# imatge-upc/rsis

Hardware: AMD Instinct MI355X
Metric: training images/sec at 256x256, T=10, batch=32 per GPU (higher is better)
Workload: dtype f32

## Files before the change

### include/rsis_hip.h

```cpp
#ifndef RSIS_HIP_H
#define RSIS_HIP_H
#include <stddef.h>
#ifdef __cplusplus
extern "C" {
#endif

#define RSIS_ABI_VERSION 2

#define RSIS_DTYPE_F32 0
#define RSIS_DTYPE_BF16 1
#define RSIS_DTYPE_BF16_BLK 2
#define RSIS_DTYPE_F32_WINO 3

int rsis_version(void);
const char* rsis_error_string(int code);
int rsis_conv_uses_wino(int ks, int stride, int pad, int Cin, int Cout, int nseg, int lstm_hid);

int rsis_set_deterministic(int on);
int rsis_get_deterministic(void);

int rsis_conv_uses_bf16(int ks, int stride, int pad, int Cout);
long rsis_conv_packed_bytes_fwd(int dtype, int Cout, int ks, int stride, int pad, int nseg, const int* Cseg);
long rsis_conv_packed_bytes_dgrad(int dtype, int Cout, int ks, int stride, int pad, int c_count);
int rsis_conv_pack_fwd(const float* W, void* Wp, int Cout, int Ctot, int ks, int stride, int pad, int nseg, const int* Cseg,
                       const int* Coff, int lstm_hid, int dtype, void* stream);
int rsis_conv_pack_dgrad(const float* W, void* Wd, int Cout, int Ctot, int ks, int stride, int pad, int nseg, const int* Cseg,
                         const int* Coff, int lstm_hid, int dtype, void* stream);

int rsis_conv2d_fwd(const float* const* src, const int* Csrc, int nsrc, int B, int H, int W, const void* Wp, int Cout,
                    int ks, int stride, int pad, const float* bias, const float* addend, float* out, int Ho, int Wo,
                    int tile, int dtype, void* stream);
int rsis_conv2d_fwd_bn_eval(const float* const* src, const int* Csrc, int nsrc, int B, int H, int W, const void* Wp, int Cout,
                            int ks, int stride, int pad, const float* bias, const float* addend, const float* gamma, const float* beta,
                            const float* running_mean, const float* running_var, float eps, int relu, float* out, int Ho, int Wo,
                            int tile, int dtype, void* stream);

int rsis_conv2d_dgrad(const float* dy, int B, int Cout, int Hy, int Wy, const void* Wd, int Cin_packed, int ks, int stride,
                      int pad, float* const* dx, const int* Cdx, int ndst, int Hx, int Wx, const float* addend, int tile,
                      int dtype, void* stream);

int rsis_conv2d_wgrad(const float* dy, const float* x, float* dW, int B, int Cs, int H, int W, int Cout, int Ho, int Wo,
                      int ks, int stride, int pad, int Ctot, int c_off, int lstm_hid, int dtype, void* stream);

typedef struct rsis_wgrad_job {
  const float* dy;
  const float* x;
  float* dW;
  int B, Cs, H, W, Cout, Ho, Wo, ks, stride, pad, Ctot, c_off, lstm_hid, dtype;
} rsis_wgrad_job;
int rsis_conv2d_wgrad_batch(const rsis_wgrad_job* jobs, int njobs, void* stream);

int rsis_bias_grad(const float* dy, float* db, int B, int C, int HW, int lstm_hid, void* stream);

int rsis_convlstm_fwd(const float* const* src, const int* Csrc, int nsrc, int B, int H, int W, const void* Wp,
                      const float* bias_packed, const float* addend, const float* c_prev, float* h_out, float* c_out,
                      float* act_out, int hid, int ks, int pad, int tile, int dtype, void* stream);

typedef struct rsis_lstm_job {
  const float* src[3];
  int Csrc[3];
  int nsrc, B, H, W;
  const void* Wp;
  const float* bias_packed;
  const float* addend;
  const float* c_prev;
  float* h_out;
  float* c_out;
  float* act_out;
  int hid, ks, pad, tile, dtype;
  unsigned long long* side_key;
} rsis_lstm_job;
int rsis_convlstm_fwd_batch(const rsis_lstm_job* jobs, int njobs, void* stream);

int rsis_convlstm_bwd_gates(const float* dh, const float* dh2, const float* dc_next, const float* act, const float* c_prev,
                            const float* c, float* da, float* dc_prev, float* da_sum, int B, int hid, int HW, void* stream);

typedef struct rsis_lstm_bwd_job {
  const float* dh;
  const float* dh2;
  const float* dc_next;
  const float* act;
  const float* c_prev;
  const float* c;
  float* da;
  float* dc_prev;
  int B, hid, HW;
} rsis_lstm_bwd_job;
int rsis_convlstm_bwd_gates_batch(const rsis_lstm_bwd_job* jobs, int njobs, void* stream);
typedef struct rsis_dgrad_job {
  const float* dy;
  int B, Cout, Hy, Wy;
  const void* Wd;
  int Cin_packed, ks, stride, pad;
  float* dx[3];
  int Cdx[3];
// ... 264 lines not shown
```

### rsis_amd/csrc/api.hip

```cpp
#include "common.h"
#include "../../include/rsis_hip.h"
#include "launchers.h"
#include <stdlib.h>

static inline int krows_of(int C, int ks) { return rsis_roundup(C * ks * ks, RSIS_KPAD); }
static inline int log2i(int s) { int l = 0; while ((1 << l) < s) ++l; return l; }
static inline bool use_direct(int ks, int stride, int pad) { return ks == 3 && stride == 1 && pad == 1; }
static inline bool use_direct_s2(int ks, int stride, int pad) { return ks == 3 && stride == 2 && pad == 1; }
static inline bool use_direct_f2(int ks, int stride, int pad) {
  static const bool on = !(getenv("RSIS_CONV_F2") && getenv("RSIS_CONV_F2")[0] == '0');
  return on && use_direct_s2(ks, stride, pad);
}
static inline bool use_direct_fwd(int ks, int stride, int pad) { return use_direct(ks, stride, pad) || use_direct_f2(ks, stride, pad); }
static inline int seg_chunks(int nseg, const int* Cseg, int ck) {
  int q = 0;
  for (int s = 0; s < nseg; ++s) q += (Cseg[s] + ck - 1) / ck;
  return q;
}
static inline int direct_rows(int nseg, const int* Cseg) { return seg_chunks(nseg, Cseg, RSIS_CK) * RSIS_CK * 9; }
static inline bool bf16_geom(int ks, int stride, int pad, int Cout) {
  return Cout > 1 && ((ks == 3 && stride == 1 && pad == 1) || (ks == 1 && pad == 0));
}
static inline bool use_bf16(int dtype, int ks, int stride, int pad, int Cout) {
  return dtype == RSIS_DTYPE_BF16 && bf16_geom(ks, stride, pad, Cout);
}
static inline bool wino_geom(int ks, int stride, int pad, int Cin, int Cout, int nseg, int lstm_hid) {
  return ks == 3 && stride == 1 && pad == 1 && nseg == 1 && lstm_hid == 0 && Cin >= 32 && Cout >= 32 && Cin % 32 == 0 && Cout % 32 == 0;
}
static inline bool wino_geom_dgrad(int ks, int stride, int pad, int Cin, int Cout) {
  return ks == 3 && stride == 1 && pad == 1 && Cin >= 32 && Cout >= 32 && Cin % 32 == 0 && Cout % 32 == 0;
}
static inline bool use_wino(int dtype, int ks, int stride, int pad, int Cin, int Cout, int nseg, int lstm_hid) {
  return dtype == RSIS_DTYPE_F32_WINO && wino_geom(ks, stride, pad, Cin, Cout, nseg, lstm_hid);
}
static inline int bf16_rows(int ks, int nseg, const int* Cseg) {
  const int ckb = bf16_ckb(ks * ks);
  return seg_chunks(nseg, Cseg, ckb) * ks * ks * (ckb / 8);
}
static int g_deterministic = -1;
int rsis_deterministic() {
  if (g_deterministic < 0) g_deterministic = (getenv("RSIS_DETERMINISTIC") && getenv("RSIS_DETERMINISTIC")[0] == '1') ? 1 : 0;
  return g_deterministic;
}
static inline bool conv_splitk_ok() {
  static const bool env_ok = !(getenv("RSIS_CONV_SPLITK") && getenv("RSIS_CONV_SPLITK")[0] == '0');
  return env_ok && !rsis_deterministic();
}
static inline bool splitk_geom(int B, int H, int W, int rows, int nq, int min_chunks) {
  const long px_tiles = (long)B * rsis_cdiv(H, 8) * rsis_cdiv(W, W <= 8 ? 8 : 16);
  return nq >= min_chunks && px_tiles * rsis_cdiv(rows, 64) < 160;
}
static int zero_dsts(const ConvArgs& a, hipStream_t st) {
  for (int i = 0; i < a.ndst; ++i)
    if (rsis_zero_async(a.dst[i], sizeof(float) * (size_t)a.B * a.Cd[i] * a.oH * a.oW, st) != RSIS_OK) return RSIS_ERR_LAUNCH;
  return RSIS_OK;
}
static int splitk_enable(ConvArgs& a, hipStream_t st) { a.ksplit = 0; return zero_dsts(a, st); }
static inline int direct_variant(int tile) { const int v = tile % 10; return (tile > 0 && v >= 1 && v <= 9) ? v : 0; }

extern "C" {

int rsis_version(void) { return RSIS_ABI_VERSION; }

int rsis_set_deterministic(int on) {
  const int prev = rsis_deterministic();
  g_deterministic = on ? 1 : 0;
  return prev;
}
int rsis_get_deterministic(void) { return rsis_deterministic(); }

const char* rsis_error_string(int code) {
  switch (code) {
    case RSIS_OK: return "ok";
    case RSIS_ERR_ARG: return "invalid argument";
    case RSIS_ERR_LAUNCH: return "HIP launch failed";
    case RSIS_ERR_UNSUPPORTED: return "unsupported configuration";
    default: return "unknown error";
  }
}

int rsis_conv_uses_bf16(int ks, int stride, int pad, int Cout) { return bf16_geom(ks, stride, pad, Cout) ? 1 : 0; }
int rsis_conv_uses_wino(int ks, int stride, int pad, int Cin, int Cout, int nseg, int lstm_hid) {
  return wino_geom(ks, stride, pad, Cin, Cout, nseg, lstm_hid) ? 1 : 0;
}

struct PackPlan { int status; PackMode mode; int krows; int ldw; long bytes; };
static PackPlan pack_plan(bool dgrad, int dtype, int Cout, int Ctot, int ks, int stride, int pad, int nseg, const int* Cseg, const int* Coff,
                          int lstm_hid) {
  PackPlan p = {RSIS_OK, PACK_IGEMM_FWD, 0, 0, 0};
  int csum = 0;
  for (int s = 0; s < nseg; ++s) csum += Cseg[s];
  p.ldw = rsis_roundup(dgrad ? csum : Cout, RSIS_LDW_ALIGN);
  if (lstm_hid > 0 && dtype == RSIS_DTYPE_BF16 && ks != 3) { p.status = RSIS_ERR_UNSUPPORTED; return p; }
  if (dtype == RSIS_DTYPE_F32_WINO && (dgrad ? wino_geom_dgrad(ks, stride, pad, csum, Cout) : wino_geom(ks, stride, pad, csum, Cout, nseg, lstm_hid))) {
    if (!dgrad && (csum != Ctot || (Coff && Coff[0] != 0))) { p.status = RSIS_ERR_UNSUPPORTED; return p; }
    p.mode = dgrad ? PACK_WINO_DGRAD : PACK_WINO_FWD;
    p.krows = dgrad ? (csum / 32) * (Cout / 8) : (Cout / 32) * (csum / 8);
    p.bytes = (long)p.krows * 32 * 8 * 16 * 4;
    return p;
  }
  long cell = 4;
  if (use_bf16(dtype, ks, stride, pad, Cout)) {
    p.mode = dgrad ? PACK_BF16_DGRAD : PACK_BF16_FWD;
    p.krows = dgrad ? bf16_rows(ks, 1, &Cout) : bf16_rows(ks, nseg, Cseg);
    cell = 16;
  } else if (dgrad ? use_direct(ks, stride, pad) : use_direct_fwd(ks, stride, pad)) {
    p.mode = dgrad ? PACK_DIRECT_DGRAD : PACK_DIRECT_FWD;
    p.krows = dgrad ? direct_rows(1, &Cout) : direct_rows(nseg, Cseg);
  } else if (dgrad && use_direct_s2(ks, stride, pad) && nseg == 1) {
    p.mode = PACK_DIRECT_DGRAD_S2;
    p.krows = direct_rows(1, &Cout);
  } else {
    p.mode = dgrad ? PACK_IGEMM_DGRAD : PACK_IGEMM_FWD;
    p.krows = krows_of(dgrad ? Cout : csum, ks);
  }
  p.bytes = (long)p.krows * p.ldw * cell;
  return p;
}

long rsis_conv_packed_bytes_fwd(int dtype, int Cout, int ks, int stride, int pad, int nseg, const int* Cseg) {
  if (nseg < 1 || nseg > RSIS_MAX_SRC || !Cseg) return -1;
  int csum = 0;
  for (int s = 0; s < nseg; ++s) csum += Cseg[s];
  return pack_plan(false, dtype, Cout, csum, ks, stride, pad, nseg, Cseg, nullptr, 0).bytes;
}

long rsis_conv_packed_bytes_dgrad(int dtype, int Cout, int ks, int stride, int pad, int c_count) {
  const int one[1] = {c_count}, two[2] = {c_count, 0};
  const long a = pack_plan(true, dtype, Cout, c_count, ks, stride, pad, 1, one, nullptr, 0).bytes;
  const long b = pack_plan(true, dtype, Cout, c_count, ks, stride, pad, 2, two, nullptr, 0).bytes;
  return a > b ? a : b;
}

static int pack_args_check(int Cout, int Ctot, int ks, int nseg, const int* Cseg, const int* Coff, int lstm_hid) {
  if (nseg < 1 || nseg > RSIS_MAX_SRC || !Cseg) return RSIS_ERR_ARG;
  int base = 0;
  for (int s = 0; s < nseg; ++s) {
    const int off = Coff ? Coff[s] : base;
    if (Cseg[s] < 1 || off < 0 || off + Cseg[s] > Ctot) return RSIS_ERR_ARG;
    base += Cseg[s];
  }
  if (Cout < 1 || ks < 1 || (long)Cout * Ctot * ks * ks >= (1L << 31)) return RSIS_ERR_ARG;
  return (lstm_hid > 0 && Cout != 4 * lstm_hid) ? RSIS_ERR_ARG : RSIS_OK;
}

static int pack_one(bool dgrad, const float* W, void* out, int Cout, int Ctot, int ks, int stride, int pad, int nseg, const int* Cseg,
                    const int* Coff, int lstm_hid, int dtype, void* stream) {
  if (!W || !out || pack_args_check(Cout, Ctot, ks, nseg, Cseg, Coff, lstm_hid)) return RSIS_ERR_ARG;
  const PackPlan p = pack_plan(dgrad, dtype, Cout, Ctot, ks, stride, pad, nseg, Cseg, Coff, lstm_hid);
  if (p.status) return p.status;
  return rsis_l_pack(p.mode, W, out, Cout, Ctot, ks, nseg, Cseg, Coff, p.ldw, p.krows, lstm_hid, (hipStream_t)stream);
}
int rsis_conv_pack_fwd(const float* W, void* Wp, int Cout, int Ctot, int ks, int stride, int pad, int nseg, const int* Cseg,
                       const int* Coff, int lstm_hid, int dtype, void* stream) {
  return pack_one(false, W, Wp, Cout, Ctot, ks, stride, pad, nseg, Cseg, Coff, lstm_hid, dtype, stream);
}
int rsis_conv_pack_dgrad(const float* W, void* Wd, int Cout, int Ctot, int ks, int stride, int pad, int nseg, const int* Cseg,
                         const int* Coff, int lstm_hid, int dtype, void* stream) {
  return pack_one(true, W, Wd, Cout, Ctot, ks, stride, pad, nseg, Cseg, Coff, lstm_hid, dtype, stream);
}

int rsis_conv_pack_job_fill(rsis_pack_job* j) {
  if (!j || pack_args_check(j->Cout, j->Ctot, j->ks, j->nseg, j->Cseg, j->Coff, j->lstm_hid)) return -1;
  const PackPlan p = pack_plan(j->dgrad != 0, j->dtype, j->Cout, j->Ctot, j->ks, j->stride, j->pad, j->nseg, j->Cseg, j->Coff, j->lstm_hid);
  if (p.status) return -1;
  j->imode = p.mode; j->krows = p.krows; j->ldw = p.ldw;
  return rsis_l_pack_blocks(p.mode, p.krows, p.ldw, j->ks);
}

int rsis_conv_pack_batch(const rsis_pack_job* jobs_dev, int njobs, int total_blocks, void* stream) {
  if (!jobs_dev || njobs < 1 || total_blocks < 1) return RSIS_ERR_ARG;
  return rsis_l_pack_batch(jobs_dev, njobs, total_blocks, (hipStream_t)stream);
}


int rsis_conv_out_wgrad(const float* dy, const float* x, float* dW, float* db, int B, int Cin, int H, int W, void* stream) {
  if (!dy || !x || !dW || B < 1) return RSIS_ERR_ARG;
  if (!rsis_c1_supported(Cin) || W % 4 != 0) return RSIS_ERR_UNSUPPORTED;
  return rsis_l_c1_wgrad(dy, x, dW, db, B, Cin, H, W, 1, (hipStream_t)stream);
}

static inline bool c1_seq_ok(int T, int B, int Cin, int H, int W) {
  return T >= 1 && B >= 1 && rsis_c1_supported(Cin) && W % 4 == 0 && (long)T * B * Cin * H * W < (1L << 40);
}
int rsis_conv_out_seq_fwd(const float* x, const void* Wp, const float* bias, float* y, int T, int B, int Cin, int H, int W, void* stream) {
// ... 11 lines not shown
  if (!c1_seq_ok(T, B, Cin, H, W)) return RSIS_ERR_UNSUPPORTED;
  return rsis_l_c1_wgrad(dy, x, dW, db, T * B, Cin, H, W, T, (hipStream_t)stream);
}
int rsis_sum_leading(const float* x, float* y, int T, long n, void* stream) {
  if (!x || !y || T < 1 || n < 1) return RSIS_ERR_ARG;
  return rsis_l_sum_leading(x, y, T, n, (hipStream_t)stream);
}

int rsis_affine_nearest(const float* x, float* y, const float* mat, int mat_rows, int N, int C, int H, int W, void* stream) {
  if (!x || !y || !mat || x == y || N < 1 || C < 1 || H < 1 || W < 1 || (mat_rows != 2 && mat_rows != 3)) return RSIS_ERR_ARG;
  if ((long)H * W >= (1L << 31) || N > 65535) return RSIS_ERR_UNSUPPORTED;
  return rsis_l_affine_nearest(x, y, mat, N, C, H, W, mat_rows * 3, (hipStream_t)stream);
}

long rsis_targets_work_ints(int B) { return B < 1 ? 0 : rsis_l_targets_work_ints(B); }

int rsis_targets_from_maps(const int* ins, const int* seg, int B, int H, int W, int T, float* y_mask, long long* y_class, float* sw_mask,
                           float* sw_class, int* work, void* stream) {
  if (!ins || !seg || !y_mask || !y_class || !sw_mask || !sw_class || !work || B < 1 || H < 1 || W < 1 || T < 1) return RSIS_ERR_ARG;
  if ((long)H * W >= (1L << 31) || B > 65535) return RSIS_ERR_UNSUPPORTED;
  return rsis_l_targets_from_maps(ins, seg, B, H, W, T, y_mask, y_class, sw_mask, sw_class, work, (hipStream_t)stream);
}

long rsis_instance_maps_work_ints(int B) { return B < 1 ? 0 : rsis_l_instance_maps_work_ints(B); }

int rsis_instance_maps(const int* raw, const int* class_of_label, int n_labels, int B, int H, int W, int* ins, int* seg, int* work,
                       void* stream) {
  if (!raw || !class_of_label || !ins || !seg || !work || raw == ins || raw == seg || ins == seg || n_labels < 1 || n_labels > 66 ||
      B < 1 || H < 1 || W < 1)
    return RSIS_ERR_ARG;
  if ((long)H * W >= (1L << 31) || B > 65535) return RSIS_ERR_UNSUPPORTED;
  return rsis_l_instance_maps(raw, class_of_label, n_labels, B, H, W, ins, seg, work, (hipStream_t)stream);
}

int rsis_palette_to_ids(const unsigned char* rgb, long npix, const unsigned char* table, int ntab, unsigned char* ids, void* stream) {
  if (!rgb || !table || !ids || npix < 1 || ntab < 1 || ntab > 256) return RSIS_ERR_ARG;
  return rsis_l_palette_to_ids(rgb, npix, table, ntab, ids, (hipStream_t)stream);
}

int rsis_idmap_rle_encode(const unsigned char* idmap, int h, int w, const int* ids, int k, unsigned int* counts, int cap, int* nruns,
                          void* stream) {
  if (!idmap || !ids || !counts || !nruns || h < 1 || w < 1 || k < 1 || cap < 1 || (long)h * w >= (1L << 32)) return RSIS_ERR_ARG;
  return rsis_l_idmap_rle_encode(idmap, h, w, ids, k, counts, cap, nruns, (hipStream_t)stream);
}

static int fill_sources(ConvArgs& a, const float* const* src, const int* Csrc, int nsrc, int ks, bool allow_empty = false) {
  if (nsrc < (allow_empty ? 0 : 1) || nsrc > RSIS_MAX_SRC || (nsrc > 0 && (!src || !Csrc))) return RSIS_ERR_ARG;
  a.nsrc = nsrc;
  a.K = 0;
  for (int s = 0; s < RSIS_MAX_SRC; ++s) { a.src[s] = nsrc > 0 ? src[0] : nullptr; a.C[s] = 0; }
  for (int s = 0; s < nsrc; ++s) {
    if (!src[s] || Csrc[s] < 1) return RSIS_ERR_ARG;
    a.src[s] = src[s]; a.C[s] = Csrc[s]; a.K += Csrc[s] * ks * ks;
  }
  return RSIS_OK;
}

struct BnEval { const float* gamma; const float* beta; const float* mean; const float* var; float eps; int relu; };

static int conv2d_fwd_impl(const float* const* src, const int* Csrc, int nsrc, int B, int H, int W, const void* Wp, int Cout,
                           int ks, int stride, int pad, const float* bias, const float* addend, float* out, int Ho, int Wo,
                           int tile, int dtype, void* stream, const BnEval* bn) {
  const bool allow_splitk = tile >= 100;
  tile %= 100;
  ConvArgs a = {};
  int rc = fill_sources(a, src, Csrc, nsrc, ks);
  if (rc) return rc;
  if (!Wp || !out || B < 1 || stride < 1) return RSIS_ERR_ARG;
  if (Ho != (H + 2 * pad - ks) / stride + 1 || Wo != (W + 2 * pad - ks) / stride + 1) return RSIS_ERR_ARG;
  a.B = B; a.H = H; a.W = W; a.Ho = Ho; a.Wo = Wo; a.stride = stride; a.pad = pad; a.sshift = 0;
  a.wp = (const float*)Wp; a.ldw = rsis_roundup(Cout, RSIS_LDW_ALIGN); a.Cout = Cout; a.bias = bias; a.addend = addend;
  a.dst[0] = out; a.Cd[0] = Cout; a.ndst = 1;
  a.ostride = 1; a.oH = Ho; a.oW = Wo; a.ksplit = 1;
  a.precise = allow_splitk ? 0 : 1;
  if (bn) {
    if (!bn->gamma || !bn->beta || !bn->mean || !bn->var) return RSIS_ERR_ARG;
    if (allow_splitk || Cout % 4 != 0 || (size_t)B * Cout * Ho * Wo * 4 >= (1ull << 31)) return RSIS_ERR_UNSUPPORTED;
    if (dtype != RSIS_DTYPE_F32 && (dtype != RSIS_DTYPE_BF16 || use_bf16(dtype, ks, stride, pad, Cout))) return RSIS_ERR_UNSUPPORTED;
    if (use_direct(ks, stride, pad) && Cout == 1) return RSIS_ERR_UNSUPPORTED;
    a.ep_gamma = bn->gamma; a.ep_beta = bn->beta; a.ep_mean = bn->mean; a.ep_var = bn->var; a.ep_eps = bn->eps; a.ep_relu = bn->relu ? 1 : 0;
  }
  if (use_wino(dtype, ks, stride, pad, Csrc[0], Cout, nsrc, 0))
    return rsis_launch_conv_wino(src[0], Wp, bias, addend, out, B, Csrc[0], Cout, H, W, (hipStream_t)stream, a.precise);
  if (use_bf16(dtype, ks, stride, pad, Cout)) {
    if (stride != 1) return RSIS_ERR_UNSUPPORTED;
    if (ks == 1 && nsrc != 1) return RSIS_ERR_UNSUPPORTED;
    if (ks == 3 && allow_splitk && conv_splitk_ok() && !addend && splitk_geom(B, H, W, Cout, seg_chunks(a.nsrc, a.C, RSIS_CKB3), 16) &&
        splitk_enable(a, (hipStream_t)stream))
      return RSIS_ERR_LAUNCH;
    return rsis_launch_conv_bf16(a, ks, 0, direct_variant(tile), (hipStream_t)stream);
  }
  if (use_direct(ks, stride, pad) && Cout == 1 && nsrc == 1 && !addend && rsis_c1_supported(Csrc[0]) && W % 4 == 0)
    return rsis_l_c1_fwd(src[0], (const float*)Wp, a.ldw, bias, out, B, Csrc[0], H, W, 1, (hipStream_t)stream);
  if (use_direct(ks, stride, pad)) {
    if (allow_splitk && conv_splitk_ok() && splitk_geom(B, H, W, Cout, seg_chunks(a.nsrc, a.C, RSIS_CK), 32) && splitk_enable(a, (hipStream_t)stream))
      return RSIS_ERR_LAUNCH;
    return rsis_launch_conv3x3_direct(a, 0, direct_variant(tile), (hipStream_t)stream);
  }
  if (use_direct_f2(ks, stride, pad))
    return rsis_launch_conv3x3_direct(a, 3, direct_variant(tile), (hipStream_t)stream);
  return rsis_launch_conv_igemm(a, ks, false, 0, tile, (hipStream_t)stream);
}

int rsis_conv2d_fwd(const float* const* src, const int* Csrc, int nsrc, int B, int H, int W, const void* Wp, int Cout,
                    int ks, int stride, int pad, const float* bias, const float* addend, float* out, int Ho, int Wo,
                    int tile, int dtype, void* stream) {
  return conv2d_fwd_impl(src, Csrc, nsrc, B, H, W, Wp, Cout, ks, stride, pad, bias, addend, out, Ho, Wo, tile, dtype, stream, nullptr);
}

int rsis_conv2d_fwd_bn_eval(const float* const* src, const int* Csrc, int nsrc, int B, int H, int W, const void* Wp, int Cout,
                            int ks, int stride, int pad, const float* bias, const float* addend, const float* gamma, const float* beta,
                            const float* running_mean, const float* running_var, float eps, int relu, float* out, int Ho, int Wo,
                            int tile, int dtype, void* stream) {
  const BnEval bn = {gamma, beta, running_mean, running_var, eps, relu};
  return conv2d_fwd_impl(src, Csrc, nsrc, B, H, W, Wp, Cout, ks, stride, pad, bias, addend, out, Ho, Wo, tile % 100, dtype, stream, &bn);
}

static int dgrad_fill(ConvArgs& a, const float* dy, int B, int Cout, int Hy, int Wy, const void* Wd, int Cin_packed, int ks, int stride, int pad,
                      float* const* dx, const int* Cdx, int ndst, int Hx, int Wx, const float* addend) {
  a = ConvArgs{};
  const float* srcs[1] = {dy};
  const int cs[1] = {Cout};
  const int rc = fill_sources(a, srcs, cs, 1, ks);
  if (rc) return rc;
  int ctot = 0;
  for (int i = 0; i < ndst; ++i) { if (!dx[i] || Cdx[i] < 1) return RSIS_ERR_ARG; a.dst[i] = dx[i]; a.Cd[i] = Cdx[i]; ctot += Cdx[i]; }
  if (ctot > Cin_packed) return RSIS_ERR_ARG;
  a.ndst = ndst;
  a.B = B; a.H = Hy; a.W = Wy; a.Ho = Hx; a.Wo = Wx; a.stride = stride; a.pad = pad; a.sshift = log2i(stride);
  a.ostride = 1; a.oH = Hx; a.oW = Wx; a.ksplit = 1;
  a.wp = (const float*)Wd; a.ldw = rsis_roundup(Cin_packed, RSIS_LDW_ALIGN); a.Cout = ctot; a.bias = nullptr; a.addend = addend;
  return RSIS_OK;
}

int rsis_conv2d_dgrad(const float* dy, int B, int Cout, int Hy, int Wy, const void* Wd, int Cin_packed, int ks, int stride,
                      int pad, float* const* dx, const int* Cdx, int ndst, int Hx, int Wx, const float* addend, int tile,
                      int dtype, void* stream) {
  if (!dy || !Wd || !dx || !Cdx || ndst < 1 || ndst > RSIS_MAX_SRC) return RSIS_ERR_ARG;
  const bool inplace = addend && ndst == 1 && stride > 1 && ks == 1 && pad == 0 && addend == dx[0];
  if (addend && !inplace && (ndst != 1 || stride != 1)) return RSIS_ERR_UNSUPPORTED;
  if (stride != 1 && stride != 2 && stride != 4) return RSIS_ERR_UNSUPPORTED;
  ConvArgs a;
  const int rc = dgrad_fill(a, dy, B, Cout, Hy, Wy, Wd, Cin_packed, ks, stride, pad, dx, Cdx, ndst, Hx, Wx, addend);
  if (rc) return rc;
  const int ctot = a.Cout;
  if (dtype == RSIS_DTYPE_F32_WINO && wino_geom_dgrad(ks, stride, pad, Cin_packed, Cout)) {
    if (ndst > 2 || ctot % 32 != 0 || Cdx[0] % 32 != 0 || Hx != Hy || Wx != Wy || (ndst == 2 && addend)) return RSIS_ERR_UNSUPPORTED;
    if (ndst == 1) return rsis_launch_conv_wino(dy, Wd, nullptr, addend, dx[0], B, Cout, ctot, Hy, Wy, (hipStream_t)stream, 0);
    const float* xs[1] = {dy}; const void* us[1] = {Wd}; float* y0[1] = {dx[0]}; float* y1[1] = {dx[1]};
    const int b1[1] = {B}, c1[1] = {Cout}, co1[1] = {ctot}, c01[1] = {Cdx[0]}, h1[1] = {Hy}, w1[1] = {Wy};
    return rsis_launch_conv_wino_group(1, xs, us, y0, y1, b1, c1, co1, c01, h1, w1, (hipStream_t)stream);
  }
  if (use_bf16(dtype, ks, stride, pad, Cout)) {
    if (ks == 3) {
      if (Hx != Hy || Wx != Wy) return RSIS_ERR_ARG;
      if (conv_splitk_ok() && !addend && splitk_geom(B, Hx, Wx, ctot, seg_chunks(a.nsrc, a.C, RSIS_CKB3), 16) && splitk_enable(a, (hipStream_t)stream))
        return RSIS_ERR_LAUNCH;
      return rsis_launch_conv_bf16(a, 3, 0, direct_variant(tile), (hipStream_t)stream);
    }
    if (stride > 1) {
      if (Hy != (Hx - 1) / stride + 1 || Wy != (Wx - 1) / stride + 1) return RSIS_ERR_ARG;
      if (!inplace && zero_dsts(a, (hipStream_t)stream)) return RSIS_ERR_LAUNCH;
      a.ostride = stride;
    } else if (Hx != Hy || Wx != Wy) return RSIS_ERR_ARG;
    a.Ho = Hy; a.Wo = Wy; a.stride = 1; a.sshift = 0;
    return rsis_launch_conv_bf16(a, 1, 0, direct_variant(tile), (hipStream_t)stream);
  }
  if (use_direct(ks, stride, pad)) {
    if (Hx != Hy || Wx != Wy) return RSIS_ERR_ARG;
    if (Cout == 1 && ndst == 1 && Cin_packed == Cdx[0] && rsis_c1_supported(Cdx[0]) && !addend)
      return rsis_l_c1_dgrad(dy, (const float*)Wd, a.ldw, dx[0], B, Cdx[0], Hx, Wx, 1, (hipStream_t)stream);
    if (conv_splitk_ok() && !addend && splitk_geom(B, Hx, Wx, ctot, seg_chunks(a.nsrc, a.C, RSIS_CK), 32) && splitk_enable(a, (hipStream_t)stream))
      return RSIS_ERR_LAUNCH;
    return rsis_launch_conv3x3_direct(a, 0, direct_variant(tile), (hipStream_t)stream);
  }
  if (use_direct_s2(ks, stride, pad) && ndst == 1 && Cdx[0] == Cin_packed && Hy == (Hx + 1) / 2 && Wy == (Wx + 1) / 2) {
    a.Ho = Hy; a.Wo = Wy; a.oH = Hx; a.oW = Wx;
    return rsis_launch_conv3x3_direct(a, 2, direct_variant(tile), (hipStream_t)stream);
  }
  if (ks == 1 && pad == 0 && stride > 1) {
    if (!inplace && zero_dsts(a, (hipStream_t)stream)) return RSIS_ERR_LAUNCH;
    a.Ho = Hy; a.Wo = Wy; a.stride = 1; a.sshift = 0; a.ostride = stride;
    return rsis_launch_conv_igemm(a, ks, false, 0, tile, (hipStream_t)stream);
  }
  return rsis_launch_conv_igemm(a, ks, true, 0, tile, (hipStream_t)stream);
}

static int wgrad_route(WgradArgs& a, int ks, int lstm_hid, int dtype) {
  if (dtype == RSIS_DTYPE_BF16_BLK) {
    a.blk = 1;
    return rsis_wgrad_bf16_supported(a, ks) ? 1 : -1;
  }
  if (dtype != RSIS_DTYPE_BF16) {
    const int staged = rsis_wgrad_staged_limbs(a, ks);
    if (staged < 0) return -1;
    if (staged > 0) { a.limbs = 1; return 1; }
  }
  if (use_direct(ks, a.stride, a.pad) && a.Cout == 1 && lstm_hid == 0 && rsis_c1_supported(a.Cs) && a.H == a.Ho && a.W == a.Wo && a.W % 4 == 0)
    return 0;
  if (dtype == RSIS_DTYPE_BF16 && rsis_wgrad_bf16_supported(a, ks)) return 1;
  static const bool tiled_ok = !(getenv("RSIS_WGRAD_TILED") && getenv("RSIS_WGRAD_TILED")[0] == '0');
  if (tiled_ok && rsis_wgrad_tiled_supported(a, ks)) return 2;
  return 3;
}
static int wgrad_fill(WgradArgs& a, const float* dy, const float* x, float* dW, int B, int Cs, int H, int W, int Cout, int Ho, int Wo,
                      int ks, int stride, int pad, int Ctot, int c_off, int lstm_hid) {
  if (!dy || !x || !dW || c_off < 0 || c_off + Cs > Ctot) return RSIS_ERR_ARG;
  a = WgradArgs{};
  a.dy = dy; a.x = x; a.dw = dW; a.B = B; a.Cs = Cs; a.H = H; a.W = W; a.Ho = Ho; a.Wo = Wo; a.Cout = Cout;
  a.stride = stride; a.pad = pad; a.ldo = Ctot * ks * ks; a.n_off = c_off * ks * ks; a.interleave_hid = lstm_hid;
  return RSIS_OK;
}
static int wgrad_launch_one(WgradArgs& a, int route, int ks, hipStream_t st) {
  switch (route) {
    case 0: return rsis_l_c1_wgrad(a.dy, a.x, a.dw + a.n_off, nullptr, a.B, a.Cs, a.H, a.W, 1, st);
    case 1: return rsis_launch_conv_wgrad_bf16(a, ks, st);
    case 2: return rsis_launch_conv_wgrad_tiled(a, ks, st);
    default: return rsis_launch_conv_wgrad(a, ks, st);
  }
}

int rsis_conv2d_wgrad(const float* dy, const float* x, float* dW, int B, int Cs, int H, int W, int Cout, int Ho, int Wo,
                      int ks, int stride, int pad, int Ctot, int c_off, int lstm_hid, int dtype, void* stream) {
  WgradArgs a;
  const int rc = wgrad_fill(a, dy, x, dW, B, Cs, H, W, Cout, Ho, Wo, ks, stride, pad, Ctot, c_off, lstm_hid);
  if (rc) return rc;
  const int route = wgrad_route(a, ks, lstm_hid, dtype);
  if (route < 0) return RSIS_ERR_UNSUPPORTED;
  return wgrad_launch_one(a, route, ks, (hipStream_t)stream);
}

int rsis_conv2d_wgrad_batch(const rsis_wgrad_job* jobs, int njobs, void* stream) {
  if (!jobs || njobs < 1) return RSIS_ERR_ARG;
  WgradArgs* tiled[4] = {(WgradArgs*)malloc(sizeof(WgradArgs) * njobs), (WgradArgs*)malloc(sizeof(WgradArgs) * njobs),
                         (WgradArgs*)malloc(sizeof(WgradArgs) * njobs), (WgradArgs*)malloc(sizeof(WgradArgs) * njobs)};
  int nt[4] = {0, 0, 0, 0};
  int rc = (tiled[0] && tiled[1] && tiled[2] && tiled[3]) ? RSIS_OK : RSIS_ERR_LAUNCH;
  for (int j = 0; j < njobs && rc == RSIS_OK; ++j) {
    const rsis_wgrad_job& q = jobs[j];
    WgradArgs a;
    rc = wgrad_fill(a, q.dy, q.x, q.dW, q.B, q.Cs, q.H, q.W, q.Cout, q.Ho, q.Wo, q.ks, q.stride, q.pad, q.Ctot, q.c_off, q.lstm_hid);
    if (rc) break;
    const int route = wgrad_route(a, q.ks, q.lstm_hid, q.dtype);
    if (route < 0) { rc = RSIS_ERR_UNSUPPORTED; break; }
    if ((route == 1 || route == 2) && (q.ks == 1 || q.ks == 3) && !rsis_deterministic()) {
      const int li = (route == 1 ? 2 : 0) + (q.ks == 3);
      tiled[li][nt[li]++] = a;
    } else rc = wgrad_launch_one(a, route, q.ks, (hipStream_t)stream);
  }
  if (rc == RSIS_OK) rc = rsis_launch_conv_wgrad_tiled_group(tiled[0], nt[0], 1, (hipStream_t)stream);
  if (rc == RSIS_OK) rc = rsis_launch_conv_wgrad_tiled_group(tiled[1], nt[1], 3, (hipStream_t)stream);
  if (rc == RSIS_OK) rc = rsis_launch_conv_wgrad_bf16_group(tiled[2], nt[2], 1, (hipStream_t)stream);
  if (rc == RSIS_OK) rc = rsis_launch_conv_wgrad_bf16_group(tiled[3], nt[3], 3, (hipStream_t)stream);
  for (int i = 0; i < 4; ++i) free(tiled[i]);
  return rc;
}

int rsis_bias_grad(const float* dy, float* db, int B, int C, int HW, int lstm_hid, void* stream) {
  if (!dy || !db) return RSIS_ERR_ARG;
  return rsis_l_channel_sum(dy, db, B, C, HW, lstm_hid, (hipStream_t)stream);
}

static int lstm_fill(ConvArgs& a, int& route, const float* const* src, const int* Csrc, int nsrc, int B, int H, int W, const void* Wp,
                     const float* bias_packed, const float* addend, const float* c_prev, float* h_out, float* c_out, float* act_out, int hid,
                     int ks, int pad, int dtype, unsigned long long* side_key = nullptr) {
  a = ConvArgs{};
  int rc = fill_sources(a, src, Csrc, nsrc, ks, addend != nullptr);
  if (rc) return rc;
  if (!Wp || !h_out || !c_out || hid < 1 || B < 1) return RSIS_ERR_ARG;
  if (2 * pad != ks - 1) return RSIS_ERR_UNSUPPORTED;
  if (dtype == RSIS_DTYPE_BF16 && ks != 3) return RSIS_ERR_UNSUPPORTED;
  a.B = B; a.H = H; a.W = W; a.Ho = H; a.Wo = W; a.stride = 1; a.pad = pad; a.sshift = 0;
  a.wp = (const float*)Wp; a.ldw = rsis_roundup(4 * hid, RSIS_LDW_ALIGN); a.Cout = 4 * hid; a.bias = bias_packed; a.addend = addend;
  a.ndst = 1; a.dst[0] = nullptr; a.Cd[0] = 4 * hid;
  a.hid = hid; a.c_prev = c_prev; a.h_out = h_out; a.c_out = c_out; a.act_out = act_out;
  a.ostride = 1; a.oH = H; a.oW = W; a.ksplit = 1;
  route = use_bf16(dtype, ks, 1, pad, 4 * hid) ? 0 : (use_direct(ks, 1, pad) ? 1 : 2);
  a.side_key = side_key;
  a.precise = act_out ? 0 : 1;
  if (side_key && (route == 2 || (long)H * W >= 0x7FFFFFFFL)) return RSIS_ERR_UNSUPPORTED;
  return RSIS_OK;
}
static int lstm_launch_one(ConvArgs& a, int route, int ks, int tile, hipStream_t st) {
  if (route == 0) return rsis_launch_conv_bf16(a, 3, 1, direct_variant(tile), st);
  if (route == 1) return rsis_launch_conv3x3_direct(a, 1, direct_variant(tile), st);
  return rsis_launch_conv_igemm(a, ks, false, 1, tile, st);
}

int rsis_convlstm_fwd(const float* const* src, const int* Csrc, int nsrc, int B, int H, int W, const void* Wp,
                      const float* bias_packed, const float* addend, const float* c_prev, float* h_out, float* c_out,
                      float* act_out, int hid, int ks, int pad, int tile, int dtype, void* stream) {
  ConvArgs a;
  int route = 0;
  const int rc = lstm_fill(a, route, src, Csrc, nsrc, B, H, W, Wp, bias_packed, addend, c_prev, h_out, c_out, act_out, hid, ks, pad, dtype);
  if (rc) return rc;
  return lstm_launch_one(a, route, ks, tile, (hipStream_t)stream);
}

int rsis_convlstm_fwd_batch(const rsis_lstm_job* jobs, int njobs, void* stream) {
  if (!jobs || njobs < 1) return RSIS_ERR_ARG;
  ConvArgs* grp = (ConvArgs*)malloc(sizeof(ConvArgs) * njobs);
  int* force = (int*)malloc(sizeof(int) * njobs);
  if (!grp || !force) { free(grp); free(force); return RSIS_ERR_LAUNCH; }
  int ng = 0, rc = RSIS_OK;
  for (int j = 0; j < njobs && rc == RSIS_OK; ++j) {
    const rsis_lstm_job& q = jobs[j];
    if (q.nsrc < 0 || q.nsrc > RSIS_MAX_SRC) { rc = RSIS_ERR_ARG; break; }
    ConvArgs a;
    int route = 0;
    rc = lstm_fill(a, route, q.src, q.Csrc, q.nsrc, q.B, q.H, q.W, q.Wp, q.bias_packed, q.addend, q.c_prev, q.h_out, q.c_out, q.act_out,
                   q.hid, q.ks, q.pad, q.dtype, q.side_key);
    if (rc) break;
    const bool groupable = route == 1 && (size_t)q.B * 4 * q.hid * q.H * q.W * 4 < (1ull << 31) && !rsis_deterministic();
    if (groupable) { force[ng] = direct_variant(q.tile % 100); grp[ng++] = a; }
    else rc = lstm_launch_one(a, route, q.ks, q.tile, (hipStream_t)stream);
  }
  if (rc == RSIS_OK && ng == 1) rc = rsis_launch_conv3x3_direct(grp[0], 1, force[0], (hipStream_t)stream);
  else if (rc == RSIS_OK && ng > 1) rc = rsis_launch_convlstm_direct_group(grp, ng, force, (hipStream_t)stream);
  free(grp); free(force);
  return rc;
}

int rsis_convlstm_bwd_gates(const float* dh, const float* dh2, const float* dc_next, const float* act, const float* c_prev,
                            const float* c, float* da, float* dc_prev, float* da_sum, int B, int hid, int HW, void* stream) {
  if (!act || !c || !da) return RSIS_ERR_ARG;
  return rsis_l_lstm_bwd(dh, dh2, dc_next, act, c_prev, c, da, dc_prev, da_sum, B, hid, HW, (hipStream_t)stream);
}

int rsis_upsample_bilinear_ac_fwd(const float* x, float* y, long BC, int Hi, int Wi, int Ho, int Wo, void* stream) {
  if (!x || !y) return RSIS_ERR_ARG;
  return rsis_l_upsample_fwd(x, y, BC, Hi, Wi, Ho, Wo, nullptr, (hipStream_t)stream);
}
int rsis_upsample_bilinear_ac_scaled_fwd(const float* x, const float* scale, float* y, long BC, int Hi, int Wi, int Ho, int Wo, void* stream) {
  if (!x || !y || BC < 1 || Hi < 1 || Wi < 1 || Ho < 1 || Wo < 1) return RSIS_ERR_ARG;
  if (scale && Hi == Ho && Wi == Wo) return rsis_l_scale_planes(x, scale, y, BC, Hi * Wi, (hipStream_t)stream);
  return rsis_l_upsample_fwd(x, y, BC, Hi, Wi, Ho, Wo, scale, (hipStream_t)stream);
}
int rsis_upsample_maxpool_scaled_bwd(const float* dy, const float* dpool, const int* argmax, const float* scale, float* dx, long BC, int Hi, int Wi,
                                     int Ho, int Wo, void* stream) {
  if (!dy || !dx || !dpool || !argmax || BC < 1 || Hi < 1 || Wi < 1 || Ho < 1 || Wo < 1) return RSIS_ERR_ARG;
  return rsis_l_upsample_bwd(dy, dx, BC, Hi, Wi, Ho, Wo, dpool, argmax, scale, (hipStream_t)stream);
}
int rsis_global_maxpool_scaled_bwd_add(const float* dy, const int* argmax, const float* scale, float* dx, long BC, int HW, void* stream) {
  if (!dy || !dx || !argmax || BC < 1 || HW < 1) return RSIS_ERR_ARG;
  return rsis_l_gmax_bwd_add(dy, argmax, dx, BC, HW, scale, (hipStream_t)stream);
}
int rsis_scale_planes(const float* x, const float* scale, float* y, long BC, int HW, void* stream) {
  if (!x || !scale || !y || BC < 1 || HW < 1) return RSIS_ERR_ARG;
  return rsis_l_scale_planes(x, scale, y, BC, HW, (hipStream_t)stream);
}
int rsis_dropout_scales(unsigned int* state, float* s2, float* mc, float* ms, long n, float p2, float pc, float ps, void* stream) {
  if (!state || !s2 || !mc || !ms || n < 1 || n > (1L << 33)) return RSIS_ERR_ARG;
  if (!(p2 >= 0.f && p2 < 1.f) || !(pc >= 0.f && pc < 1.f) || !(ps >= 0.f && ps < 1.f)) return RSIS_ERR_ARG;
  return rsis_l_dropout_scales(state, s2, mc, ms, n, p2, pc, ps, (hipStream_t)stream);
}
int rsis_dropout_heads_mask(float* side, const float* s2, const float* mc, const float* ms, float* side_c, float* side_s, long n, void* stream) {
  if (!side || !s2 || !mc || !ms || !side_c || !side_s || n < 1) return RSIS_ERR_ARG;
  return rsis_l_dropout_heads_mask(side, s2, mc, ms, side_c, side_s, n, (hipStream_t)stream);
}
int rsis_dropout_heads_mask_bwd(const float* dside_c, const float* dside_s, const float* mc, const float* ms, float* dside, long n, void* stream) {
  if (!mc || !ms || !dside || n < 1) return RSIS_ERR_ARG;
  return rsis_l_dropout_heads_mask_bwd(dside_c, dside_s, mc, ms, dside, n, (hipStream_t)stream);
// ... 453 lines not shown
    const int rc = blk_resize_jobs(&plain, 1, &out[j], bwd);
    if (rc) return rc;
    out[j].scale = q.scale;
  }
  return RSIS_OK;
}
int rsis_blk_upsample_fwd_scaled_batch(const rsis_blk_resize_scaled_job* jobs, int njobs, void* stream) {
  BlkResizeScaledJob a[64];
  const int rc = blk_resize_scaled_jobs(jobs, njobs, a, false);
  return rc ? rc : rsis_l_blk_upsample_fwd_scaled(a, njobs, (hipStream_t)stream);
}
int rsis_blk_upsample_bwd_scaled_batch(const rsis_blk_resize_scaled_job* jobs, int njobs, void* stream) {
  BlkResizeScaledJob a[64];
  const int rc = blk_resize_scaled_jobs(jobs, njobs, a, true);
  return rc ? rc : rsis_l_blk_upsample_bwd_scaled(a, njobs, (hipStream_t)stream);
}
int rsis_blk_lstm_bwd_batch(const rsis_blk_lstm_bwd_job* jobs, int njobs, void* stream) {
  if (!jobs || njobs < 1 || njobs > 64) return RSIS_ERR_ARG;
  BlkLstmBwdJob a[64];
  for (int j = 0; j < njobs; ++j) {
    const rsis_blk_lstm_bwd_job& q = jobs[j];
    if (!q.dh || !q.act || !q.c || !q.da || q.B < 1 || q.hid < 8 || (q.hid & 7) || q.HW < 1) return RSIS_ERR_ARG;
    a[j].dh = q.dh; a[j].dh2 = q.dh2; a[j].dc_next = q.dc_next; a[j].act = q.act; a[j].c_prev = q.c_prev; a[j].c = q.c; a[j].da = q.da;
    a[j].dc_prev = q.dc_prev; a[j].B = q.B; a[j].hid = q.hid; a[j].HW = q.HW;
  }
  return rsis_l_blk_lstm_bwd(a, njobs, (hipStream_t)stream);
}
static inline bool blk_c1_ok(int T, int B, int H, int W) { return T >= 1 && B >= 1 && H >= 1 && W >= 4 && W % 4 == 0 && (long)H * W < (1L << 27); }
int rsis_blk_conv_out_seq_fwd(const void* x, const float* Wref, const float* bias, float* y, int T, int B, int H, int W, void* stream) {
  if (!x || !Wref || !y) return RSIS_ERR_ARG;
  if (!blk_c1_ok(T, B, H, W)) return RSIS_ERR_UNSUPPORTED;
  return rsis_l_blk_c1_fwd(x, Wref, bias, y, T, B, H, W, (hipStream_t)stream);
}
int rsis_blk_conv_out_seq_dgrad(const float* dy, const float* Wref, void* dx, int T, int B, int H, int W, void* stream) {
  if (!dy || !Wref || !dx) return RSIS_ERR_ARG;
  if (!blk_c1_ok(T, B, H, W)) return RSIS_ERR_UNSUPPORTED;
  return rsis_l_blk_c1_dgrad(dy, Wref, dx, T, B, H, W, (hipStream_t)stream);
}
int rsis_blk_conv_out_seq_wgrad(const float* dy, const void* x, float* dW, float* db, int T, int B, int H, int W, void* stream) {
  if (!dy || !x || !dW) return RSIS_ERR_ARG;
  if (!blk_c1_ok(T, B, H, W)) return RSIS_ERR_UNSUPPORTED;
  return rsis_l_blk_c1_wgrad(dy, x, dW, db, T, B, H, W, (hipStream_t)stream);
}
int rsis_blk_sum_leading(const void* x, void* y, int T, long ncells, void* stream) {
  if (!x || !y || T < 1 || ncells < 1) return RSIS_ERR_ARG;
  return rsis_l_blk_sum_leading(x, y, T, ncells, (hipStream_t)stream);
}
int rsis_blk_bias_grad(const void* dy, float* db, int B, int C, int HW, int lstm_hid, void* stream) {
  if (!dy || !db || B < 1 || C < 8 || (C & 7) || HW < 1 || (lstm_hid > 0 && C != 4 * lstm_hid)) return RSIS_ERR_ARG;
  return rsis_l_blk_channel_sum(dy, db, B, C, HW, lstm_hid, (hipStream_t)stream);
}

int rsis_convlstm_bwd_gates_batch(const rsis_lstm_bwd_job* jobs, int njobs, void* stream) {
  if (!jobs || njobs < 1 || njobs > 64) return RSIS_ERR_ARG;
  const void* ptrs[64 * 8];
  int dims[64 * 3];
  for (int j = 0; j < njobs; ++j) {
    const rsis_lstm_bwd_job& q = jobs[j];
    if (!q.act || !q.c || !q.da || q.B < 1 || q.hid < 1 || q.HW < 1) return RSIS_ERR_ARG;
    const void* p8[8] = {q.dh, q.dh2, q.dc_next, q.act, q.c_prev, q.c, q.da, q.dc_prev};
    for (int k = 0; k < 8; ++k) ptrs[j * 8 + k] = p8[k];
    dims[j * 3] = q.B; dims[j * 3 + 1] = q.hid; dims[j * 3 + 2] = q.HW;
  }
  return rsis_l_lstm_bwd_group(ptrs, dims, njobs, (hipStream_t)stream);
}
int rsis_conv2d_dgrad_batch(const rsis_dgrad_job* jobs, int njobs, void* stream) {
  if (!jobs || njobs < 1 || njobs > 64) return RSIS_ERR_ARG;
  ConvArgs grp[64];
  int force[64], ng = 0, rc = RSIS_OK;
  const float* wx[4]; const void* wu[4]; float* wy0[4]; float* wy1[4];
  int wb[4], wc[4], wco[4], wc0[4], wh[4], ww[4], nw = 0;
  for (int j = 0; j < njobs && rc == RSIS_OK; ++j) {
    const rsis_dgrad_job& q = jobs[j];
    if (!q.dy || !q.Wd || q.ndst < 1 || q.ndst > RSIS_MAX_SRC) return RSIS_ERR_ARG;
    int ctot = 0;
    for (int i = 0; i < q.ndst; ++i) { if (!q.dx[i] || q.Cdx[i] < 1) return RSIS_ERR_ARG; ctot += q.Cdx[i]; }
    if (q.dtype == RSIS_DTYPE_F32_WINO && wino_geom_dgrad(q.ks, q.stride, q.pad, q.Cin_packed, q.Cout) && !q.addend && q.ndst <= 2 &&
        ctot % 32 == 0 && q.Cdx[0] % 32 == 0 && q.Hx == q.Hy && q.Wx == q.Wy) {
      wx[nw] = q.dy; wu[nw] = q.Wd; wy0[nw] = q.dx[0]; wy1[nw] = q.ndst == 2 ? q.dx[1] : nullptr;
      wb[nw] = q.B; wc[nw] = q.Cout; wco[nw] = ctot; wc0[nw] = q.Cdx[0]; wh[nw] = q.Hy; ww[nw] = q.Wy;
      if (++nw == 4) { rc = rsis_launch_conv_wino_group(nw, wx, wu, wy0, wy1, wb, wc, wco, wc0, wh, ww, (hipStream_t)stream); nw = 0; }
      continue;
    }
    const bool groupable = q.dtype == RSIS_DTYPE_F32 && use_direct(q.ks, q.stride, q.pad) && !q.addend && q.Hx == q.Hy && q.Wx == q.Wy &&
                           !(q.Cout == 1) && ctot <= q.Cin_packed && (size_t)q.B * (ctot > q.Cout ? ctot : q.Cout) * q.Hy * q.Wy * 4 < (1ull << 31) &&
                           !rsis_deterministic();
    if (!groupable) {
      rc = rsis_conv2d_dgrad(q.dy, q.B, q.Cout, q.Hy, q.Wy, q.Wd, q.Cin_packed, q.ks, q.stride, q.pad, q.dx, q.Cdx, q.ndst, q.Hx, q.Wx, q.addend, q.tile,
                             q.dtype, stream);
      continue;
    }
    rc = dgrad_fill(grp[ng], q.dy, q.B, q.Cout, q.Hy, q.Wy, q.Wd, q.Cin_packed, q.ks, q.stride, q.pad, q.dx, q.Cdx, q.ndst, q.Hx, q.Wx, q.addend);
    if (rc) break;
    force[ng++] = direct_variant(q.tile);
  }
  if (rc == RSIS_OK && nw > 0) rc = rsis_launch_conv_wino_group(nw, wx, wu, wy0, wy1, wb, wc, wco, wc0, wh, ww, (hipStream_t)stream);
  if (rc == RSIS_OK && ng == 1) rc = rsis_launch_conv3x3_direct(grp[0], 0, force[0], (hipStream_t)stream);
  else if (rc == RSIS_OK && ng > 1) rc = rsis_launch_conv3x3_direct_group_plain(grp, ng, force, (hipStream_t)stream);
  return rc;
}

int rsis_upconv_out_supported(int C, int Hs, int Ws, int Ho, int Wo) { return rsis_upconv_supported(C, Hs, Ws, Ho, Wo) ? 1 : 0; }
int rsis_upconv_out_bwd_blocks(int T, int B, int Hs, int Ws) { return rsis_upconv_bwd_blocks(T, B, Hs, Ws); }
int rsis_upconv_out_fwd(const void* h, int h_blk, const float* w, const float* bias, float* out, int T, int B, int C, int Hs, int Ws, int Ho, int Wo,
                        void* stream) {
  if (!h || !w || !out || T < 1 || B < 1) return RSIS_ERR_ARG;
  if (!rsis_upconv_supported(C, Hs, Ws, Ho, Wo)) return RSIS_ERR_UNSUPPORTED;
  return rsis_l_upconv_fwd(h, h_blk, w, bias, out, T, B, Hs, Ws, Ho, Wo, (hipStream_t)stream);
}
int rsis_upconv_out_bwd(const float* dout, const void* h, int h_blk, const float* w, void* dh, float* dW, float* db, const float* dside, const int* arg,
                        float* partial, int T, int B, int C, int Hs, int Ws, int Ho, int Wo, void* stream) {
  if (!dout || !h || !w || !dh || !partial || T < 1 || B < 1 || (dside && !arg)) return RSIS_ERR_ARG;
  if (!rsis_upconv_supported(C, Hs, Ws, Ho, Wo)) return RSIS_ERR_UNSUPPORTED;
  return rsis_l_upconv_bwd(dout, h, h_blk, w, dh, dW, db, dside, arg, partial, T, B, Hs, Ws, Ho, Wo, (hipStream_t)stream);
}
}
```

### rsis_amd/csrc/common.h

```cpp
#pragma once
#include <hip/hip_runtime.h>
#include <stdint.h>

#define RSIS_OK 0
#define RSIS_ERR_ARG 1
#define RSIS_ERR_LAUNCH 2
#define RSIS_ERR_UNSUPPORTED 3

#define RSIS_KPAD 32
#define RSIS_CK 8
#define RSIS_CKB3 16
#define RSIS_CKB1 64
#define RSIS_LDW_ALIGN 128
#define RSIS_MAX_SRC 3

enum PackMode {
  PACK_IGEMM_FWD = 0,
  PACK_IGEMM_DGRAD = 1,
  PACK_DIRECT_FWD = 2,
  PACK_DIRECT_DGRAD = 3,
  PACK_DIRECT_DGRAD_S2 = 4,
  PACK_BF16_FWD = 5,
  PACK_BF16_DGRAD = 6,
  PACK_WINO_FWD = 7,
  PACK_WINO_DGRAD = 8
};
__host__ __device__ __forceinline__ int bf16_ckb(int KK) { return KK == 1 ? RSIS_CKB1 : RSIS_CKB3; }

typedef float f32x16 __attribute__((ext_vector_type(16)));
typedef float f32x4 __attribute__((ext_vector_type(4)));

static inline int rsis_check_launch() {
  hipError_t e = hipGetLastError();
  return e == hipSuccess ? RSIS_OK : RSIS_ERR_LAUNCH;
}

int rsis_zero_async(void* p, size_t bytes, hipStream_t st);

int rsis_deterministic();

static inline int ew_grid(long total) {
  long g = (total + 255) / 256;
  if (g > 256 * 16) g = 256 * 16;
  if (g < 1) g = 1;
  return (int)g;
}
static inline int rsis_cdiv(long a, long b) { return (int)((a + b - 1) / b); }
static inline int rsis_roundup(int a, int b) { return ((a + b - 1) / b) * b; }

__device__ __forceinline__ void rsis_bn_affine(float rstd, float gamma, float beta, float mean, float& sc, float& sh) {
  sc = rstd * gamma;
  sh = __builtin_fmaf(-mean, sc, beta);
}
__device__ __forceinline__ float rsis_bn_eval_rstd(float var, float eps) { return 1.0f / sqrtf(var + eps); }
__device__ __forceinline__ float rsis_bn_apply(float v, float sc, float sh, float r, int relu) {
  const float t = __builtin_fmaf(v, sc, sh) + r;
  return relu ? fmaxf(t, 0.f) : t;
}
__device__ __forceinline__ float rsis_sigmoid(float x) { return 1.0f / (1.0f + expf(-x)); }
__device__ __forceinline__ float rsis_sigmoid_fast(float x) { return __builtin_amdgcn_rcpf(1.0f + __builtin_amdgcn_exp2f(-1.4426950408889634f * x)); }
__device__ __forceinline__ float rsis_tanh_fast(float x) { return 2.0f * __builtin_amdgcn_rcpf(1.0f + __builtin_amdgcn_exp2f(-2.8853900817779268f * x)) - 1.0f; }

__device__ __forceinline__ void ac_coord(int o, float scale, int in, int& i0, int& i1, float& l1) {
  const float of = (float)o;
  const float src = scale * of;
  i0 = (int)src;
  if (i0 > in - 1) i0 = in - 1;
  i1 = i0 + (i0 < in - 1 ? 1 : 0);
  l1 = fmaf(scale, of, -(float)i0);
}
static inline float ac_scale(int in, int out) { return out > 1 ? (float)(in - 1) / (float)(out - 1) : 0.f; }

struct ConvArgs {
  const float* src[RSIS_MAX_SRC];
  int C[RSIS_MAX_SRC];
  int nsrc;
  int K;
  int B, H, W;
  int Ho, Wo;
  int stride, pad, sshift;
  const float* wp;
  int ldw;
  int Cout;
  const float* bias;
  const float* addend;
  const float* ep_gamma; const float* ep_beta; const float* ep_mean; const float* ep_var;
  float ep_eps;
  int ep_relu, ep_round;
  float* dst[RSIS_MAX_SRC];
  int Cd[RSIS_MAX_SRC];
  int ndst;
  int n_co_tiles, n_px_tiles;
  int ostride, oH, oW;
  int ksplit;
  int hid;
  const float* c_prev;
  float* h_out;
  float* c_out;
  float* act_out;
  unsigned long long* side_key;
  int precise;
};

__device__ __forceinline__ unsigned long long rsis_side_key(float v, int idx) {
  unsigned u = __float_as_uint(v);
  u = (u & 0x80000000u) ? ~u : (u | 0x80000000u);
  return ((unsigned long long)u << 32) | (unsigned)(0x7FFFFFFF - idx);
}
__device__ __forceinline__ float rsis_side_value(unsigned long long k) {
  unsigned u = (unsigned)(k >> 32);
  u = (u & 0x80000000u) ? (u & 0x7FFFFFFFu) : ~u;
  return __uint_as_float(u);
}
__device__ __forceinline__ int rsis_side_index(unsigned long long k) { return 0x7FFFFFFF - (int)(unsigned)(k & 0xFFFFFFFFull); }
__device__ __forceinline__ unsigned long long rsis_key_max32(unsigned long long k) {
#pragma unroll
  for (int o = 16; o > 0; o >>= 1) {
    const unsigned long long t = __shfl_xor(k, o, 64);
    k = t > k ? t : k;
  }
  return k;
}

#define RSIS_SIDE_CHECK_TILES 192
__device__ __forceinline__ void rsis_side_key_max4(unsigned long long* row, int j0, int hid, const unsigned long long* k, bool lane_ok, bool check) {
  unsigned long long cur[4] = {0ull, 0ull, 0ull, 0ull};
  if (check && lane_ok) {
#pragma unroll
    for (int r4 = 0; r4 < 4; ++r4) cur[r4] = __hip_atomic_load(row + (j0 + 2 * r4 < hid ? j0 + 2 * r4 : 0), __ATOMIC_RELAXED, __HIP_MEMORY_SCOPE_AGENT);
  }
#pragma unroll
  for (int r4 = 0; r4 < 4; ++r4)
    if (lane_ok && k[r4] != 0ull && j0 + 2 * r4 < hid && k[r4] > cur[r4]) atomicMax(row + j0 + 2 * r4, k[r4]);
}

__device__ __forceinline__ void rsis_side_key_block(unsigned long long* park, int wave, int WGM, int WGN, int hi, const unsigned long long* kk,
                                                    bool lane_ok, unsigned long long* row, int jbase, int hid, bool check) {
  if (lane_ok) {
#pragma unroll
    for (int r4 = 0; r4 < 4; ++r4) park[wave * 8 + 2 * r4 + hi] = kk[r4];
  }
  __syncthreads();
  const int t = threadIdx.x;
  if (t < WGM * 8) {
    const int wm = t >> 3, c = t & 7;
    unsigned long long k = 0ull;
    for (int wn = 0; wn < WGN; ++wn) {
      const unsigned long long v = park[(wm * WGN + wn) * 8 + c];
      k = v > k ? v : k;
    }
    const int j = jbase + t;
    if (k != 0ull && j < hid) {
      const unsigned long long cur = check ? __hip_atomic_load(row + j, __ATOMIC_RELAXED, __HIP_MEMORY_SCOPE_AGENT) : 0ull;
      if (k > cur) atomicMax(row + j, k);
    }
  }
}

struct WgradArgs {
  const float* dy;
  const float* x;
  float* dw;
  int B, Cs, H, W, Ho, Wo, Cout;
  int stride, pad;
  int ldo, n_off;
  int interleave_hid;
  int chunk;
  int n_co_tiles, n_n_tiles;
  int blk;
  int limbs;
};

struct BlkConvJob {
  const void* src[RSIS_MAX_SRC];
  int C[RSIS_MAX_SRC];
  int nsrc;
  int B, H, W;
  const void* wp;
  int ldw;
  int Cout;
  const float* bias;
  const void* addend;
  void* dst[2];
  int Cd[2];
// ... 31 lines not shown
```

### rsis_amd/csrc/conv3x3_direct.hip

```cpp
#include "common.h"
#include "launchers.h"
#include <stdlib.h>
#ifndef XCD_CHUNKED
#define XCD_CHUNKED 1
#endif

enum { EPI_PLAIN = 0, EPI_LSTM = 1, EPI_S2 = 2, EPI_F2 = 3 };
typedef __attribute__((address_space(3))) void* lds_vp_t;
#define CK RSIS_CK
#ifndef RSIS_ACC_FLUSH
#define RSIS_ACC_FLUSH 4
#endif
#define RSIS_FLUSH_MIN_CHUNKS 48

typedef const float __attribute__((address_space(1)))* gcf_t;
typedef float __attribute__((address_space(1)))* gf_t;
typedef const f32x4 __attribute__((address_space(1)))* gcf4_t;

template <int BM, int TW, int TH, int NI, int EPI, int NWV>
constexpr int direct_lds_floats() {
  constexpr int S = EPI == EPI_F2 ? 2 : 1;
  constexpr int PW = TW * S + 3 - S, PH = TH * S + 3 - S;
  constexpr int XS = CK * NI * PH * PW, WS = CK * 9 * BM, NT = NWV * 64;
  return 2 * ((XS + NT - 1) / NT * NT + WS);
}

template <int BM, int TW, int TH, int NI, int EPI, int KSP = 1, int NWV = 4, bool FLUSH = false, bool BNE = false>
__device__ __forceinline__ void conv3x3_direct_body(const ConvArgs& p, const int bid, const int kz, const int ksplit, float* const lds) {
#if __HIP_DEVICE_COMPILE__
  constexpr int BN = TW * TH * NI;
  constexpr int NT = NWV * 64;
  constexpr int WGM = BM / 32, WGN = NWV / WGM / KSP;
  constexpr int TN = BN / WGN / 32;
  constexpr int S = EPI == EPI_F2 ? 2 : 1;
  constexpr int PW = TW * S + 3 - S, PH = TH * S + 3 - S;
  constexpr int IMS = PH * PW;
  constexpr int CHS = NI * IMS;
  constexpr int XS = CK * CHS, WS = CK * 9 * BM;
  constexpr int XSP = (XS + NT - 1) / NT * NT;
  constexpr int NX = (XS + NT - 1) / NT;
  constexpr int W_F4 = WS / 4;
  constexpr int NW = (W_F4 + NT - 1) / NT;
  static_assert(TN >= 1 && BN % (WGN * 32) == 0 && WGM * WGN * KSP == NWV && (CK / 2) % KSP == 0 && (KSP == 1 || EPI != EPI_S2), "tile");

  static_assert(2 * (XSP + WS) == direct_lds_floats<BM, TW, TH, NI, EPI, NWV>(), "LDS size helper out of sync");
  float* const Xs0 = lds;
  float* const Ws0 = lds + 2 * XSP;

  const gcf_t src0 = (gcf_t)p.src[0], src1 = (gcf_t)p.src[1], src2 = (gcf_t)p.src[2];
  const int C0 = p.C[0], C1 = p.C[1], C2 = p.C[2];
  const int q0 = (C0 + CK - 1) / CK, q1 = (C1 + CK - 1) / CK, q2 = (C2 + CK - 1) / CK;
  const int nq_all = q0 + q1 + q2;
  const int q_begin = (int)((long)nq_all * kz / ksplit), q_end = (int)((long)nq_all * (kz + 1) / ksplit);
  const int nq = q_end - q_begin;
  const int Hs = p.H, Ws = p.W, HWs = Hs * Ws;
  const int H = EPI == EPI_F2 ? p.Ho : p.H, W = EPI == EPI_F2 ? p.Wo : p.W, HW = H * W, B = p.B;
  const int ldw = p.ldw;

  const int xcd = bid & 7, q = bid >> 3;
  const int co_t = q % p.n_co_tiles;
  const int sp_t = XCD_CHUNKED ? xcd * ((p.n_px_tiles + 7) >> 3) + q / p.n_co_tiles : (q / p.n_co_tiles) * 8 + xcd;
  if (sp_t >= p.n_px_tiles) return;
  const int tiles_x = (W + TW - 1) / TW, tiles_y = (H + TH - 1) / TH;
  const int tx = sp_t % tiles_x;
  const int ty = (sp_t / tiles_x) % tiles_y;
  const int b0 = (sp_t / (tiles_x * tiles_y)) * NI;
  const int x0 = tx * TW, y0 = ty * TH;

  const int tid = threadIdx.x;
  const int lane = tid & 63, l31 = lane & 31, hi = lane >> 5;
  const int wave = __builtin_amdgcn_readfirstlane(tid >> 6);
  const int wk = wave / (WGM * WGN);
  const int wm = (wave / WGN) % WGM, wn = wave % WGN;

  static_assert(NI == 1, "LDS-DMA staging addresses one image per block");
  unsigned xvo[NX];
#pragma unroll
  for (int i = 0; i < NX; ++i) {
    const int e = tid + i * NT;
    const int cl = e / CHS, rem2 = e - cl * CHS;
    const int py = rem2 / PW, pxx = rem2 - py * PW;
    const int gy = y0 * S + py - 1, gx = x0 * S + pxx - 1;
    const bool ok = (e < XS) && ((unsigned)gy < (unsigned)Hs) && ((unsigned)gx < (unsigned)Ws);
    xvo[i] = ok ? (unsigned)(cl * HWs + gy * Ws + gx) * 4u : 0x7FFFFFF0u;
  }
  unsigned wvo[NW];
#pragma unroll
  for (int i = 0; i < NW; ++i) {
    const int idx = tid + i * NT;
    const int row = idx / (BM / 4), c4 = idx % (BM / 4);
    wvo[i] = (unsigned)(row * ldw + c4 * 4) * 4u;
  }

  int xoff[TN];
#pragma unroll
  for (int j = 0; j < TN; ++j) {
    const int pp = (wn * TN + j) * 32 + l31;
    const int x = pp % TW, y = (pp / TW) % TH, img = pp / (TW * TH);
    xoff[j] = hi * CHS + img * IMS + y * S * PW + x * S;
  }
  constexpr int C2W = CK / 2 / KSP;
  const int woff = hi * BM + wm * 32 + l31 + wk * (C2W * 9 * 2) * BM;
  const int xk = wk * (2 * C2W) * CHS;

  constexpr int NACC = EPI == EPI_S2 ? 4 : 1;
  f32x16 accs[NACC][TN];
#pragma unroll
  for (int c = 0; c < NACC; ++c)
#pragma unroll
    for (int j = 0; j < TN; ++j)
#pragma unroll
      for (int r = 0; r < 16; ++r) accs[c][j][r] = 0.f;
  f32x16 (&acc)[TN] = accs[0];

  const gcf_t wbase = (gcf_t)p.wp + co_t * BM;

  int cs = 0, cq = q_begin;
  if (cs == 0 && cq >= q0 && q0 < nq_all) { cq -= q0; cs = 1; }
  if (cs == 1 && cq >= q1 && q0 + q1 < nq_all) { cq -= q1; cs = 2; }

#define DIRECT_ISSUE(QG, BUF)                                                                             \
  {                                                                                                       \
    gcf_t src = src0; int Cs = C0;                                                                        \
    if (cs == 1) { src = src1; Cs = C1; }                                                                 \
    if (cs == 2) { src = src2; Cs = C2; }                                                                 \
    const int c0 = cq * CK;                                                                               \
    const int cn = min(CK, Cs - c0);                                                                      \
    const float* xb = (const float*)src + ((size_t)b0 * Cs + c0) * HWs;                                   \
    const __amdgpu_buffer_rsrc_t rx_ = __builtin_amdgcn_make_buffer_rsrc((void*)xb, 0, cn * HWs * 4, 0x00020000); \
    float* Xs = Xs0 + (BUF) * XSP + wave * 64;                                                            \
    _Pragma("unroll") for (int i = 0; i < NX; ++i)                                                        \
      __builtin_amdgcn_raw_ptr_buffer_load_lds(rx_, (lds_vp_t)(Xs + i * NT), 4, xvo[i], 0, 0, 0);        \
    const float* wrow = (const float*)wbase + (size_t)(QG) * (CK * 9) * ldw;                              \
    const __amdgpu_buffer_rsrc_t rw_ = __builtin_amdgcn_make_buffer_rsrc((void*)wrow, 0, CK * 9 * ldw * 4, 0x00020000); \
    float* Ws = Ws0 + (BUF) * WS + wave * 256;                                                            \
    _Pragma("unroll") for (int i = 0; i < NW; ++i)                                                        \
      if (W_F4 % NT == 0 || i * NT + wave * 64 < W_F4)                                                    \
        __builtin_amdgcn_raw_ptr_buffer_load_lds(rw_, (lds_vp_t)(Ws + i * NT * 4), 16, wvo[i], 0, 0, 0);  \
    if (++cq == (cs == 0 ? q0 : (cs == 1 ? q1 : q2))) { cq = 0; ++cs; if (cs == 1 && q1 == 0) ++cs; }     \
  }
#define DIRECT_LAND() __builtin_amdgcn_s_waitcnt(0x0F70);
  if (nq > 0) DIRECT_ISSUE(q_begin, 0)
  DIRECT_LAND()
  __syncthreads();
  static_assert(!FLUSH || EPI == EPI_PLAIN || EPI == EPI_LSTM, "segmented accumulation: plain and LSTM epilogues");
  f32x16 tot[FLUSH ? TN : 1];
  if constexpr (FLUSH) {
#pragma unroll
    for (int j = 0; j < TN; ++j)
#pragma unroll
      for (int r = 0; r < 16; ++r) tot[j][r] = 0.f;
  }
  for (int t = 0; t < nq; ++t) {
    const int cur = t & 1;
    const bool more = t + 1 < nq;
    if constexpr (FLUSH) {
      if (t > 0 && (t & (RSIS_ACC_FLUSH - 1)) == 0) {
#pragma unroll
        for (int j = 0; j < TN; ++j)
#pragma unroll
          for (int r = 0; r < 16; ++r) { tot[j][r] += acc[j][r]; acc[j][r] = 0.f; }
      }
    }
    if (more) DIRECT_ISSUE(q_begin + t + 1, cur ^ 1)
    {
      const float* Xs = Xs0 + cur * XSP;
      const float* Ws = Ws0 + cur * WS + woff;
#pragma unroll
      for (int c2 = 0; c2 < C2W; ++c2)
#pragma unroll
        for (int r = 0; r < 3; ++r)
#pragma unroll
          for (int s = 0; s < 3; ++s) {
            const float a = Ws[((c2 * 9 + r * 3 + s) * 2) * BM];
            float b[TN];
#pragma unroll
            for (int j = 0; j < TN; ++j)
              b[j] = Xs[xk + xoff[j] + (2 * c2) * CHS + (EPI == EPI_S2 ? ((r == 0) + 1) * PW + (s == 0) + 1 : r * PW + s)];
            const int cls = EPI == EPI_S2 ? (r != 1) * 2 + (s != 1) : 0;
#pragma unroll
            for (int j = 0; j < TN; ++j) accs[cls][j] = __builtin_amdgcn_mfma_f32_32x32x2f32(a, b[j], accs[cls][j], 0, 0, 0);
          }
    }
    DIRECT_LAND()
    __syncthreads();
  }
#undef DIRECT_ISSUE
#undef DIRECT_LAND
  if constexpr (FLUSH) {
#pragma unroll
    for (int j = 0; j < TN; ++j)
#pragma unroll
      for (int r = 0; r < 16; ++r) acc[j][r] += tot[j][r];
  }

  if constexpr (BNE) {
    float* tab = lds + direct_lds_floats<BM, TW, TH, NI, EPI, NWV>() - 2 * BM;
    if (tid < BM) {
      const int row = co_t * BM + tid;
      float sc = 0.f, sh = 0.f;
      if (row < p.Cout) rsis_bn_affine(rsis_bn_eval_rstd(p.ep_var[row], p.ep_eps), p.ep_gamma[row], p.ep_beta[row], p.ep_mean[row], sc, sh);
      tab[tid] = sc; tab[BM + tid] = sh;
    }
    if constexpr (KSP == 1) __syncthreads();
  }
  if constexpr (KSP > 1) {
    float* red = lds + ((wm * WGN + wn) * TN) * 16 * 64;
    if (wk > 0) {
#pragma unroll
      for (int j = 0; j < TN; ++j)
#pragma unroll
        for (int r = 0; r < 16; ++r) red[(j * 16 + r) * 64 + lane] = acc[j][r];
    }
    __syncthreads();
    if (wk > 0) return;
#pragma unroll
    for (int j = 0; j < TN; ++j)
#pragma unroll
      for (int r = 0; r < 16; ++r) acc[j][r] += red[(j * 16 + r) * 64 + lane];
  }
  const int co_base = co_t * BM + wm * 32;
  const gcf_t bias = (gcf_t)p.bias, addend = (gcf_t)p.addend;
  unsigned long long best[4] = {0ull, 0ull, 0ull, 0ull};
  float bv[16];
  {
    const int nrows = EPI == EPI_LSTM ? 4 * p.hid : p.Cout;
    const __amdgpu_buffer_rsrc_t rb = __builtin_amdgcn_make_buffer_rsrc((void*)(bias ? (const void*)p.bias : (const void*)p.wp), 0, bias ? nrows * 4 : 0, 0x00020000);
#pragma unroll
    for (int r = 0; r < 16; ++r)
      bv[r] = __builtin_bit_cast(float, __builtin_amdgcn_raw_buffer_load_b32(rb, (unsigned)(co_base + 4 * hi + (r & 3) + 8 * (r >> 2)) * 4u, 0, 0));
  }
#pragma unroll
  for (int j = 0; j < TN; ++j) {
    const int pp = (wn * TN + j) * 32 + l31;
    const int x = pp % TW, y = (pp / TW) % TH, img = pp / (TW * TH);
    const int ob = b0 + img, oy = y0 + y, ox = x0 + x;
    const bool inb = ob < B && oy < H && ox < W;
    const bool fast_plain = (EPI == EPI_PLAIN || EPI == EPI_F2) && p.ndst == 1 && ksplit == 1 && (size_t)B * p.Cout * HW * 4 < (1ull << 31);
    const bool fast_lstm = EPI == EPI_LSTM && (size_t)p.B * 4 * p.hid * HW * 4 < (1ull << 31);
    if (!inb && !fast_plain && !fast_lstm) continue;
    const int osp = oy * W + ox;
    if (EPI == EPI_S2) {
      const gf_t d0 = (gf_t)p.dst[0];
      const int Cd0 = p.Cd[0], oH = p.oH, oW = p.oW;
#pragma unroll
      for (int c = 0; c < NACC; ++c) {
        const int py = 2 * oy + (c >> 1), px = 2 * ox + (c & 1);
        if (py >= oH || px >= oW) continue;
#pragma unroll
        for (int r = 0; r < 16; ++r) {
          const int co = co_base + (r & 3) + 8 * (r >> 2) + 4 * hi;
          if (co < Cd0) d0[((size_t)ob * Cd0 + co) * ((size_t)oH * oW) + py * oW + px] = accs[c][j][r];
        }
      }
    } else if (EPI == EPI_PLAIN || EPI == EPI_F2) {
      const gf_t d0 = (gf_t)p.dst[0], d1 = (gf_t)p.dst[1], d2 = (gf_t)p.dst[2];
      const int Cd0 = p.Cd[0], Cd1 = p.Cd[1], Cd2 = p.Cd[2], Cout = p.Cout;
      const int e1 = Cd0, e2 = Cd0 + Cd1;
      if (fast_plain) {
        const __amdgpu_buffer_rsrc_t ro = __builtin_amdgcn_make_buffer_rsrc((void*)p.dst[0], 0, (unsigned)((size_t)B * Cout * HW * 4), 0x00020000);
        const __amdgpu_buffer_rsrc_t ra = __builtin_amdgcn_make_buffer_rsrc((void*)(addend ? p.addend : p.dst[0]), 0, (unsigned)((size_t)B * Cout * HW * 4), 0x00020000);
        const unsigned vo = (unsigned)((ob * Cout + co_base + 4 * hi) * HW + osp) * 4u;
        const unsigned rowb = (unsigned)HW * 4u;
        const int rows_left = inb ? Cout - (co_base + 4 * hi) : 0;
        float av[16];
        if (addend) {
#pragma unroll
          for (int r = 0; r < 16; ++r) {
            const int k = (r & 3) + 8 * (r >> 2);
            av[r] = __builtin_bit_cast(float, __builtin_amdgcn_raw_buffer_load_b32(ra, k < rows_left ? vo + k * rowb : 0x7FFFFFF0u, 0, 0));
          }
        }
        if constexpr (BNE) {
          const float* tab = lds + direct_lds_floats<BM, TW, TH, NI, EPI, NWV>() - 2 * BM + wm * 32 + 4 * hi;
#pragma unroll
          for (int g = 0; g < 4; ++g) {
// ... 44 lines not shown
        const __amdgpu_buffer_rsrc_t r_c = __builtin_amdgcn_make_buffer_rsrc((void*)p.c_out, 0, sspan, 0x00020000);
        const __amdgpu_buffer_rsrc_t r_h = __builtin_amdgcn_make_buffer_rsrc((void*)p.h_out, 0, sspan, 0x00020000);
        const unsigned rowb = (unsigned)HW * 4u;
        const int jh0 = (co_base >> 2) + hi;
        const unsigned vg = (unsigned)((ob * 4 * hid + 4 * jh0) * HW + osp) * 4u;
        const unsigned vs = (unsigned)((ob * hid + jh0) * HW + osp) * 4u;
        float ga[4][4], cpv[4];
#pragma unroll
        for (int r4 = 0; r4 < 4; ++r4) {
          const bool ok = inb && jh0 + 2 * r4 < hid;
#pragma unroll
          for (int g = 0; g < 4; ++g)
            ga[r4][g] = __builtin_bit_cast(float, __builtin_amdgcn_raw_buffer_load_b32(r_add, ok ? vg + (8 * r4 + g) * rowb : 0x7FFFFFF0u, 0, 0));
          cpv[r4] = __builtin_bit_cast(float, __builtin_amdgcn_raw_buffer_load_b32(r_cp, ok ? vs + 2 * r4 * rowb : 0x7FFFFFF0u, 0, 0));
        }
#pragma unroll
        for (int r4 = 0; r4 < 4; ++r4) {
          const bool ok = inb && jh0 + 2 * r4 < hid;
          const float ai = acc[j][4 * r4 + 0] + ga[r4][0] + bv[4 * r4 + 0], af = acc[j][4 * r4 + 1] + ga[r4][1] + bv[4 * r4 + 1];
          const float ao = acc[j][4 * r4 + 2] + ga[r4][2] + bv[4 * r4 + 2], ag = acc[j][4 * r4 + 3] + ga[r4][3] + bv[4 * r4 + 3];
          const float gi = rsis_sigmoid(ai), gf = rsis_sigmoid(af), go = rsis_sigmoid(ao), gg = tanhf(ag);
          const float c = gf * cpv[r4] + gi * gg;
          const float h = go * tanhf(c);
          if (p.side_key && ok) { const unsigned long long k = rsis_side_key(h, osp); best[r4] = k > best[r4] ? k : best[r4]; }
          const unsigned os = ok ? vs + 2 * r4 * rowb : 0x7FFFFFF0u, og = ok ? vg + 8 * r4 * rowb : 0x7FFFFFF0u;
          __builtin_amdgcn_raw_buffer_store_b32(__builtin_bit_cast(unsigned, c), r_c, os, 0, 0);
          __builtin_amdgcn_raw_buffer_store_b32(__builtin_bit_cast(unsigned, h), r_h, os, 0, 0);
          __builtin_amdgcn_raw_buffer_store_b32(__builtin_bit_cast(unsigned, gi), r_act, og, 0, 0);
          __builtin_amdgcn_raw_buffer_store_b32(__builtin_bit_cast(unsigned, gf), r_act, og + rowb, 0, 0);
          __builtin_amdgcn_raw_buffer_store_b32(__builtin_bit_cast(unsigned, go), r_act, og + 2 * rowb, 0, 0);
          __builtin_amdgcn_raw_buffer_store_b32(__builtin_bit_cast(unsigned, gg), r_act, og + 3 * rowb, 0, 0);
        }
        continue;
      }
      if (!inb) continue;
#pragma unroll
      for (int r4 = 0; r4 < 4; ++r4) {
        const int jh = (co_base >> 2) + 2 * r4 + hi;
        if (jh >= hid) continue;
        const int cop = jh * 4;
        float ai = acc[j][4 * r4 + 0], af = acc[j][4 * r4 + 1], ao = acc[j][4 * r4 + 2], ag = acc[j][4 * r4 + 3];
        if (bias) { ai += bias[cop]; af += bias[cop + 1]; ao += bias[cop + 2]; ag += bias[cop + 3]; }
        const size_t gidx = ((size_t)ob * 4 * hid + cop) * HW + osp;
        if (addend) {
          ai += addend[gidx]; af += addend[gidx + HW];
          ao += addend[gidx + 2 * (size_t)HW]; ag += addend[gidx + 3 * (size_t)HW];
        }
        const float gi = rsis_sigmoid(ai), gf = rsis_sigmoid(af), go = rsis_sigmoid(ao), gg = tanhf(ag);
        const size_t sidx = ((size_t)ob * hid + jh) * HW + osp;
        const float cp = c_prev ? c_prev[sidx] : 0.f;
        const float c = gf * cp + gi * gg;
        const float h = go * tanhf(c);
        if (p.side_key) { const unsigned long long k = rsis_side_key(h, osp); best[r4] = k > best[r4] ? k : best[r4]; }
        c_out[sidx] = c;
        h_out[sidx] = h;
        if (act_out) {
          act_out[gidx] = gi; act_out[gidx + HW] = gf;
          act_out[gidx + 2 * (size_t)HW] = go; act_out[gidx + 3 * (size_t)HW] = gg;
        }
      }
    }
  }
  if constexpr (EPI == EPI_LSTM) {
    if (p.side_key) {
      unsigned long long kk[4];
#pragma unroll
      for (int r4 = 0; r4 < 4; ++r4) kk[r4] = rsis_key_max32(best[r4]);
      if constexpr (KSP == 1)
        rsis_side_key_block((unsigned long long*)lds, wave, WGM, WGN, hi, kk, l31 == 0, p.side_key + (size_t)b0 * p.hid, (co_t * BM) >> 2, p.hid,
                            tiles_x * tiles_y >= RSIS_SIDE_CHECK_TILES);
      else
        rsis_side_key_max4(p.side_key + (size_t)b0 * p.hid, (co_base >> 2) + hi, p.hid, kk, l31 == 0, tiles_x * tiles_y >= RSIS_SIDE_CHECK_TILES);
    }
  }
#endif
}

template <int BM, int TW, int TH, int NI, int EPI, int KSP = 1, int NWV = 4, bool FLUSH = false, bool BNE = false>
__global__ __launch_bounds__(NWV * 64) void conv3x3_direct_kernel(const ConvArgs p) {
  __shared__ __attribute__((aligned(16))) float lds[direct_lds_floats<BM, TW, TH, NI, EPI, NWV>()];
  conv3x3_direct_body<BM, TW, TH, NI, EPI, KSP, NWV, FLUSH, BNE>(p, blockIdx.x, blockIdx.y, gridDim.y, lds);
}

#define RSIS_DG_MAXJ 8
constexpr int cmax(int a, int b) { return a > b ? a : b; }
struct DirectGroup {
  int n;
  int begin[RSIS_DG_MAXJ + 1];
  int variant[RSIS_DG_MAXJ];
  ConvArgs job[RSIS_DG_MAXJ];
};
static_assert(sizeof(DirectGroup) <= 4000, "kernel arguments are limited to 4 KB");

template <int EPI, bool FLUSH = false>
__global__ __launch_bounds__(256) void conv3x3_direct_group_kernel(const DirectGroup g) {
  constexpr int LMAX = cmax(cmax(direct_lds_floats<32, 16, 8, 1, EPI, 4>(), direct_lds_floats<32, 32, 8, 1, EPI, 4>()),
                            direct_lds_floats<32, 8, 8, 1, EPI, 4>());
  __shared__ __attribute__((aligned(16))) float lds[LMAX];
  const int b = blockIdx.x;
  int j = 0;
#pragma unroll
  for (int k = 1; k < RSIS_DG_MAXJ; ++k) j += (k < g.n && g.begin[k] <= b) ? 1 : 0;
  const ConvArgs& p = g.job[j];
  const int local = b - g.begin[j];
  switch (g.variant[j]) {
    case 4: conv3x3_direct_body<32, 16, 8, 1, EPI, 1, 4, FLUSH>(p, local, 0, 1, lds); break;
    case 5: conv3x3_direct_body<32, 32, 8, 1, EPI, 1, 4, FLUSH>(p, local, 0, 1, lds); break;
    default: conv3x3_direct_body<32, 8, 8, 1, EPI, 2, 4, FLUSH>(p, local, 0, 1, lds); break;
  }
}

template <int BM, int TW, int TH, int NI, int EPI, int KSP = 1, int NWV = 4>
static int launch_direct_cfg(ConvArgs& a, hipStream_t st) {
  a.n_co_tiles = rsis_cdiv(a.Cout, BM);
  const int gw = EPI == EPI_F2 ? a.Wo : a.W, gh = EPI == EPI_F2 ? a.Ho : a.H;
  a.n_px_tiles = rsis_cdiv(gw, TW) * rsis_cdiv(gh, TH) * rsis_cdiv(a.B, NI);
  const int grid = a.n_co_tiles * 8 * rsis_cdiv(a.n_px_tiles, 8);
  int ksplit = 1;
  if (EPI == EPI_PLAIN && a.ksplit == 0) {
    int nq = 0;
    for (int s = 0; s < a.nsrc; ++s) nq += (a.C[s] + RSIS_CK - 1) / RSIS_CK;
    const int blocks = a.n_co_tiles * a.n_px_tiles;
    if (blocks < 160 && nq >= 32) {
      ksplit = rsis_cdiv(512, blocks);
      if (ksplit > nq / 8) ksplit = nq / 8;
      if (ksplit > 16) ksplit = 16;
      if (ksplit < 1) ksplit = 1;
    }
  }
  if (a.ep_gamma) {
    if constexpr (EPI == EPI_PLAIN || EPI == EPI_F2) {
      if (ksplit != 1 || a.ndst != 1 || a.Cout % 4 != 0 || (size_t)a.B * a.Cout * a.H * a.W * 4 >= (1ull << 31)) return RSIS_ERR_UNSUPPORTED;
      hipLaunchKernelGGL((conv3x3_direct_kernel<BM, TW, TH, NI, EPI, KSP, NWV, NWV == 4 && EPI == EPI_PLAIN, true>), dim3(grid, 1), dim3(NWV * 64), 0, st, a);
      return rsis_check_launch();
    } else {
      return RSIS_ERR_UNSUPPORTED;
    }
  }
  if constexpr ((EPI == EPI_PLAIN || EPI == EPI_LSTM) && NWV == 4) {
    int nq = 0;
    for (int s = 0; s < a.nsrc; ++s) nq += (a.C[s] + RSIS_CK - 1) / RSIS_CK;
    if (nq / ksplit >= RSIS_FLUSH_MIN_CHUNKS || (a.precise && nq / ksplit > RSIS_ACC_FLUSH)) {
      hipLaunchKernelGGL((conv3x3_direct_kernel<BM, TW, TH, NI, EPI, KSP, NWV, true>), dim3(grid, ksplit), dim3(NWV * 64), 0, st, a);
      return rsis_check_launch();
    }
  }
  hipLaunchKernelGGL((conv3x3_direct_kernel<BM, TW, TH, NI, EPI, KSP, NWV>), dim3(grid, ksplit), dim3(NWV * 64), 0, st, a);
  return rsis_check_launch();
}

template <int EPI>
static int pick_direct_variant(const ConvArgs& a, int force) {
  int v = force;
  if (v <= 0) {
    const bool small_co = a.Cout <= 32;
    if (a.W <= 8 && a.H <= 8) {
      const long b64 = (long)rsis_cdiv(a.Cout, 64) * a.B;
      const bool gsplit = EPI == EPI_PLAIN && a.ksplit == 0 && b64 < 160;
      v = (EPI != EPI_S2 && b64 < 1024 && !gsplit) ? 6 : 1;
    }
    else if (a.W <= 16) v = small_co ? 4 : 2;
    else v = small_co ? 5 : 3;
    if (v == 3) {
      const long blocks = (long)rsis_cdiv(a.Cout, 64) * rsis_cdiv(a.W, 32) * rsis_cdiv(a.H, 8) * a.B;
      if (blocks < 200) v = 2;
    }
    if (v == 2 || v == 3) {
      const int tw = v == 2 ? 16 : 32;
      const long blocks = (long)rsis_cdiv(a.Cout, 64) * rsis_cdiv(a.W, tw) * rsis_cdiv(a.H, 8) * a.B;
      if (blocks < 512) v = v == 2 ? 4 : 5;
    }
    if (v == 5 && a.W <= 32 && a.Cout > 32) v = 4;
    if (EPI != EPI_S2 && (v == 3 || v == 5) && a.W >= 64 && a.H >= 16 && a.Cout <= 64) v = 8;
  }
  if (EPI == EPI_S2 && v == 3) v = 5;
  if (EPI == EPI_S2 && v == 6) v = 1;
  return v;
}

template <int EPI>
static int launch_direct_epi(ConvArgs& a, hipStream_t st, int force) {
  const int v = pick_direct_variant<EPI>(a, force);
  switch (v) {
    case 1: return launch_direct_cfg<64, 8, 8, 1, EPI>(a, st);
    case 2: return launch_direct_cfg<64, 16, 8, 1, EPI>(a, st);
    case 3: if constexpr (EPI != EPI_S2) return launch_direct_cfg<64, 32, 8, 1, EPI>(a, st); else return RSIS_ERR_ARG;
    case 4: return launch_direct_cfg<32, 16, 8, 1, EPI>(a, st);
    case 5: return launch_direct_cfg<32, 32, 8, 1, EPI>(a, st);
    case 6: if constexpr (EPI != EPI_S2) return launch_direct_cfg<32, 8, 8, 1, EPI, 2>(a, st); else return RSIS_ERR_ARG;
    case 7: if constexpr (EPI != EPI_S2) return launch_direct_cfg<64, 32, 16, 1, EPI, 1, 8>(a, st); else return RSIS_ERR_ARG;
    case 8: if constexpr (EPI != EPI_S2) return launch_direct_cfg<32, 32, 16, 1, EPI, 1, 8>(a, st); else return RSIS_ERR_ARG;
    case 9: if constexpr (EPI != EPI_S2) return launch_direct_cfg<64, 16, 16, 1, EPI, 1, 8>(a, st); else return RSIS_ERR_ARG;
    default: return RSIS_ERR_ARG;
  }
}

static int launch_direct_f2(ConvArgs& a, hipStream_t st, int force) {
  int v = force;
  if (v != 1 && v != 4) v = (a.Wo <= 8 || (long)rsis_cdiv(a.Cout, 32) * rsis_cdiv(a.Wo, 16) * rsis_cdiv(a.Ho, 8) * a.B < 256) ? 1 : 4;
  if (v == 1) return launch_direct_cfg<64, 8, 8, 1, EPI_F2>(a, st);
  return launch_direct_cfg<32, 16, 8, 1, EPI_F2>(a, st);
}

int rsis_launch_conv3x3_direct(ConvArgs& a, int epi, int force_variant, hipStream_t st) {
  if (a.nsrc < 0 || a.nsrc > RSIS_MAX_SRC) return RSIS_ERR_ARG;
  if (epi == EPI_F2) return launch_direct_f2(a, st, force_variant);
  if (epi == EPI_LSTM) return launch_direct_epi<EPI_LSTM>(a, st, force_variant);
  if (epi == EPI_S2) return launch_direct_epi<EPI_S2>(a, st, force_variant);
  return launch_direct_epi<EPI_PLAIN>(a, st, force_variant);
}

template <int EPI>
static int launch_direct_group(ConvArgs* jobs, int n, const int* force_variant, hipStream_t st);
int rsis_launch_convlstm_direct_group(ConvArgs* jobs, int n, const int* force_variant, hipStream_t st) {
  return launch_direct_group<EPI_LSTM>(jobs, n, force_variant, st);
}
int rsis_launch_conv3x3_direct_group_plain(ConvArgs* jobs, int n, const int* force_variant, hipStream_t st) {
  return launch_direct_group<EPI_PLAIN>(jobs, n, force_variant, st);
}
template <int EPI>
static int launch_direct_group(ConvArgs* jobs, int n, const int* force_variant, hipStream_t st) {
  if (n < 1) return RSIS_OK;
  for (int j0 = 0; j0 < n; j0 += RSIS_DG_MAXJ) {
    const int m = n - j0 < RSIS_DG_MAXJ ? n - j0 : RSIS_DG_MAXJ;
    int order[RSIS_DG_MAXJ], var[RSIS_DG_MAXJ];
    long work[RSIS_DG_MAXJ];
    for (int j = 0; j < m; ++j) {
      ConvArgs& a = jobs[j0 + j];
      if (a.nsrc < 0 || a.nsrc > RSIS_MAX_SRC) return RSIS_ERR_ARG;
      int v = pick_direct_variant<EPI>(a, force_variant ? force_variant[j0 + j] : 0);
      if (v == 1) v = 6; else if (v == 2 || v == 9) v = 4; else if (v == 3 || v == 7 || v == 8) v = 5;
      var[j] = v;
      int nq = 0;
      for (int s = 0; s < a.nsrc; ++s) nq += (a.C[s] + RSIS_CK - 1) / RSIS_CK;
      work[j] = (long)nq * (v == 6 ? 64 : (v == 5 ? 256 : 128));
      order[j] = j;
    }
    for (int x = 1; x < m; ++x)
      for (int y = x; y > 0 && work[order[y]] > work[order[y - 1]]; --y) { const int t = order[y]; order[y] = order[y - 1]; order[y - 1] = t; }
    DirectGroup g;
    g.n = m;
    int blocks = 0;
    for (int k = 0; k < m; ++k) {
      const int j = order[k];
      ConvArgs a = jobs[j0 + j];
      const int v = var[j];
      const int bm = 32, tw = v == 6 ? 8 : (v == 5 ? 32 : 16);
      a.n_co_tiles = rsis_cdiv(a.Cout, bm);
      a.n_px_tiles = rsis_cdiv(a.W, tw) * rsis_cdiv(a.H, 8) * a.B;
      a.ksplit = 1;
      g.begin[k] = blocks;
      g.variant[k] = v;
      g.job[k] = a;
      blocks += a.n_co_tiles * 8 * rsis_cdiv(a.n_px_tiles, 8);
    }
    for (int k = m; k <= RSIS_DG_MAXJ; ++k) g.begin[k] = blocks;
    bool precise = false;
    for (int k = 0; k < m; ++k) precise = precise || g.job[k].precise != 0;
    if (EPI == EPI_LSTM && precise) hipLaunchKernelGGL((conv3x3_direct_group_kernel<EPI_LSTM, true>), dim3(blocks), dim3(256), 0, st, g);
    else hipLaunchKernelGGL((conv3x3_direct_group_kernel<EPI>), dim3(blocks), dim3(256), 0, st, g);
    if (rsis_check_launch() != RSIS_OK) return RSIS_ERR_LAUNCH;
  }
  return RSIS_OK;
}
```

### rsis_amd/csrc/pack.hip

```cpp
#include "blk_cell.h"
#include "../../include/rsis_hip.h"
#include "launchers.h"

struct SegMap { int n; int C[3]; int off[3]; };

__device__ __forceinline__ int seg_channel(const SegMap& m, int cg) {
  int base = 0;
#pragma unroll
  for (int s = 0; s < 3; ++s) {
    if (s < m.n) {
      if (cg < base + m.C[s]) return m.off[s] + (cg - base);
      base += m.C[s];
    }
  }
  return -1;
}
__device__ __forceinline__ int ref_row(int cop, int hid) { return hid > 0 ? (cop & 3) * hid + (cop >> 2) : cop; }

template <int KKC = 0>
__device__ __forceinline__ int pack_elem_idx(int mode, int row, int col, int Cout, int Ctot, int KKr, const SegMap& m, int hid) {
  const int KK = KKC ? KKC : KKr;
  if (mode == PACK_IGEMM_FWD) {
    if (col >= Cout) return -1;
    const int cg = row / KK, rs = row - cg * KK;
    const int ci = seg_channel(m, cg);
    return ci >= 0 ? (ref_row(col, hid) * Ctot + ci) * KK + rs : -1;
  }
  if (mode == PACK_IGEMM_DGRAD) {
    const int cop = row / KK, rs = row - cop * KK;
    const int ci = seg_channel(m, col);
    return (cop < Cout && ci >= 0) ? (ref_row(cop, hid) * Ctot + ci) * KK + rs : -1;
  }
  const int qg = row / (RSIS_CK * 9), kin = row - qg * (RSIS_CK * 9);
  const int pair = kin >> 1, h = kin & 1;
  const int cc = pair / 9, rs = pair - cc * 9;
  if (mode == PACK_DIRECT_FWD) {
    if (col >= Cout) return -1;
    int qs = 0, r = -1;
#pragma unroll
    for (int s = 0; s < 3; ++s) {
      if (s < m.n) {
        const int nq = (m.C[s] + RSIS_CK - 1) / RSIS_CK;
        if (qg >= qs && qg < qs + nq) {
          const int c = (qg - qs) * RSIS_CK + 2 * cc + h;
          if (c < m.C[s]) r = (ref_row(col, hid) * Ctot + m.off[s] + c) * 9 + rs;
        }
        qs += nq;
      }
    }
    return r;
  }
  const int c = qg * RSIS_CK + 2 * cc + h;
  const int ci = seg_channel(m, col);
  return (c < Cout && ci >= 0) ? (ref_row(c, hid) * Ctot + ci) * 9 + (mode == PACK_DIRECT_DGRAD ? 8 - rs : rs) : -1;
}
template <int KKC = 0>
__device__ __forceinline__ float pack_elem(int mode, const float* __restrict__ W, int row, int col, int Cout, int Ctot, int KKr,
                                           const SegMap& m, int hid) {
  const int i = pack_elem_idx<KKC>(mode, row, col, Cout, Ctot, KKr, m, hid);
  const float v = W[i < 0 ? 0 : i];
  return i < 0 ? 0.f : v;
}

__global__ void pack_kernel(int mode, const float* __restrict__ W, float* __restrict__ out, int Cout, int Ctot, int KK, SegMap m, int ldw,
                            int krows, int hid) {
  const long total = (long)krows * ldw;
  for (long e = blockIdx.x * (long)blockDim.x + threadIdx.x; e < total; e += (long)gridDim.x * blockDim.x) {
    const int row = (int)(e / ldw), col = (int)(e - (long)row * ldw);
    out[e] = pack_elem(mode, W, row, col, Cout, Ctot, KK, m, hid);
  }
}

__device__ __forceinline__ unsigned short to_bf16(float v) { return (unsigned short)(blk_pack2(v, 0.f) & 0xFFFFu); }

__device__ __forceinline__ int pack_bf16_idx(int mode, int kb, int col, int e, int Cout, int Ctot, int KK, const SegMap& m, int hid) {
  const int CKB = bf16_ckb(KK), NCB = CKB / 8;
  const int q = kb / (KK * NCB), rem = kb - q * (KK * NCB);
  const int rs = rem / NCB, cb = rem - rs * NCB;
  const int cl = cb * 8 + e;
  if (mode == PACK_BF16_FWD) {
    if (col >= Cout) return -1;
    int qs = 0, r = -1;
#pragma unroll
    for (int s = 0; s < 3; ++s) {
      if (s < m.n) {
        const int nq = (m.C[s] + CKB - 1) / CKB;
        if (q >= qs && q < qs + nq) {
          const int c = (q - qs) * CKB + cl;
          if (c < m.C[s]) r = (ref_row(col, hid) * Ctot + m.off[s] + c) * KK + rs;
        }
        qs += nq;
      }
    }
    return r;
  }
  const int c = q * CKB + cl;
  const int ci = seg_channel(m, col);
  return (c < Cout && ci >= 0) ? (ref_row(c, hid) * Ctot + ci) * KK + (KK == 9 ? 8 - rs : rs) : -1;
}
__device__ __forceinline__ float pack_bf16_src(int mode, const float* __restrict__ W, int kb, int col, int e, int Cout, int Ctot, int KK,
                                               const SegMap& m, int hid) {
  const int i = pack_bf16_idx(mode, kb, col, e, Cout, Ctot, KK, m, hid);
  const float v = W[i < 0 ? 0 : i];
  return i < 0 ? 0.f : v;
}

__global__ void pack_bf16_kernel(int mode, const float* __restrict__ W, unsigned short* __restrict__ out, int Cout, int Ctot, int KK,
                                 SegMap m, int ldw, int nkb, int hid) {
  const long total = (long)nkb * ldw * 8;
  for (long i = blockIdx.x * (long)blockDim.x + threadIdx.x; i < total; i += (long)gridDim.x * blockDim.x) {
    const int e = (int)(i & 7);
    const long cell = i >> 3;
    const int kb = (int)(cell / ldw), col = (int)(cell - (long)kb * ldw);
    out[i] = to_bf16(pack_bf16_src(mode, W, kb, col, e, Cout, Ctot, KK, m, hid));
  }
}

__device__ __forceinline__ void pack_tile_bf16(const rsis_pack_job& j, int tb, unsigned short* lds16) {
  SegMap m;
  m.n = j.nseg;
#pragma unroll
  for (int s = 0; s < 3; ++s) { m.C[s] = j.Cseg[s]; m.off[s] = j.Coff[s]; }
  const int KK = j.ks * j.ks, CKB = bf16_ckb(KK), NCB = CKB / 8;
  const int nct = j.ldw / 64;
  const int c0 = (tb % nct) * 64;
  unsigned short* out = (unsigned short*)j.out;
  if (j.imode == PACK_BF16_FWD) {
    const int R = KK * NCB;
    const int q = tb / nct;
    const int run = KK * CKB;
    for (int i0 = threadIdx.x; i0 < 64 * run; i0 += 256 * 4) {
      int src[4], dst[4];
#pragma unroll
      for (int u = 0; u < 4; ++u) {
        const int i = i0 + 256 * u;
        const int cl = i / run, idx = i - cl * run;
        const int ch = idx / KK, rs = idx - ch * KK;
        const int kb = q * R + rs * NCB + (ch >> 3);
        dst[u] = i < 64 * run ? ((rs * NCB + (ch >> 3)) * 64 + cl) * 8 + (ch & 7) : -1;
        src[u] = i < 64 * run ? pack_bf16_idx(PACK_BF16_FWD, kb, c0 + cl, ch & 7, j.Cout, j.Ctot, KK, m, j.lstm_hid) : -1;
      }
      float v[4];
#pragma unroll
      for (int u = 0; u < 4; ++u) v[u] = j.W[src[u] < 0 ? 0 : src[u]];
#pragma unroll
      for (int u = 0; u < 4; ++u)
        if (dst[u] >= 0) lds16[dst[u]] = to_bf16(src[u] < 0 ? 0.f : v[u]);
    }
    __syncthreads();
    const u32x4* src = (const u32x4*)lds16;
    for (int i = threadIdx.x; i < R * 64; i += 256) {
      const int rr = i >> 6, cl = i & 63;
      *(u32x4*)(out + ((long)(q * R + rr) * j.ldw + c0 + cl) * 8) = src[i];
    }
  } else {
    const int r0 = (tb / nct) * 16;
    for (int i = threadIdx.x; i < 16 * 64; i += 256) {
      const int rr = i >> 6, cl = i & 63;
      if (r0 + rr >= j.krows) continue;
      int src[8];
      float f[8];
#pragma unroll
      for (int e = 0; e < 8; ++e) src[e] = pack_bf16_idx(PACK_BF16_DGRAD, r0 + rr, c0 + cl, e, j.Cout, j.Ctot, KK, m, j.lstm_hid);
#pragma unroll
      for (int e = 0; e < 8; ++e) f[e] = j.W[src[e] < 0 ? 0 : src[e]];
      unsigned v[4];
#pragma unroll
      for (int e2 = 0; e2 < 4; ++e2) {
        const unsigned lo = to_bf16(src[2 * e2] < 0 ? 0.f : f[2 * e2]), hi = to_bf16(src[2 * e2 + 1] < 0 ? 0.f : f[2 * e2 + 1]);
        v[e2] = lo | (hi << 16);
      }
      const u32x4 cell = {v[0], v[1], v[2], v[3]};
      *(u32x4*)(out + ((long)(r0 + rr) * j.ldw + c0 + cl) * 8) = cell;
    }
  }
}

__device__ __forceinline__ void pack_tile_wino(int mode, const float* __restrict__ W, float* __restrict__ out, int Cout, int Ctot, int tb,
                                               const SegMap& m, int hid) {
  int csum = 0;
#pragma unroll
  for (int s_ = 0; s_ < 3; ++s_) csum += s_ < m.n ? m.C[s_] : 0;
  const int n_red = mode == PACK_WINO_FWD ? csum : Cout, nq = n_red >> 3;
  const int ot = tb / nq, q = tb - ot * nq;
  const int cl = threadIdx.x >> 5, col = threadIdx.x & 31;
  const int o = ot * 32 + col, rch = q * 8 + cl;
  const int cop = mode == PACK_WINO_FWD ? o : rch, cg = mode == PACK_WINO_FWD ? rch : o;
  const int ci = seg_channel(m, cg);
  const bool ok = ci >= 0 && cop < Cout;
  const float* g_ = W + ((size_t)ref_row(ok ? cop : 0, hid) * Ctot + (ok ? ci : 0)) * 9;
  float g[9];
#pragma unroll
  for (int k = 0; k < 9; ++k) g[k] = g_[mode == PACK_WINO_FWD ? k : 8 - k];
#pragma unroll
  for (int k = 0; k < 9; ++k) g[k] = ok ? g[k] : 0.f;
  float t[4][3];
#pragma unroll
  for (int s_ = 0; s_ < 3; ++s_) {
    t[0][s_] = g[s_];
    t[1][s_] = 0.5f * (g[s_] + g[3 + s_] + g[6 + s_]);
    t[2][s_] = 0.5f * (g[s_] - g[3 + s_] + g[6 + s_]);
    t[3][s_] = g[6 + s_];
  }
  float* o_ = out + ((size_t)tb * 16) * 256 + cl * 32 + col;
#pragma unroll
  for (int i = 0; i < 4; ++i) {
    o_[(4 * i + 0) * 256] = t[i][0];
    o_[(4 * i + 1) * 256] = 0.5f * (t[i][0] + t[i][1] + t[i][2]);
    o_[(4 * i + 2) * 256] = 0.5f * (t[i][0] - t[i][1] + t[i][2]);
    o_[(4 * i + 3) * 256] = t[i][2];
  }
}
__global__ __launch_bounds__(256) void pack_wino_kernel(int mode, const float* __restrict__ W, float* __restrict__ out, int Cout, int Ctot, SegMap m,
                                                        int hid) {
  pack_tile_wino(mode, W, out, Cout, Ctot, blockIdx.x, m, hid);
}

#define PACK_T 64
#define PACK_TC 64
template <int KKC>
__device__ __forceinline__ void pack_tile(const rsis_pack_job& j, int tb, float (*tile)[PACK_TC + 1]) {
  SegMap m;
  m.n = j.nseg;
#pragma unroll
  for (int s = 0; s < 3; ++s) { m.C[s] = j.Cseg[s]; m.off[s] = j.Coff[s]; }
  const int nct = j.ldw / PACK_TC;
  const int l = threadIdx.x & 63, q = threadIdx.x >> 6, KK = j.ks * j.ks;
  const int c0 = (tb % nct) * PACK_TC;
  int r0, nrow;
  if (j.imode >= PACK_DIRECT_DGRAD) {
    constexpr int R = RSIS_CK * 9;
    r0 = (tb / nct) * R;
    nrow = R;
    constexpr int PER = (PACK_TC * 9 + 255) / 256;
    for (int c = 0; c < RSIS_CK; c += 2) {
      int src[2 * PER], kin_[2 * PER], cl_[2 * PER];
#pragma unroll
      for (int u = 0; u < 2 * PER; ++u) {
        const int cu = c + u / PER, i = threadIdx.x + 256 * (u % PER);
        const int cl = i / 9, tap = i - cl * 9;
        const int rs = j.imode == PACK_DIRECT_DGRAD ? 8 - tap : tap;
        const int kin = ((cu >> 1) * 9 + rs) * 2 + (cu & 1);
        const bool ok = i < PACK_TC * 9;
        kin_[u] = ok ? kin : -1; cl_[u] = cl;
        src[u] = ok ? pack_elem_idx<KKC>(j.imode, r0 + kin, c0 + cl, j.Cout, j.Ctot, KK, m, j.lstm_hid) : -1;
      }
      float v[2 * PER];
#pragma unroll
      for (int u = 0; u < 2 * PER; ++u) v[u] = j.W[src[u] < 0 ? 0 : src[u]];
#pragma unroll
      for (int u = 0; u < 2 * PER; ++u)
        if (kin_[u] >= 0) tile[kin_[u]][cl_[u]] = src[u] < 0 ? 0.f : v[u];
    }
  } else {
    r0 = (tb / nct) * PACK_T;
    nrow = min(PACK_T, j.krows - r0);
    if (j.imode == PACK_IGEMM_DGRAD) {
      static_assert(PACK_TC == 64, "one column per lane");
      for (int rr0 = q; rr0 < nrow; rr0 += 16) {
        int src[4];
#pragma unroll
        for (int u = 0; u < 4; ++u) src[u] = rr0 + 4 * u < nrow ? pack_elem_idx<KKC>(PACK_IGEMM_DGRAD, r0 + rr0 + 4 * u, c0 + l, j.Cout, j.Ctot, KK, m, j.lstm_hid) : -1;
        float v[4];
#pragma unroll
        for (int u = 0; u < 4; ++u) v[u] = j.W[src[u] < 0 ? 0 : src[u]];
#pragma unroll
        for (int u = 0; u < 4; ++u)
          if (rr0 + 4 * u < nrow) tile[rr0 + 4 * u][l] = src[u] < 0 ? 0.f : v[u];
      }
    } else {
      const int lr = l < nrow ? l : 0;
      for (int k0 = 0; k0 < PACK_TC / 4; k0 += 4) {
        int src[4];
#pragma unroll
        for (int u = 0; u < 4; ++u) src[u] = l < nrow ? pack_elem_idx<KKC>(j.imode, r0 + lr, c0 + (k0 + u) * 4 + q, j.Cout, j.Ctot, KK, m, j.lstm_hid) : -1;
        float v[4];
#pragma unroll
        for (int u = 0; u < 4; ++u) v[u] = j.W[src[u] < 0 ? 0 : src[u]];
#pragma unroll
        for (int u = 0; u < 4; ++u)
          if (l < nrow) tile[l][(k0 + u) * 4 + q] = src[u] < 0 ? 0.f : v[u];
      }
    }
  }
  __syncthreads();
  for (int rr = q; rr < nrow; rr += 4) {
#pragma unroll
    for (int cc = l; cc < PACK_TC; cc += 64) ((float*)j.out)[(long)(r0 + rr) * j.ldw + c0 + cc] = tile[rr][cc];
  }
}

#define PACK_TPB 1
__global__ __launch_bounds__(256) void pack_batch_kernel(const rsis_pack_job* __restrict__ jobs, int njobs, int total_tiles) {
  __shared__ __attribute__((aligned(16))) float tile[RSIS_CK * 9][PACK_TC + 1];
  int lo = 0, hi = njobs - 1;
  int b = blockIdx.x * PACK_TPB;
  while (lo < hi) {
    const int mid = (lo + hi + 1) >> 1;
    if (jobs[mid].block_begin <= b) lo = mid; else hi = mid - 1;
  }
  rsis_pack_job j = jobs[lo];
  int next_begin = lo + 1 < njobs ? jobs[lo + 1].block_begin : total_tiles;
  for (int t = 0; t < PACK_TPB && b < total_tiles; ++t, ++b) {
    if (b >= next_begin) {
      ++lo;
      j = jobs[lo];
      next_begin = lo + 1 < njobs ? jobs[lo + 1].block_begin : total_tiles;
    }
    const int tb = b - j.block_begin;
    if (j.imode >= PACK_WINO_FWD) {
      SegMap wm;
      wm.n = j.nseg;
#pragma unroll
      for (int s_ = 0; s_ < 3; ++s_) { wm.C[s_] = j.Cseg[s_]; wm.off[s_] = j.Coff[s_]; }
      pack_tile_wino(j.imode, j.W, (float*)j.out, j.Cout, j.Ctot, tb, wm, j.lstm_hid);
    }
    else if (j.imode >= PACK_BF16_FWD) pack_tile_bf16(j, tb, (unsigned short*)&tile[0][0]);
    else if (j.ks == 1) pack_tile<1>(j, tb, tile);
    else if (j.ks == 3) pack_tile<9>(j, tb, tile);
    else pack_tile<0>(j, tb, tile);
    __syncthreads();
  }
}

int rsis_l_pack_batch(const rsis_pack_job* jobs, int njobs, int total_blocks, hipStream_t st) {
  hipLaunchKernelGGL(pack_batch_kernel, dim3((total_blocks + PACK_TPB - 1) / PACK_TPB), dim3(256), 0, st, jobs, njobs, total_blocks);
  return rsis_check_launch();
}
int rsis_l_pack_blocks(PackMode mode, int krows, int ldw, int ks) {
  if (mode >= PACK_WINO_FWD) return krows;
  if (mode == PACK_BF16_FWD) return krows / (ks * ks * (bf16_ckb(ks * ks) / 8)) * (ldw / 64);
  if (mode == PACK_BF16_DGRAD) return (krows + 15) / 16 * (ldw / 64);
  return (mode >= PACK_DIRECT_DGRAD ? krows / (RSIS_CK * 9) : (krows + PACK_T - 1) / PACK_T) * (ldw / PACK_TC);
}

static inline int pack_grid(long total) {
  long g = (total + 255) / 256;
  if (g > 4096) g = 4096;
  return (int)(g < 1 ? 1 : g);
}

int rsis_l_pack(PackMode mode, const float* W, void* out, int Cout, int Ctot, int ks, int nseg, const int* Cseg, const int* Coff,
                int ldw, int krows, int hid, hipStream_t st) {
  SegMap m = {};
  m.n = nseg;
  int base = 0;
  for (int s = 0; s < nseg; ++s) { m.C[s] = Cseg[s]; m.off[s] = Coff ? Coff[s] : base; base += Cseg[s]; }
  const long total = (long)krows * ldw;
  const dim3 g(pack_grid(total)), b(256);
  if (mode >= PACK_WINO_FWD) {
    hipLaunchKernelGGL(pack_wino_kernel, dim3(krows), b, 0, st, mode, W, (float*)out, Cout, Ctot, m, hid);
    return rsis_check_launch();
  }
  if (mode >= PACK_BF16_FWD) {
    hipLaunchKernelGGL(pack_bf16_kernel, dim3(pack_grid(total * 8)), b, 0, st, mode, W, (unsigned short*)out, Cout, Ctot, ks * ks, m, ldw,
                       krows, hid);
    return rsis_check_launch();
  }
  hipLaunchKernelGGL(pack_kernel, g, b, 0, st, mode, W, (float*)out, Cout, Ctot, ks * ks, m, ldw, krows, hid);
  return rsis_check_launch();
}
```

### rsis_amd/decoder_fused.py

```python
import os

import torch

from . import _lib, ops
from ._lib import check, int_array, lib, ptr, ptr_array, require_cuda_f32, stream

_GATE_QUEUE = [None]
WAVEFRONT = [os.environ.get("RSIS_DECODER_WAVEFRONT", "1") != "0"]
FUSED_POOL = [os.environ.get("RSIS_FUSED_POOL", "1") != "0"]
_BLK_WGRAD = [os.environ.get("RSIS_DECODER_BLK_WGRAD", "1") != "0"]


def _flush_gates():
    q, _GATE_QUEUE[0] = _GATE_QUEUE[0], None
    if not q:
        return
    jobs = (_lib.LstmJob * len(q))()
    for j, (f, _keep) in zip(jobs, q):
        srcs, segs, j.B, j.H, j.W, j.Wp, j.bias_packed, j.addend, j.c_prev, j.h_out, j.c_out, j.act_out, j.hid, j.ks, j.pad, j.tile, j.dtype, j.side_key = f
        j.nsrc = len(srcs)
        for k, (s, c) in enumerate(zip(srcs, segs)):
            j.src[k], j.Csrc[k] = s, c
    check(lib().rsis_convlstm_fwd_batch(jobs, len(q), stream()), "rsis_convlstm_fwd_batch")


class LevelTape(object):

    def __init__(self, cell, level, c_up, c_skip, cap):
        self.cell, self.level, self.c_up, self.c_skip, self.cap = cell, level, c_up, c_skip, cap
        self.hid = cell.hidden_size
        self.ks, self.pad = cell.kernel_size, cell.padding
        self.H = self.C = self.ACT = self.UP = self.DA = self.da_sum = None
        self.DHP, self.dhp_t = None, -1
        self.G = None
        self.n_fwd = 0
        self.n_bwd = 0
        self.last_h = self.last_c = None
        self.need_grad = False
        self.KEY = self.SIDE = self.ARG = None

    def pooled(self, t):
        return None if self.KEY is None else (self.SIDE[t], self.ARG[t])

    def release(self):
        self.H = self.C = self.ACT = self.UP = self.DA = self.da_sum = None
        self.DHP, self.dhp_t = None, -1
        self.G = self.last_h = self.last_c = None
        self.KEY = self.SIDE = self.ARG = None

    def alloc_forward(self, B, Hh, Ww, device, need_grad):
        hid, cap = self.hid, self.cap
        self.need_grad = need_grad
        if need_grad:
            self.H = torch.empty((cap, B, hid, Hh, Ww), dtype=torch.float32, device=device)
            self.C = torch.empty_like(self.H)
            self.ACT = torch.empty((cap, B, 4 * hid, Hh, Ww), dtype=torch.float32, device=device)
            if self.c_up > 0:
                self.UP = torch.empty((cap, B, self.c_up, Hh, Ww), dtype=torch.float32, device=device)


def _packs(cell, c_up, c_skip):
    key = ("fused", c_up, c_skip, getattr(cell, "dtype", ops.DTYPE_F32))
    if key not in cell._packs:
        hid, ks, pad = cell.hidden_size, cell.kernel_size, cell.padding
        skip_off = c_up
        h_off = c_up + c_skip
        dt = getattr(cell, "dtype", ops.DTYPE_F32)
        hoist = ops.PackedConv(ks, [c_skip], lstm_hid=hid, stride=1, pad=pad, offs=[skip_off], dtype=dt)
        segs, offs = ([c_up], [0]) if c_up > 0 else ([], [])
        dyn = ops.PackedConv(ks, segs + [hid], lstm_hid=hid, stride=1, pad=pad, offs=offs + [h_off], dtype=dt)
        cell._packs[key] = (hoist, dyn)
    return cell._packs[key]


def dyn_dgrad_pack(cell, c_up, c_skip, H, W):
    _hoist, dyn = _packs(cell, c_up, c_skip)
    hid = cell.hidden_size
    if (dyn.dtype != ops.DTYPE_F32 or not ops.WINOGRAD_GATES[0] or cell.kernel_size != 3 or cell.padding != 1 or min(H, W) < 12
            or (c_up + hid) % 32 or c_up % 32 or c_up == 0 or (4 * hid) % 32):
        return dyn
    key = ("fused-dgrad-wino", c_up, c_skip)
    if key not in cell._packs:
        cell._packs[key] = ops.PackedConv(3, list(dyn.segs), lstm_hid=hid, stride=1, pad=1, offs=list(dyn.offs), dtype=ops.DTYPE_F32_WINO)
    return cell._packs[key]


class _HoistFn(torch.autograd.Function):

    @staticmethod
    def forward(ctx, tl, skip, weight, bias):
        skip = skip if skip.is_contiguous() else skip.contiguous()
        require_cuda_f32(skip, weight, bias)
        L = lib()
        hoist, _dyn = _packs(tl.cell, tl.c_up, tl.c_skip)
        B, Cs, H, W = skip.shape
        wp = hoist.fwd(weight, bias)
        G = torch.empty((B, 4 * tl.hid, H, W), dtype=torch.float32, device=skip.device)
        check(L.rsis_conv2d_fwd(ptr_array([skip]), int_array([Cs]), 1, B, H, W, ptr(wp), 4 * tl.hid, tl.ks, 1, tl.pad,
                                ptr(hoist.bias_p), None, ptr(G), H, W, ops.FORCE_TILE[0], hoist.dtype, stream()), "rsis_conv2d_fwd(hoist)")
        ctx.tl = tl
        ctx.wparam, ctx.bparam = weight, bias
        ctx.save_for_backward(skip, weight)
        return G

    @staticmethod
    def backward(ctx, dG):
        tl = ctx.tl
        skip, weight = ctx.saved_tensors
        L = lib()
        dG = dG if dG.is_contiguous() else dG.contiguous()
        hoist, _dyn = _packs(tl.cell, tl.c_up, tl.c_skip)
        B, Cs, H, W = skip.shape
        dskip = dW = db = None
        if ctx.needs_input_grad[1]:
            wd = hoist.dgrad(weight)
            dskip = torch.empty_like(skip)
            check(L.rsis_conv2d_dgrad(ptr(dG), B, 4 * tl.hid, H, W, ptr(wd), hoist.cin, tl.ks, 1, tl.pad, ptr_array([dskip]),
                                      int_array([Cs]), 1, H, W, None, ops.FORCE_TILE[0], hoist.dtype, stream()), "rsis_conv2d_dgrad(hoist)")
        if ctx.needs_input_grad[2]:
            tgt = ops._direct_target(ctx.wparam)
            dW = tgt if tgt is not None else torch.zeros_like(weight)
            ops.wgrad_launch(L, dG, skip, dW, B, Cs, H, W, 4 * tl.hid, H, W, tl.ks, 1, tl.pad, weight.shape[1], tl.c_up, tl.hid,
                             hoist.dtype, "rsis_conv2d_wgrad(hoist)", tgt is not None)
            if tgt is not None:
                dW = None
        if ctx.needs_input_grad[3]:
            tgt = ops._direct_target(ctx.bparam)
            db = tgt if tgt is not None else torch.zeros(4 * tl.hid, dtype=torch.float32, device=dG.device)
            check(L.rsis_bias_grad(ptr(dG), ptr(db), B, 4 * tl.hid, H * W, tl.hid, stream()), "rsis_bias_grad(hoist)")
            if tgt is not None:
                db = None
        return None, dskip, dW, db


class _StepFn(torch.autograd.Function):

    @staticmethod
    def forward(ctx, tl, t, up, h_prev, c_prev, G, weight):
        require_cuda_f32(up, h_prev, c_prev, G, weight)
        L = lib()
        _hoist, dyn = _packs(tl.cell, tl.c_up, tl.c_skip)
        B, _, H, W = G.shape
        hid = tl.hid
        need_grad = any(ctx.needs_input_grad) and tl.need_grad
        stacked = need_grad and t < tl.cap
        srcs = []
        if up is not None:
            srcs.append(up if up.is_contiguous() else up.contiguous())
        if h_prev is not None:
            h_prev = h_prev if h_prev.is_contiguous() else h_prev.contiguous()
            c_prev = c_prev if c_prev.is_contiguous() else c_prev.contiguous()
            srcs.append(h_prev)
        if stacked:
            h, c, act = tl.H[t], tl.C[t], tl.ACT[t]
        else:
            h = torch.empty((B, hid, H, W), dtype=torch.float32, device=G.device)
            c = torch.empty_like(h)
            act = torch.empty((B, 4 * hid, H, W), dtype=torch.float32, device=G.device) if need_grad else None
        wp = dyn.fwd(weight)
        pa = ptr_array(srcs) if srcs else None
        ia = int_array([s.shape[1] for s in srcs]) if srcs else None
        if _GATE_QUEUE[0] is not None:
# ... 317 lines not shown
```

### rsis_amd/decoder_seq.py

```python
import os

import torch

from . import _lib, decoder_fused, dropout, ops
from ._lib import check, int_array, lib, ptr, ptr_array, stream

ENABLED = [os.environ.get("RSIS_DECODER_SEQ", "1") != "0"]
RECORD, LAST = [False], {}


def _is_blk(t):
    return t.dtype == torch.bfloat16 and t.dim() == 5 and t.shape[-1] == 8


def _chan(t):
    return t.shape[1] * 8 if _is_blk(t) else t.shape[1]


def supported(decoder, skip_feats, T):
    n = len(decoder.clstm_list)
    if not (ENABLED[0] and decoder_fused.WAVEFRONT[0] and decoder_fused.FUSED_POOL[0] and decoder.fused and decoder.skip_mode == "concat" and
            len(skip_feats) == n and T >= 1 and "forward" not in decoder.__dict__):
        return False
    if not all(0 <= p < 1 for p in dropout.rates(decoder)):
        return False
    if not all(f.is_cuda and ((f.dtype == torch.float32 and f.dim() == 4) or _is_blk(f)) for f in skip_feats):
        return False
    if any(_is_blk(f) for f in skip_feats) and not blk_supported(decoder, skip_feats):
        return False
    if not all(c.kernel_size == 3 and c.padding == 1 for c in decoder.clstm_list):
        return False
    if decoder.conv_out.kernel_size != 3 or decoder.conv_out.padding != 1 or decoder.conv_out.bias is None:
        return False
    hs = [c.hidden_size for c in decoder.clstm_list]
    if sum(hs) != decoder.fc_class.weight.shape[1] or not ops.heads_supported([skip_feats[0]] * n, decoder.fc_class, decoder.fc_stop, min_rows=1):
        return False
    for i, c in enumerate(decoder.clstm_list):
        c_up = 0 if i == 0 else hs[i - 1]
        if c.input_size != c_up + _chan(skip_feats[i]):
            return False
    return True


class ShapeProbe(object):

    def __init__(self, B, C, H, W, blk):
        self.is_cuda = True
        self.dtype = torch.bfloat16 if blk else torch.float32
        self.shape = (B, C // 8, H, W, 8) if blk else (B, C, H, W)

    def dim(self):
        return len(self.shape)


def supported_for_input(decoder, skip_channels, B, H, W, T):
    sizes, h, w = [], H, W
    for _ in range(5):
        h, w = (h + 1) // 2, (w + 1) // 2
        sizes.append((h, w))
    sizes = sizes[::-1]
    if any(c % 8 for c in skip_channels[:4]):
        return False
    probes = [ShapeProbe(B, c, hh, ww, i < 4) for i, (c, (hh, ww)) in enumerate(zip(skip_channels, sizes))]
    return supported(decoder, probes, T) and blk_supported(decoder, probes)


BLK_ENABLED = [os.environ.get("RSIS_DECODER_BLK", "1") != "0"]


def blk_supported(decoder, skip_feats):
    if not BLK_ENABLED[0]:
        return False
    hs = [c.hidden_size for c in decoder.clstm_list]
    if not all(getattr(c, "dtype", ops.DTYPE_F32) == ops.DTYPE_BF16 for c in decoder.clstm_list):
        return False
    if any(h % 8 for h in hs) or any(_chan(f) % 8 for f in skip_feats) or hs[-1] != 8:
        return False
    return (2 * skip_feats[-1].shape[3]) % 4 == 0


class _Level(object):
    __slots__ = ("cell", "hid", "c_up", "c_skip", "H", "W", "hoist", "dyn", "G", "Hs", "Cs", "ACT", "UP", "KEY", "SIDE", "ARG", "skip")


UPCONV = [os.environ.get("RSIS_UPCONV", "1") != "0"]


def _heads_bwd_all_steps(L, levels, hs, n, T, B, Wc, Ws, probs_tb, dp_tb, ds_tb, dsides, hb):
    def call(rows, sl, wide=False):
        return ops.heads_bwd_launch(L, [lv.SIDE[sl] for lv in levels], hs, rows, Wc, Ws, probs_tb[sl], dp_tb[sl] if dp_tb is not None else None,
                                    ds_tb[sl] if ds_tb is not None else None, [ds[sl] for ds in dsides], hb, wide)
    K, ncls = sum(hs), Wc.shape[0]
    if ops.heads_family(T * B, K, ncls, backward=True) == "small":
        check(call(T * B, slice(None)), "rsis_heads_bwd(all steps)")
    elif ops.heads_family(B, K, ncls, backward=True) == "small":
        for t in range(T):
            check(call(B, t), "rsis_heads_bwd")
    else:
        check(call(T * B, slice(None), True), "rsis_heads_wide_bwd(all steps)")


class _Side(object):
    __slots__ = ("SIDE",)

    def __init__(self, side):
        self.SIDE = side


class _Drop(object):
    __slots__ = ("S2", "MC", "MS", "s2", "SIDEC", "SIDES")


def _heads_fwd_masked(L, SIDE, drop, hs, T, B, Wc, bc, Ws, bs, probs_tb, stop_tb):
    check(L.rsis_dropout_heads_mask(ptr(SIDE), ptr(drop.S2), ptr(drop.MC), ptr(drop.MS), ptr(drop.SIDEC), ptr(drop.SIDES), SIDE.numel(), stream()),
          "rsis_dropout_heads_mask")
    ops.heads_fwd_launch(L, _per_level(drop.SIDEC, hs, T, B), hs, T * B, Wc, bc, Ws, bs, probs_tb, torch.empty_like(stop_tb))
    ops.heads_fwd_launch(L, _per_level(drop.SIDES, hs, T, B), hs, T * B, Wc, bc, Ws, bs, torch.empty_like(probs_tb), stop_tb)


def _heads_bwd_masked(L, drop, hs, T, B, Wc, Ws, probs_tb, dp_tb, ds_tb, DSIDE, hb):
    n = len(hs)
    dsc = dss = None
    if dp_tb is not None:
        dsc = torch.empty_like(DSIDE)
        _heads_bwd_all_steps(L, [_Side(v) for v in _per_level(drop.SIDEC, hs, T, B)], hs, n, T, B, Wc, Ws, probs_tb, dp_tb, None,
                             _per_level(dsc, hs, T, B), [hb[0], hb[1], None, None])
    if ds_tb is not None:
        dss = torch.empty_like(DSIDE)
        _heads_bwd_all_steps(L, [_Side(v) for v in _per_level(drop.SIDES, hs, T, B)], hs, n, T, B, Wc, Ws, probs_tb, None, ds_tb,
                             _per_level(dss, hs, T, B), [None, None, hb[2], hb[3]])
    check(L.rsis_dropout_heads_mask_bwd(ptr(dsc), ptr(dss), ptr(drop.MC), ptr(drop.MS), ptr(DSIDE), DSIDE.numel(), stream()),
          "rsis_dropout_heads_mask_bwd")


def _per_level(buf, hs, T, B):
    return [v.view(T, B, h) for v, h in zip(buf.split([T * B * h for h in hs]), hs)]


def _diagonal(d, n, T):
    return [(i, d - i) for i in range(n) if 0 <= d - i < T]


def _gate_srcs(lv, t):
    return ([lv.UP[t]] if lv.c_up > 0 else []) + ([lv.Hs[t - 1]] if t > 0 else [])


class _Layout(object):

    def __init__(self, L, T, B, dev):
        self.L, self.T, self.B, self.dev = L, T, B, dev


class _Nchw(_Layout):
    blk = 0
    by_level = True

    def empty(self, lead, C, H, W):
        return torch.empty(lead + (C, H, W), dtype=torch.float32, device=self.dev)

    def to_nchw(self, x):
        return x
    from_nchw = to_nchw

    def hoist(self, levels, feats, gates_w, gates_b, need_grad):
        _lib.require_cuda_f32(*feats)
        for lv, f, w, b in zip(levels, feats, gates_w, gates_b):
            lv.skip = f
            wp = lv.hoist.fwd(w, b)
            check(self.L.rsis_conv2d_fwd(ptr_array([f]), int_array([lv.c_skip]), 1, self.B, lv.H, lv.W, ptr(wp), 4 * lv.hid, 3, 1, 1,
                                         ptr(lv.hoist.bias_p), None, ptr(lv.G), lv.H, lv.W, ops.FORCE_TILE[0] + (100 if need_grad else 0),
                                         lv.hoist.dtype, stream()), "rsis_conv2d_fwd(hoist)")

    def gates(self, levels, cells, wps):
        jobs = (_lib.LstmJob * len(cells))()
        for j, (i, t) in zip(jobs, cells):
            lv = levels[i]
            srcs = _gate_srcs(lv, t)
            j.nsrc = len(srcs)
            for k, s in enumerate(srcs):
                j.src[k], j.Csrc[k] = s.data_ptr(), s.shape[1]
            (j.B, j.H, j.W, j.Wp, j.bias_packed, j.addend, j.c_prev, j.h_out, j.c_out, j.act_out, j.hid, j.ks, j.pad, j.tile, j.dtype,
             j.side_key) = (self.B, lv.H, lv.W, wps[i].data_ptr(), None, lv.G.data_ptr(), lv.Cs[t - 1].data_ptr() if t > 0 else None,
                            lv.Hs[t].data_ptr(), lv.Cs[t].data_ptr(), lv.ACT[t].data_ptr() if lv.ACT is not None else None, lv.hid, 3, 1,
                            ops.FORCE_TILE[0], lv.dyn.dtype, lv.KEY[t].data_ptr())
        check(self.L.rsis_convlstm_fwd_batch(jobs, len(cells), stream()), "rsis_convlstm_fwd_batch")

    def up(self, levels, cells, s2=None):
        for i, t in cells:
            if i + 1 < len(levels):
                lv, nx = levels[i], levels[i + 1]
                if s2 is not None:
                    check(self.L.rsis_upsample_bilinear_ac_scaled_fwd(ptr(lv.Hs[t]), ptr(s2[i][t]), ptr(nx.UP[t]), self.B * lv.hid, lv.H, lv.W, nx.H,
                                                                      nx.W, stream()), "rsis_upsample_scaled_fwd")
                elif (nx.H, nx.W) == (lv.H, lv.W):
                    nx.UP[t].copy_(lv.Hs[t])
                else:
                    check(self.L.rsis_upsample_bilinear_ac_fwd(ptr(lv.Hs[t]), ptr(nx.UP[t]), self.B * lv.hid, lv.H, lv.W, nx.H, nx.W, stream()),
                          "rsis_upsample_fwd")

    def tail(self, last, UP5, conv_out, co_w, co_b, out_masks, heads, sc=None):
        L, T, B = self.L, self.T, self.B
        H5, W5 = 2 * last.H, 2 * last.W
        if sc is not None:
            check(L.rsis_upsample_bilinear_ac_scaled_fwd(ptr(last.Hs), ptr(sc), ptr(UP5), T * B * last.hid, last.H, last.W, H5, W5, stream()),
                  "rsis_upsample_scaled_fwd(all steps)")
        else:
            check(L.rsis_upsample_bilinear_ac_fwd(ptr(last.Hs), ptr(UP5), T * B * last.hid, last.H, last.W, H5, W5, stream()), "rsis_upsample_fwd(all steps)")
        heads()
        co_pack = conv_out._pack
        co_wp = co_pack.fwd(co_w)
        self.seq_ok = last.hid in (4, 8, 16) and W5 % 4 == 0
        if self.seq_ok:
            check(L.rsis_conv_out_seq_fwd(ptr(UP5), ptr(co_wp), ptr(co_b.detach()), ptr(out_masks), T, B, last.hid, H5, W5, stream()),
                  "rsis_conv_out_seq_fwd")
        else:
            tmp = torch.empty((B, 1, H5, W5), dtype=torch.float32, device=self.dev)
            for t in range(T):
                check(L.rsis_conv2d_fwd(ptr_array([UP5[t]]), int_array([last.hid]), 1, B, H5, W5, ptr(co_wp), 1, 3, 1, 1, ptr(co_b.detach()), None,
                                        ptr(tmp), H5, W5, ops.FORCE_TILE[0], co_pack.dtype, stream()), "rsis_conv2d_fwd(conv_out)")
                out_masks[:, t].copy_(tmp.view(B, -1))

    def tail_bwd(self, d_masks, last, UP5, dUP5, conv_out, co_w, dW, db):
        L, T, B = self.L, self.T, self.B
        H5, W5 = 2 * last.H, 2 * last.W
        co_pack = conv_out._pack
        co_wd = co_pack.dgrad(co_w)
        dW = dW() if dW else None
        db = db() if db else None
        if self.seq_ok:
            check(L.rsis_conv_out_seq_dgrad(ptr(d_masks), ptr(co_wd), ptr(dUP5), T, B, last.hid, H5, W5, stream()), "rsis_conv_out_seq_dgrad")
            if dW is not None:
                check(L.rsis_conv_out_seq_wgrad(ptr(d_masks), ptr(UP5), ptr(dW), ptr(db), T, B, last.hid, H5, W5, stream()), "rsis_conv_out_seq_wgrad")
            elif db is not None:
                db += d_masks.sum()
            return
        for t in range(T):
            dy = d_masks[:, t].contiguous().view(B, 1, H5, W5)
            check(L.rsis_conv2d_dgrad(ptr(dy), B, 1, H5, W5, ptr(co_wd), co_pack.cin, 3, 1, 1, ptr_array([dUP5[t]]), int_array([last.hid]), 1,
                                      H5, W5, None, ops.FORCE_TILE[0], co_pack.dtype, stream()), "rsis_conv2d_dgrad(conv_out)")
            if dW is not None:
                check(L.rsis_conv2d_wgrad(ptr(dy), ptr(UP5[t]), ptr(dW), B, last.hid, H5, W5, 1, H5, W5, 3, 1, 1, last.hid, 0, 0, co_pack.dtype,
                                          stream()), "rsis_conv2d_wgrad(conv_out)")
            if db is not None:
                check(L.rsis_bias_grad(ptr(dy), ptr(db), B, 1, H5 * W5, 0, stream()), "rsis_bias_grad(conv_out)")

    def up5_bwd(self, dUP5, dside, last, DH_last, sc=None):
        if sc is not None:
            check(self.L.rsis_upsample_maxpool_scaled_bwd(ptr(dUP5), ptr(dside), ptr(last.ARG), ptr(sc), ptr(DH_last), self.T * self.B * last.hid,
                                                          last.H, last.W, 2 * last.H, 2 * last.W, stream()), "rsis_upsample_maxpool_scaled_bwd(all steps)")
            return
        check(self.L.rsis_upsample_maxpool_bwd(ptr(dUP5), ptr(dside), ptr(last.ARG), ptr(DH_last), self.T * self.B * last.hid, last.H, last.W,
                                               2 * last.H, 2 * last.W, stream()), "rsis_upsample_maxpool_bwd(all steps)")

    def up_bwd(self, levels, cells, DUP, DH, dsides, s2=None):
        B = self.B
        for i, t in cells:
            if i + 1 < len(levels):
                lv, nx = levels[i], levels[i + 1]
                if s2 is not None and (nx.H, nx.W) == (lv.H, lv.W):
                    check(self.L.rsis_scale_planes(ptr(DUP[i + 1]), ptr(s2[i][t]), ptr(DH[i]), B * lv.hid, lv.H * lv.W, stream()), "rsis_scale_planes")
                    check(self.L.rsis_global_maxpool_scaled_bwd_add(ptr(dsides[i][t]), ptr(lv.ARG[t]), ptr(s2[i][t]), ptr(DH[i]), B * lv.hid,
                                                                    lv.H * lv.W, stream()), "rsis_global_maxpool_scaled_bwd_add")
                elif s2 is not None:
                    check(self.L.rsis_upsample_maxpool_scaled_bwd(ptr(DUP[i + 1]), ptr(dsides[i][t]), ptr(lv.ARG[t]), ptr(s2[i][t]), ptr(DH[i]),
                                                                  B * lv.hid, lv.H, lv.W, nx.H, nx.W, stream()), "rsis_upsample_maxpool_scaled_bwd")
                elif (nx.H, nx.W) == (lv.H, lv.W):
                    DH[i].copy_(DUP[i + 1])
# ... 89 lines not shown
        if dW or db:
            dW = dW() if dW else torch.zeros_like(co_w)
            db = db() if db else None
            check(L.rsis_blk_conv_out_seq_wgrad(ptr(d_masks), ptr(UP5), ptr(dW), ptr(db), T, B, H5, W5, stream()), "rsis_blk_conv_out_seq_wgrad")

    def up5_bwd(self, dUP5, dside, last, DH_last, sc=None):
        ops.blk_upsample_bwd_batch([ops.blk_resize_job(dUP5.flatten(0, 1), DH_last.flatten(0, 1), dside, last.ARG, backward=True, scale=sc)])

    def up_bwd(self, levels, cells, DUP, DH, dsides, s2=None):
        ups = [ops.blk_resize_job(DUP[i + 1], DH[i], dsides[i][t], levels[i].ARG[t], backward=True, scale=s2[i][t] if s2 is not None else None)
               for i, t in cells if i + 1 < len(levels)]
        if ups:
            ops.blk_upsample_bwd_batch(ups)

    def lstm_bwd(self, jobs):
        ops.blk_lstm_bwd_batch([ops.blk_lstm_bwd_job(*job) for job in jobs])

    def dgrad(self, jobs):
        if jobs:
            ops.blk_conv3x3_batch([ops.blk_conv_job([dy], wd, sum(x.shape[1] for x in dxs) * 8, cpack=cin, dsts=dxs) for dy, wd, cin, _dt, dxs in jobs])

    def sum_t(self, DA, dG):
        check(self.L.rsis_blk_sum_leading(ptr(DA), ptr(dG), self.T, dG.numel() // 8, stream()), "rsis_blk_sum_leading")

    skip_dgrad = dgrad

    def bias_grad(self, dG, db, lv):
        check(self.L.rsis_blk_bias_grad(ptr(dG), ptr(db), self.B, 4 * lv.hid, lv.H * lv.W, lv.hid, stream()), "rsis_blk_bias_grad")

    def wgrad_formats(self, lv):
        return ops.DTYPE_BF16_BLK, ops.DTYPE_BF16_BLK, lambda x: x.flatten(0, 1)


class _DecoderSeqFn(torch.autograd.Function):

    @staticmethod
    def forward(ctx, layout, decoder, T, keep, want_hidden, *tensors):
        L = lib()
        n = len(decoder.clstm_list)
        feats = [t.contiguous() for t in tensors[:n]]
        params = tensors[n:]
        gates_w, gates_b = params[0:2 * n:2], params[1:2 * n:2]
        co_w, co_b, Wc, bc, Ws, bs = params[2 * n:2 * n + 6]
        _lib.require_cuda_f32(*params)
        need_grad = bool(keep) and any(ctx.needs_input_grad)
        dev = feats[0].device
        B = feats[0].shape[0]
        lay = layout(L, T, B, dev)
        hs = [c.hidden_size for c in decoder.clstm_list]
        tot = sum(hs)
        f32 = dict(dtype=torch.float32, device=dev)
        KEY = torch.zeros(T * B * tot, dtype=torch.int64, device=dev)
        SIDE = torch.empty(T * B * tot, **f32)
        ARG = torch.empty(T * B * tot, dtype=torch.int32, device=dev)
        levels = []
        for i, cell in enumerate(decoder.clstm_list):
            lv = _Level()
            lv.cell, lv.hid, lv.c_up, lv.c_skip = cell, hs[i], (0 if i == 0 else hs[i - 1]), _chan(feats[i])
            lv.H, lv.W = feats[i].shape[2], feats[i].shape[3]
            lv.hoist, lv.dyn = decoder_fused._packs(cell, lv.c_up, lv.c_skip)
            lv.G = lay.empty((B,), 4 * lv.hid, lv.H, lv.W)
            lv.Hs = lay.empty((T, B), lv.hid, lv.H, lv.W)
            lv.Cs = torch.empty((T, B, lv.hid, lv.H, lv.W), **f32)
            lv.ACT = lay.empty((T, B), 4 * lv.hid, lv.H, lv.W) if need_grad else None
            lv.UP = lay.empty((T, B), lv.c_up, lv.H, lv.W) if lv.c_up > 0 else None
            levels.append(lv)
        for lv, key, side, arg in zip(levels, _per_level(KEY, hs, T, B), _per_level(SIDE, hs, T, B), _per_level(ARG, hs, T, B)):
            lv.KEY, lv.SIDE, lv.ARG = key, side, arg
        drop = None
        p2, pc, ps = dropout.rates(decoder)
        if p2 > 0 or pc > 0 or ps > 0:
            drop = _Drop()
            drop.S2, drop.MC, drop.MS = dropout.draw(dropout.decoder_state(decoder, dev), T * B * tot, p2, pc, ps)
            drop.s2 = _per_level(drop.S2, hs, T, B) if p2 > 0 else None
            drop.SIDEC, drop.SIDES = torch.empty(T * B * tot, **f32), torch.empty(T * B * tot, **f32)
        s2 = drop.s2 if drop is not None else None
        lay.hoist(levels, feats, gates_w, gates_b, need_grad)
        last = levels[-1]
        H5, W5 = 2 * last.H, 2 * last.W
        upc = UPCONV[0] and s2 is None and L.rsis_upconv_out_supported(last.hid, last.H, last.W, H5, W5) == 1
        UP5 = None if upc else lay.empty((T, B), last.hid, H5, W5)
        probs_tb = torch.empty((T, B, Wc.shape[0]), **f32)
        stop_tb = torch.empty((T, B, 1), **f32)
        wps = [lv.dyn.fwd(w) for lv, w in zip(levels, gates_w)]
        for d in range(T + n - 1):
            cells = _diagonal(d, n, T)
            lay.gates(levels, cells, wps)
            if s2 is not None:
                lay.up(levels, cells, s2)
            else:
                lay.up(levels, cells)

        def heads():
            ops.heads_fwd_launch(L, [v.SIDE for v in levels], hs, T * B, Wc, bc, Ws, bs, probs_tb, stop_tb,
                                 ([v.KEY for v in levels], [v.ARG for v in levels]))
            if drop is not None:
                _heads_fwd_masked(L, SIDE, drop, hs, T, B, Wc, bc, Ws, bs, probs_tb, stop_tb)
        out_masks = torch.empty((B, T, H5 * W5), **f32)
        if upc:
            heads()
            check(L.rsis_upconv_out_fwd(ptr(last.Hs), lay.blk, ptr(co_w.detach()), ptr(co_b.detach()), ptr(out_masks), T, B, last.hid, last.H, last.W,
                                        H5, W5, stream()), "rsis_upconv_out_fwd")
        else:
            if s2 is not None:
                lay.tail(last, UP5, decoder.conv_out, co_w, co_b, out_masks, heads, s2[n - 1])
            else:
                lay.tail(last, UP5, decoder.conv_out, co_w, co_b, out_masks, heads)
        out_probs = probs_tb.transpose(0, 1).contiguous()
        out_stops = stop_tb.transpose(0, 1).contiguous()
        hidden = []
        if want_hidden:
            for lv in levels:
                hidden += [lay.to_nchw(lv.Hs[T - 1]), lv.Cs[T - 1]]
        if RECORD[0]:
            LAST["arg"] = [lv.ARG.clone() for lv in levels]
            if drop is not None:
                LAST["drop"] = {"s2": [v.clone() for v in s2] if s2 is not None else None, "mc": [v.clone() for v in _per_level(drop.MC, hs, T, B)],
                                "ms": [v.clone() for v in _per_level(drop.MS, hs, T, B)]}
        ctx.set_materialize_grads(False)
        if need_grad:
            ctx.lay, ctx.decoder, ctx.T, ctx.levels, ctx.upc = lay, decoder, T, levels, upc
            ctx.UP5, ctx.probs_tb, ctx.feats, ctx.params = UP5, probs_tb, feats, params
            ctx.drop = drop
        else:
            for lv in levels:
                lv.G = lv.ACT = lv.UP = lv.skip = None
        return (out_masks, out_probs, out_stops) + tuple(hidden)

    @staticmethod
    def backward(ctx, d_masks, d_probs, d_stops, *d_hidden):
        L = lib()
        lay, decoder, T, levels = ctx.lay, ctx.decoder, ctx.T, ctx.levels
        n = len(levels)
        feats, params = ctx.feats, ctx.params
        gates_w = params[0:2 * n:2]
        co_w, co_b, Wc, bc, Ws, bs = params[2 * n:2 * n + 6]
        need = ctx.needs_input_grad
        need_feat = [need[5 + i] for i in range(n)]
        need_par = [need[5 + n + k] for k in range(len(params))]
        dev = feats[0].device
        B = feats[0].shape[0]
        hs = [lv.hid for lv in levels]
        f32 = dict(dtype=torch.float32, device=dev)
        last = levels[-1]
        H5, W5 = 2 * last.H, 2 * last.W
        UP5 = ctx.UP5
        drop = ctx.drop
        s2 = drop.s2 if drop is not None else None
        grads_par = [None] * len(params)

        def target(k):
            p = params[k]
            t = ops._direct_target(p)
            if t is not None:
                return t, True
            g = torch.zeros_like(p)
            grads_par[k] = g
            return g, False

        upc = ctx.upc
        dUP5 = None if upc else torch.empty_like(UP5)
        kw, kb = 2 * n, 2 * n + 1
        have_masks = d_masks is not None
        if upc:
            d_masks = torch.zeros((B, T, H5 * W5), **f32) if d_masks is None else d_masks.contiguous()
        elif d_masks is None:
            dUP5.zero_()
        else:
            lay.tail_bwd(d_masks.contiguous(), last, UP5, dUP5, decoder.conv_out, co_w, (lambda: target(kw)[0]) if need_par[kw] else None,
                         (lambda: target(kb)[0]) if need_par[kb] else None)
        DSIDE = torch.empty(T * B * sum(hs), **f32)
        dsides = _per_level(DSIDE, hs, T, B)
        if d_probs is None and d_stops is None:
            DSIDE.zero_()
        else:
            dp_tb = d_probs.transpose(0, 1).contiguous() if d_probs is not None else None
            ds_tb = d_stops.transpose(0, 1).contiguous() if d_stops is not None else None
            hb = [target(2 * n + 2 + k)[0] if need_par[2 * n + 2 + k] else None for k in range(4)]
            if drop is None:
                _heads_bwd_all_steps(L, levels, hs, n, T, B, Wc, Ws, ctx.probs_tb, dp_tb, ds_tb, dsides, hb)
            else:
                _heads_bwd_masked(L, drop, hs, T, B, Wc, Ws, ctx.probs_tb, dp_tb, ds_tb, DSIDE, hb)
        DA = [torch.empty_like(lv.ACT) for lv in levels]
        DH = [lay.empty((B,), lv.hid, lv.H, lv.W) for lv in levels]
        DHP = [lay.empty((B,), lv.hid, lv.H, lv.W) for lv in levels]
        DC = [[torch.empty((B, lv.hid, lv.H, lv.W), **f32) for _ in range(2)] for lv in levels]
        DUP = [lay.empty((B,), lv.c_up, lv.H, lv.W) if lv.c_up > 0 else None for lv in levels]
        dpk = [decoder_fused.dyn_dgrad_pack(lv.cell, lv.c_up, lv.c_skip, lv.H, lv.W) for lv in levels]
        wds = [pk.dgrad(w) for pk, w in zip(dpk, gates_w)]
        d_hidden = d_hidden or (None,) * (2 * n)
        dhf = [lay.from_nchw(g.contiguous()) if g is not None else None for g in d_hidden[0::2]]
        dcf = [g.contiguous() if g is not None else None for g in d_hidden[1::2]]
        DH_last = lay.empty((T, B), last.hid, last.H, last.W)
        if upc:
            dW = target(kw)[0] if need_par[kw] and have_masks else None
            db = target(kb)[0] if need_par[kb] and have_masks else None
            partial = torch.empty(L.rsis_upconv_out_bwd_blocks(T, B, last.H, last.W) * 80, **f32)
            check(L.rsis_upconv_out_bwd(ptr(d_masks), ptr(last.Hs), lay.blk, ptr(co_w.detach()), ptr(DH_last), ptr(dW), ptr(db), ptr(dsides[n - 1]),
                                        ptr(last.ARG), ptr(partial), T, B, last.hid, last.H, last.W, H5, W5, stream()), "rsis_upconv_out_bwd")
        else:
            if s2 is not None:
                lay.up5_bwd(dUP5, dsides[n - 1], last, DH_last, s2[n - 1])
            else:
                lay.up5_bwd(dUP5, dsides[n - 1], last, DH_last)
        for d in range(T + n - 2, -1, -1):
            cells = _diagonal(d, n, T)
            if s2 is not None:
                lay.up_bwd(levels, cells, DUP, DH, dsides, s2)
            else:
                lay.up_bwd(levels, cells, DUP, DH, dsides)
            lstm, dg = [], []
            for i, t in cells:
                lv = levels[i]
                dh2, dcn = (dhf[i], dcf[i]) if t == T - 1 else (DHP[i], DC[i][(t + 1) & 1])
                lstm.append((DH[i] if i + 1 < n else DH_last[t], dh2, dcn, lv.ACT[t], lv.Cs[t - 1] if t > 0 else None, lv.Cs[t], DA[i][t],
                             DC[i][t & 1] if t > 0 else None))
                dxs = ([DUP[i]] if lv.c_up > 0 else []) + ([DHP[i]] if t > 0 else [])
                if dxs:
                    dg.append((DA[i][t], wds[i], lv.dyn.cin, dpk[i].dtype, dxs))
            lay.lstm_bwd(lstm)
            lay.dgrad(dg)
        dG, dskip, dfeats = [None] * n, [None] * n, [None] * n
        for grp in ([[i] for i in range(n)] if lay.by_level else [range(n)]):
            for i in grp:
                if T == 1:
                    dG[i] = DA[i][0]
                else:
                    dG[i] = torch.empty_like(levels[i].G)
                    lay.sum_t(DA[i], dG[i])
                if need_feat[i]:
                    dskip[i] = torch.empty_like(levels[i].skip)
            lay.skip_dgrad([(dG[i], levels[i].hoist.dgrad(gates_w[i]), levels[i].hoist.cin, levels[i].hoist.dtype, [dskip[i]]) for i in grp
                            if need_feat[i]])
            for i in grp:
                lv = levels[i]
                kw, kb = 2 * i, 2 * i + 1
                hid, H, W = lv.hid, lv.H, lv.W
                if need_feat[i]:
                    dfeats[i] = dskip[i] if _is_blk(feats[i]) else lay.to_nchw(dskip[i])
                if need_par[kb]:
                    lay.bias_grad(dG[i], target(kb)[0], lv)
                if need_par[kw]:
                    dW, direct = target(kw)
                    Ctot = gates_w[i].shape[1]
                    dt_skip, dt, rows = lay.wgrad_formats(lv)
                    ops.wgrad_launch(L, dG[i], lv.skip, dW, B, lv.c_skip, H, W, 4 * hid, H, W, 3, 1, 1, Ctot, lv.c_up, hid, dt_skip,
                                     "rsis_conv2d_wgrad(hoist)", direct)
                    da = rows(DA[i])
                    if lv.c_up > 0:
                        ops.wgrad_launch(L, da, rows(lv.UP), dW, T * B, lv.c_up, H, W, 4 * hid, H, W, 3, 1, 1, Ctot, 0, hid, dt,
                                         "rsis_conv2d_wgrad(batched up)", direct)
                    if T > 1:
                        ops.wgrad_launch(L, da[B:], rows(lv.Hs[:T - 1]), dW, (T - 1) * B, hid, H, W, 4 * hid, H, W, 3, 1, 1, Ctot, lv.c_up + lv.c_skip,
                                         hid, dt, "rsis_conv2d_wgrad(batched h)", direct)
        for lv in levels:
            lv.G = lv.Hs = lv.Cs = lv.ACT = lv.UP = lv.skip = None
        ctx.lay = ctx.levels = ctx.UP5 = ctx.feats = ctx.params = ctx.decoder = ctx.drop = None
        return (None, None, None, None, None) + tuple(dfeats) + tuple(grads_par)


def decoder_sequence_stacked(decoder, skip_feats, T, want_hidden=True):
    n = len(decoder.clstm_list)
    params = []
    for c in decoder.clstm_list:
        params += [c.Gates.weight, c.Gates.bias]
    params += [decoder.conv_out.weight, decoder.conv_out.bias, decoder.fc_class.weight, decoder.fc_class.bias, decoder.fc_stop.weight,
               decoder.fc_stop.bias]
    keep = torch.is_grad_enabled() and (any(f.requires_grad for f in skip_feats) or any(p.requires_grad for p in params))
    layout = _Blk if blk_supported(decoder, skip_feats) else _Nchw
    res = _DecoderSeqFn.apply(layout, decoder, int(T), keep, bool(want_hidden), *skip_feats, *params)
    out_masks, out_probs, out_stops = res[:3]
# ... 4 lines not shown
```

### rsis_amd/ops.py

```python
import ctypes
import os
import weakref

import torch

from . import _lib
from ._lib import check, int_array, lib, ptr, ptr_array, require_cuda_f32, stream

_WEIGHT_EPOCH = [0]


FORCE_TILE = [0]


DIRECT_GRAD = [False]


def _direct_target(param):
    g = param.grad if DIRECT_GRAD[0] and param is not None else None
    return g if (g is not None and g.is_contiguous() and g.dtype == torch.float32 and g.is_cuda) else None


DTYPE_F32, DTYPE_BF16 = 0, 1
DTYPE_F32_WINO = 3


def _wino_rule():
    v = os.environ.get("RSIS_WINOGRAD", "64,128,256").strip().lower()
    if v in ("0", "", "off", "none"):
        return None
    if v == "all":
        return "all"
    return {int(t) for t in v.split(",") if t.strip()}


WINOGRAD = [_wino_rule()]
TRAINING_FORWARD = [False]
WINOGRAD_INFER = [os.environ.get("RSIS_WINOGRAD_INFER", "0") == "1"]
WINOGRAD_GATES = [os.environ.get("RSIS_WINOGRAD_GATES", "1") != "0" and os.environ.get("RSIS_WINOGRAD", "x").strip().lower() not in ("0", "off", "none")]


def conv_dtype(dtype, ks, stride, pad, cin, cout):
    d = int(dtype)
    rule = WINOGRAD[0]
    if d != DTYPE_F32 or rule is None or not lib().rsis_conv_uses_wino(int(ks), int(stride), int(pad), int(cin), int(cout), 1, 0):
        return d
    return DTYPE_F32_WINO if (rule == "all" or (cin == cout and cin in rule)) else d

DTYPES = {"fp32": DTYPE_F32, "f32": DTYPE_F32, "float32": DTYPE_F32, "bf16": DTYPE_BF16, "bfloat16": DTYPE_BF16}


def set_dtype(module, dtype):
    d = DTYPES[dtype] if isinstance(dtype, str) else int(dtype)
    for m in module.modules():
        if hasattr(m, "_set_rsis_dtype"):
            m._set_rsis_dtype(d)
    return module


def set_deterministic(on=True):
    return bool(lib().rsis_set_deterministic(1 if on else 0))


def is_deterministic():
    return bool(lib().rsis_get_deterministic())


SUBSAMPLE_1X1 = [os.environ.get("RSIS_SUBSAMPLE_1X1", "1") != "0"]
_PACKS = weakref.WeakSet()
_BATCH = {"sig": None, "jobs": None, "n": 0, "blocks": 0}


def repack_all():
    L = lib()
    todo = []
    for p in list(_PACKS):
        w = p._refs[0]() if p._refs is not None else None
        if w is None or not w.is_cuda:
            continue
        b = p._refs[1]() if p._refs[1] is not None else None
        if p.wp is not None and p._key_f is not None:
            todo.append((p, w, b, p.wp, 0))
        if p.wd is not None and p._key_d is not None:
            todo.append((p, w, b, p.wd, 1))
    if not todo:
        return
    sig = tuple((id(p), w.data_ptr(), out.data_ptr(), d) for p, w, _b, out, d in todo)
    if _BATCH["sig"] != sig:
        jobs = (_lib.PackJob * len(todo))()
        blocks = 0
        for i, (p, w, _b, out, d) in enumerate(todo):
            jobs[i] = p._job(w, out, d)
            nb = L.rsis_conv_pack_job_fill(ctypes.byref(jobs[i]))
            if nb < 0:
                raise _lib.RsisHipError("rsis_conv_pack_job_fill rejected a pack job")
            jobs[i].block_begin = blocks
            blocks += nb
        raw = torch.frombuffer(bytearray(bytes(jobs)), dtype=torch.uint8).to(todo[0][1].device)
        _BATCH.update(sig=sig, jobs=raw, n=len(todo), blocks=blocks)
    check(L.rsis_conv_pack_batch(ptr(_BATCH["jobs"]), _BATCH["n"], _BATCH["blocks"], stream()), "rsis_conv_pack_batch")
    for p, w, b, _out, d in todo:
        if d == 0:
            p._key_f = p._key(w) + ((b._version, b.data_ptr()) if b is not None else ())
            if b is not None and p.lstm_hid > 0:
                p._pack_bias(b)
        else:
            p._key_d = p._key(w)


def bump_weight_epoch():
    _WEIGHT_EPOCH[0] += 1


class PackedConv(object):

    def __init__(self, ks, segs, lstm_hid=0, stride=1, pad=None, offs=None, dtype=DTYPE_F32):
        self.dtype = int(dtype)
        if int(lstm_hid) > 0 and int(ks) != 3:
            self.dtype = DTYPE_F32
        self.ks = int(ks)
        self.stride = int(stride)
        self.pad = int(ks // 2 if pad is None else pad)
        self.segs = [int(s) for s in segs]
        self.offs = [int(o) for o in offs] if offs is not None else None
        self.cin = sum(self.segs)
        self.lstm_hid = int(lstm_hid)
        self._key_f = None
        self._key_d = None
        self.training_call = False
        self._twin = None
        self.wp = None
        self.wd = None
        self.bias_p = None
        self._refs = None

    def _key(self, w):
        return (_WEIGHT_EPOCH[0], w._version, w.data_ptr(), self.dtype)

    def direct_twin(self):
        if self._twin is None:
            self._twin = PackedConv(self.ks, self.segs, lstm_hid=self.lstm_hid, stride=self.stride, pad=self.pad, offs=self.offs, dtype=DTYPE_F32)
        return self._twin

    def _pack_bias(self, bias):
        n = 4 * self.lstm_hid
        if self.bias_p is None or self.bias_p.numel() != n or self.bias_p.device != bias.device:
            self.bias_p = torch.empty(n, dtype=torch.float32, device=bias.device)
        self.bias_p.view(self.lstm_hid, 4).copy_(bias.detach().view(4, self.lstm_hid).t())

    def _job(self, w, out, dgrad):
        j = _lib.PackJob()
        j.W, j.out, j.dgrad, j.dtype = w.data_ptr(), out.data_ptr(), int(dgrad), self.dtype
        j.Cout, j.Ctot, j.ks, j.stride, j.pad = w.shape[0], w.shape[1], self.ks, self.stride, self.pad
        j.nseg, j.lstm_hid = len(self.segs), self.lstm_hid
        off = 0
        for i, c in enumerate(self.segs):
            j.Cseg[i] = c
            j.Coff[i] = self.offs[i] if self.offs is not None else off
            off += c
        return j

    def _seg_args(self):
        return len(self.segs), int_array(self.segs), (int_array(self.offs) if self.offs is not None else None)

    def fwd(self, w, bias=None):
        key = self._key(w) + ((bias._version, bias.data_ptr()) if bias is not None else ())
        if self._key_f != key:
            L = lib()
            Cout, Ctot = w.shape[0], w.shape[1]
            nseg, segs, offs = self._seg_args()
            n = L.rsis_conv_packed_bytes_fwd(self.dtype, Cout, self.ks, self.stride, self.pad, nseg, segs) // 4
            if self.wp is None or self.wp.numel() != n:
                self.wp = torch.zeros(n, dtype=torch.float32, device=w.device)
            check(L.rsis_conv_pack_fwd(ptr(w.detach()), ptr(self.wp), Cout, Ctot, self.ks, self.stride, self.pad, nseg, segs, offs,
                                       self.lstm_hid, self.dtype, stream()), "rsis_conv_pack_fwd")
            if bias is not None and self.lstm_hid > 0:
                self._pack_bias(bias)
            self._key_f = key
            self._refs = (weakref.ref(w), weakref.ref(bias) if bias is not None else None)
            _PACKS.add(self)
        return self.wp

    def dgrad(self, w):
        key = self._key(w)
        if self._key_d != key:
            L = lib()
            Cout, Ctot = w.shape[0], w.shape[1]
            nseg, segs, offs = self._seg_args()
            n = L.rsis_conv_packed_bytes_dgrad(self.dtype, Cout, self.ks, self.stride, self.pad, self.cin) // 4
            if self.wd is None or self.wd.numel() != n:
                self.wd = torch.zeros(n, dtype=torch.float32, device=w.device)
            check(L.rsis_conv_pack_dgrad(ptr(w.detach()), ptr(self.wd), Cout, Ctot, self.ks, self.stride, self.pad, nseg, segs, offs,
                                         self.lstm_hid, self.dtype, stream()), "rsis_conv_pack_dgrad")
            self._key_d = key
            if self._refs is None:
                self._refs = (weakref.ref(w), None)
            _PACKS.add(self)
        return self.wd


def _contig(t):
    return t if t.is_contiguous() else t.contiguous()


def _conv_out_size(n, ks, stride, pad):
    return (n + 2 * pad - ks) // stride + 1


def _dgrad_all(L, dy, wd, cin_packed, ks, stride, pad, srcs, Hx, Wx, addend=None, inplace=False, dtype=DTYPE_F32):
    B, Cout, Hy, Wy = dy.shape
    shapes = [tuple(s.shape) if torch.is_tensor(s) else tuple(s) for s in srcs]
    dxs = [addend] if inplace else [torch.empty(sh, dtype=torch.float32, device=dy.device) for sh in shapes]
    check(L.rsis_conv2d_dgrad(ptr(dy), B, Cout, Hy, Wy, ptr(wd), cin_packed, ks, stride, pad, ptr_array(dxs),
                              int_array([sh[1] for sh in shapes]), len(shapes), Hx, Wx, ptr(addend), FORCE_TILE[0], dtype, stream()),
          "rsis_conv2d_dgrad")
    return dxs


class GradSlot(object):

    def __init__(self):
        self.grad = None
        self.done = False

    def reset(self):
        self.grad, self.done = None, False

    def take(self):
        g, self.grad = self.grad, None
        self.done = True
        return g

    def park(self, g):
        if self.done or self.grad is not None or g is None:
            return False
        self.grad = g
        return True


class _GradTapFn(torch.autograd.Function):
    @staticmethod
    def forward(ctx, x, slot):
        ctx.slot = slot
# ... 852 lines not shown
```

Before: 963.1.

## Add bf16 three-limb split-precision path for decoder ConvLSTM gate convolutions

Adds a new F32_LIMB dtype that splits f32 weights and activations into three bf16 limbs and runs the 3x3 gate convolutions of the decoder ConvLSTM on bf16 matrix instructions, so the result stays close to f32. It covers forward and grouped dgrad, with new packing, new kernels and routing through the grouped direct launcher, and it is on by default for several decoder levels during training. The aim is to replace f32 FMA work with faster bf16 MFMA throughput. The cost is three times the packed weight memory, extra conversion work and possibly more LDS per block.

New measurement: 990.8 (median of 6 runs). 2.9% higher.

```diff
diff --git a/include/rsis_hip.h b/include/rsis_hip.h
--- a/include/rsis_hip.h
+++ b/include/rsis_hip.h
@@ -11,6 +11,7 @@
 #define RSIS_DTYPE_BF16 1
 #define RSIS_DTYPE_BF16_BLK 2
 #define RSIS_DTYPE_F32_WINO 3
+#define RSIS_DTYPE_F32_LIMB 4
 
 int rsis_version(void);
 const char* rsis_error_string(int code);
diff --git a/rsis_amd/csrc/api.hip b/rsis_amd/csrc/api.hip
--- a/rsis_amd/csrc/api.hip
+++ b/rsis_amd/csrc/api.hip
@@ -33,6 +33,13 @@
 static inline bool use_wino(int dtype, int ks, int stride, int pad, int Cin, int Cout, int nseg, int lstm_hid) {
   return dtype == RSIS_DTYPE_F32_WINO && wino_geom(ks, stride, pad, Cin, Cout, nseg, lstm_hid);
 }
+static inline bool limb_geom(int ks, int stride, int pad, int Cout, int nseg, const int* Cseg) {
+  if (!(ks == 3 && stride == 1 && pad == 1 && Cout > 1)) return false;
+  for (int s = 0; s < nseg; ++s)
+    if (Cseg[s] % 8 != 0) return false;
+  return true;
+}
+static inline bool limb_geom_dgrad(int ks, int stride, int pad, int Cout) { return ks == 3 && stride == 1 && pad == 1 && Cout > 1 && Cout % 8 == 0; }
 static inline int bf16_rows(int ks, int nseg, const int* Cseg) {
   const int ckb = bf16_ckb(ks * ks);
   return seg_chunks(nseg, Cseg, ckb) * ks * ks * (ckb / 8);
@@ -100,7 +107,11 @@
     return p;
   }
   long cell = 4;
-  if (use_bf16(dtype, ks, stride, pad, Cout)) {
+  if (dtype == RSIS_DTYPE_F32_LIMB && (dgrad ? limb_geom_dgrad(ks, stride, pad, Cout) : limb_geom(ks, stride, pad, Cout, nseg, Cseg))) {
+    p.mode = dgrad ? PACK_LIMB_DGRAD : PACK_LIMB_FWD;
+    p.krows = 3 * (dgrad ? bf16_rows(ks, 1, &Cout) : bf16_rows(ks, nseg, Cseg));
+    cell = 16;
+  } else if (use_bf16(dtype, ks, stride, pad, Cout)) {
     p.mode = dgrad ? PACK_BF16_DGRAD : PACK_BF16_FWD;
     p.krows = dgrad ? bf16_rows(ks, 1, &Cout) : bf16_rows(ks, nseg, Cseg);
     cell = 16;
@@ -278,6 +289,11 @@
   }
   if (use_wino(dtype, ks, stride, pad, Csrc[0], Cout, nsrc, 0))
     return rsis_launch_conv_wino(src[0], Wp, bias, addend, out, B, Csrc[0], Cout, H, W, (hipStream_t)stream, a.precise);
+  if (dtype == RSIS_DTYPE_F32_LIMB && limb_geom(ks, stride, pad, Cout, nsrc, Csrc)) {
+    if (!allow_splitk) return RSIS_ERR_UNSUPPORTED;
+    a.limb = 1;
+    return rsis_launch_conv3x3_direct(a, 0, direct_variant(tile), (hipStream_t)stream);
+  }
   if (use_bf16(dtype, ks, stride, pad, Cout)) {
     if (stride != 1) return RSIS_ERR_UNSUPPORTED;
     if (ks == 1 && nsrc != 1) return RSIS_ERR_UNSUPPORTED;
@@ -347,6 +363,11 @@
     const int b1[1] = {B}, c1[1] = {Cout}, co1[1] = {ctot}, c01[1] = {Cdx[0]}, h1[1] = {Hy}, w1[1] = {Wy};
     return rsis_launch_conv_wino_group(1, xs, us, y0, y1, b1, c1, co1, c01, h1, w1, (hipStream_t)stream);
   }
+  if (dtype == RSIS_DTYPE_F32_LIMB && limb_geom_dgrad(ks, stride, pad, Cout)) {
+    if (Hx != Hy || Wx != Wy) return RSIS_ERR_ARG;
+    a.limb = 1;
+    return rsis_launch_conv3x3_direct(a, 0, direct_variant(tile), (hipStream_t)stream);
+  }
   if (use_bf16(dtype, ks, stride, pad, Cout)) {
     if (ks == 3) {
       if (Hx != Hy || Wx != Wy) return RSIS_ERR_ARG;
@@ -474,6 +495,10 @@
   route = use_bf16(dtype, ks, 1, pad, 4 * hid) ? 0 : (use_direct(ks, 1, pad) ? 1 : 2);
   a.side_key = side_key;
   a.precise = act_out ? 0 : 1;
+  if (dtype == RSIS_DTYPE_F32_LIMB && limb_geom(ks, 1, pad, 4 * hid, nsrc, Csrc)) {
+    if (!act_out) return RSIS_ERR_UNSUPPORTED;
+    a.limb = 1;
+  }
   if (side_key && (route == 2 || (long)H * W >= 0x7FFFFFFFL)) return RSIS_ERR_UNSUPPORTED;
   return RSIS_OK;
 }
@@ -1093,7 +1118,8 @@
       if (++nw == 4) { rc = rsis_launch_conv_wino_group(nw, wx, wu, wy0, wy1, wb, wc, wco, wc0, wh, ww, (hipStream_t)stream); nw = 0; }
       continue;
     }
-    const bool groupable = q.dtype == RSIS_DTYPE_F32 && use_direct(q.ks, q.stride, q.pad) && !q.addend && q.Hx == q.Hy && q.Wx == q.Wy &&
+    const bool limb = q.dtype == RSIS_DTYPE_F32_LIMB && limb_geom_dgrad(q.ks, q.stride, q.pad, q.Cout);
+    const bool groupable = (q.dtype == RSIS_DTYPE_F32 || limb) && use_direct(q.ks, q.stride, q.pad) && !q.addend && q.Hx == q.Hy && q.Wx == q.Wy &&
                            !(q.Cout == 1) && ctot <= q.Cin_packed && (size_t)q.B * (ctot > q.Cout ? ctot : q.Cout) * q.Hy * q.Wy * 4 < (1ull << 31) &&
                            !rsis_deterministic();
     if (!groupable) {
@@ -1103,6 +1129,7 @@
     }
     rc = dgrad_fill(grp[ng], q.dy, q.B, q.Cout, q.Hy, q.Wy, q.Wd, q.Cin_packed, q.ks, q.stride, q.pad, q.dx, q.Cdx, q.ndst, q.Hx, q.Wx, q.addend);
     if (rc) break;
+    grp[ng].limb = limb ? 1 : 0;
     force[ng++] = direct_variant(q.tile);
   }
   if (rc == RSIS_OK && nw > 0) rc = rsis_launch_conv_wino_group(nw, wx, wu, wy0, wy1, wb, wc, wco, wc0, wh, ww, (hipStream_t)stream);
diff --git a/rsis_amd/csrc/common.h b/rsis_amd/csrc/common.h
--- a/rsis_amd/csrc/common.h
+++ b/rsis_amd/csrc/common.h
@@ -23,7 +23,9 @@
   PACK_BF16_FWD = 5,
   PACK_BF16_DGRAD = 6,
   PACK_WINO_FWD = 7,
-  PACK_WINO_DGRAD = 8
+  PACK_WINO_DGRAD = 8,
+  PACK_LIMB_FWD = 9,
+  PACK_LIMB_DGRAD = 10
 };
 __host__ __device__ __forceinline__ int bf16_ckb(int KK) { return KK == 1 ? RSIS_CKB1 : RSIS_CKB3; }
 
@@ -100,6 +102,7 @@
   float* act_out;
   unsigned long long* side_key;
   int precise;
+  int limb;
 };
 
 __device__ __forceinline__ unsigned long long rsis_side_key(float v, int idx) {
diff --git a/rsis_amd/csrc/conv3x3_direct.hip b/rsis_amd/csrc/conv3x3_direct.hip
--- a/rsis_amd/csrc/conv3x3_direct.hip
+++ b/rsis_amd/csrc/conv3x3_direct.hip
@@ -1,12 +1,12 @@
 #include "common.h"
 #include "launchers.h"
+#include "conv3x3_limb.h"
 #include <stdlib.h>
 #ifndef XCD_CHUNKED
 #define XCD_CHUNKED 1
 #endif
 
 enum { EPI_PLAIN = 0, EPI_LSTM = 1, EPI_S2 = 2, EPI_F2 = 3 };
-typedef __attribute__((address_space(3))) void* lds_vp_t;
 #define CK RSIS_CK
 #ifndef RSIS_ACC_FLUSH
 #define RSIS_ACC_FLUSH 4
@@ -25,7 +25,7 @@
   return 2 * ((XS + NT - 1) / NT * NT + WS);
 }
 
-template <int BM, int TW, int TH, int NI, int EPI, int KSP = 1, int NWV = 4, bool FLUSH = false, bool BNE = false>
+template <int BM, int TW, int TH, int NI, int EPI, int KSP = 1, int NWV = 4, bool FLUSH = false, bool BNE = false, bool LIMB = false>
 __device__ __forceinline__ void conv3x3_direct_body(const ConvArgs& p, const int bid, const int kz, const int ksplit, float* const lds) {
 #if __HIP_DEVICE_COMPILE__
   constexpr int BN = TW * TH * NI;
@@ -44,6 +44,7 @@
   static_assert(TN >= 1 && BN % (WGN * 32) == 0 && WGM * WGN * KSP == NWV && (CK / 2) % KSP == 0 && (KSP == 1 || EPI != EPI_S2), "tile");
 
   static_assert(2 * (XSP + WS) == direct_lds_floats<BM, TW, TH, NI, EPI, NWV>(), "LDS size helper out of sync");
+  static_assert(!LIMB || (KSP == 1 && NWV == 4 && NI == 1 && !FLUSH && !BNE && (EPI == EPI_PLAIN || EPI == EPI_LSTM)), "limb flavour: 256 threads, plain / LSTM");
   float* const Xs0 = lds;
   float* const Ws0 = lds + 2 * XSP;
 
@@ -113,6 +114,9 @@
       for (int r = 0; r < 16; ++r) accs[c][j][r] = 0.f;
   f32x16 (&acc)[TN] = accs[0];
 
+  if constexpr (LIMB) {
+    rsis_limb_mainloop<BM, TW, TH, TN>(p, b0, x0, y0, co_t, wm, wn, lds, acc);
+  } else {
   const gcf_t wbase = (gcf_t)p.wp + co_t * BM;
 
   int cs = 0, cq = q_begin;
@@ -192,6 +196,7 @@
     for (int j = 0; j < TN; ++j)
 #pragma unroll
       for (int r = 0; r < 16; ++r) acc[j][r] += tot[j][r];
+  }
   }
 
   if constexpr (BNE) {
@@ -402,6 +407,12 @@
   conv3x3_direct_body<BM, TW, TH, NI, EPI, KSP, NWV, FLUSH, BNE>(p, blockIdx.x, blockIdx.y, gridDim.y, lds);
 }
 
+template <int BM, int TW, int TH, int EPI>
+__global__ __launch_bounds__(256) void conv3x3_limb_kernel(const ConvArgs p) {
+  __shared__ __attribute__((aligned(16))) float lds[limb_lds_floats<BM, TW, TH>()];
+  conv3x3_direct_body<BM, TW, TH, 1, EPI, 1, 4, false, false, true>(p, blockIdx.x, 0, 1, lds);
+}
+
 #define RSIS_DG_MAXJ 8
 constexpr int cmax(int a, int b) { return a > b ? a : b; }
 struct DirectGroup {
@@ -412,11 +423,14 @@
 };
 static_assert(sizeof(DirectGroup) <= 4000, "kernel arguments are limited to 4 KB");
 
-template <int EPI, bool FLUSH = false>
-__global__ __launch_bounds__(256) void conv3x3_direct_group_kernel(const DirectGroup g) {
-  constexpr int LMAX = cmax(cmax(direct_lds_floats<32, 16, 8, 1, EPI, 4>(), direct_lds_floats<32, 32, 8, 1, EPI, 4>()),
+template <int EPI, bool LIMB>
+constexpr int group_lds_floats() {
+  constexpr int LF32 = cmax(cmax(direct_lds_floats<32, 16, 8, 1, EPI, 4>(), direct_lds_floats<32, 32, 8, 1, EPI, 4>()),
                             direct_lds_floats<32, 8, 8, 1, EPI, 4>());
-  __shared__ __attribute__((aligned(16))) float lds[LMAX];
+  return LIMB ? cmax(LF32, cmax(limb_lds_floats<32, 16, 8>(), limb_lds_floats<32, 32, 8>())) : LF32;
+}
+template <int EPI, bool FLUSH, bool LIMB>
+__device__ __forceinline__ void direct_group_program(const DirectGroup& g, float* const lds) {
   const int b = blockIdx.x;
   int j = 0;
 #pragma unroll
@@ -426,8 +440,20 @@
   switch (g.variant[j]) {
     case 4: conv3x3_direct_body<32, 16, 8, 1, EPI, 1, 4, FLUSH>(p, local, 0, 1, lds); break;
     case 5: conv3x3_direct_body<32, 32, 8, 1, EPI, 1, 4, FLUSH>(p, local, 0, 1, lds); break;
+    case 14: if constexpr (LIMB) { conv3x3_direct_body<32, 16, 8, 1, EPI, 1, 4, false, false, true>(p, local, 0, 1, lds); } break;
+    case 15: if constexpr (LIMB) { conv3x3_direct_body<32, 32, 8, 1, EPI, 1, 4, false, false, true>(p, local, 0, 1, lds); } break;
     default: conv3x3_direct_body<32, 8, 8, 1, EPI, 2, 4, FLUSH>(p, local, 0, 1, lds); break;
   }
+}
+template <int EPI, bool FLUSH = false>
+__global__ __launch_bounds__(256) void conv3x3_direct_group_kernel(const DirectGroup g) {
+  __shared__ __attribute__((aligned(16))) float lds[group_lds_floats<EPI, false>()];
+  direct_group_program<EPI, FLUSH, false>(g, lds);
+}
+template <int EPI>
+__global__ __launch_bounds__(256) void conv3x3_limb_group_kernel(const DirectGroup g) {
+  __shared__ __attribute__((aligned(16))) float lds[group_lds_floats<EPI, true>()];
+  direct_group_program<EPI, false, true>(g, lds);
 }
 
 template <int BM, int TW, int TH, int NI, int EPI, int KSP = 1, int NWV = 4>
@@ -522,8 +548,30 @@
   return launch_direct_cfg<32, 16, 8, 1, EPI_F2>(a, st);
 }
 
+static int pick_limb_variant(const ConvArgs& a, int force) {
+  if (force == 4 || force == 5) return force;
+  if (force == 3 || force == 7 || force == 8) return 5;
+  if (force > 0) return 4;
+  return a.W <= 16 ? 4 : 5;
+}
+template <int BM, int TW, int TH, int EPI>
+static int launch_limb_cfg(ConvArgs& a, hipStream_t st) {
+  a.n_co_tiles = rsis_cdiv(a.Cout, BM);
+  a.n_px_tiles = rsis_cdiv(a.W, TW) * rsis_cdiv(a.H, TH) * a.B;
+  a.ksplit = 1;
+  hipLaunchKernelGGL((conv3x3_limb_kernel<BM, TW, TH, EPI>), dim3(a.n_co_tiles * 8 * rsis_cdiv(a.n_px_tiles, 8)), dim3(256), 0, st, a);
+  return rsis_check_launch();
+}
+static int launch_limb(ConvArgs& a, int epi, int force, hipStream_t st) {
+  if (epi != EPI_PLAIN && epi != EPI_LSTM) return RSIS_ERR_UNSUPPORTED;
+  const int v = pick_limb_variant(a, force);
+  if (epi == EPI_LSTM) return v == 4 ? launch_limb_cfg<32, 16, 8, EPI_LSTM>(a, st) : launch_limb_cfg<32, 32, 8, EPI_LSTM>(a, st);
+  return v == 4 ? launch_limb_cfg<32, 16, 8, EPI_PLAIN>(a, st) : launch_limb_cfg<32, 32, 8, EPI_PLAIN>(a, st);
+}
+
 int rsis_launch_conv3x3_direct(ConvArgs& a, int epi, int force_variant, hipStream_t st) {
   if (a.nsrc < 0 || a.nsrc > RSIS_MAX_SRC) return RSIS_ERR_ARG;
+  if (a.limb) return launch_limb(a, epi, force_variant, st);
   if (epi == EPI_F2) return launch_direct_f2(a, st, force_variant);
   if (epi == EPI_LSTM) return launch_direct_epi<EPI_LSTM>(a, st, force_variant);
   if (epi == EPI_S2) return launch_direct_epi<EPI_S2>(a, st, force_variant);
@@ -550,10 +598,11 @@
       if (a.nsrc < 0 || a.nsrc > RSIS_MAX_SRC) return RSIS_ERR_ARG;
       int v = pick_direct_variant<EPI>(a, force_variant ? force_variant[j0 + j] : 0);
       if (v == 1) v = 6; else if (v == 2 || v == 9) v = 4; else if (v == 3 || v == 7 || v == 8) v = 5;
+      if (a.limb) v = 10 + pick_limb_variant(a, force_variant ? force_variant[j0 + j] : 0);
       var[j] = v;
       int nq = 0;
       for (int s = 0; s < a.nsrc; ++s) nq += (a.C[s] + RSIS_CK - 1) / RSIS_CK;
-      work[j] = (long)nq * (v == 6 ? 64 : (v == 5 ? 256 : 128));
+      work[j] = (long)nq * (v == 6 ? 64 : (v % 10 == 5 ? 256 : 128));
       order[j] = j;
     }
     for (int x = 1; x < m; ++x)
@@ -565,7 +614,7 @@
       const int j = order[k];
       ConvArgs a = jobs[j0 + j];
       const int v = var[j];
-      const int bm = 32, tw = v == 6 ? 8 : (v == 5 ? 32 : 16);
+      const int bm = 32, tw = v == 6 ? 8 : (v % 10 == 5 ? 32 : 16);
       a.n_co_tiles = rsis_cdiv(a.Cout, bm);
       a.n_px_tiles = rsis_cdiv(a.W, tw) * rsis_cdiv(a.H, 8) * a.B;
       a.ksplit = 1;
@@ -575,9 +624,11 @@
       blocks += a.n_co_tiles * 8 * rsis_cdiv(a.n_px_tiles, 8);
     }
     for (int k = m; k <= RSIS_DG_MAXJ; ++k) g.begin[k] = blocks;
-    bool precise = false;
-    for (int k = 0; k < m; ++k) precise = precise || g.job[k].precise != 0;
-    if (EPI == EPI_LSTM && precise) hipLaunchKernelGGL((conv3x3_direct_group_kernel<EPI_LSTM, true>), dim3(blocks), dim3(256), 0, st, g);
+    bool precise = false, limb = false;
+    for (int k = 0; k < m; ++k) { precise = precise || g.job[k].precise != 0; limb = limb || g.job[k].limb != 0; }
+    if (limb && precise) return RSIS_ERR_UNSUPPORTED;
+    if (limb) hipLaunchKernelGGL((conv3x3_limb_group_kernel<EPI>), dim3(blocks), dim3(256), 0, st, g);
+    else if (EPI == EPI_LSTM && precise) hipLaunchKernelGGL((conv3x3_direct_group_kernel<EPI_LSTM, true>), dim3(blocks), dim3(256), 0, st, g);
     else hipLaunchKernelGGL((conv3x3_direct_group_kernel<EPI>), dim3(blocks), dim3(256), 0, st, g);
     if (rsis_check_launch() != RSIS_OK) return RSIS_ERR_LAUNCH;
   }
diff --git a/rsis_amd/csrc/conv3x3_limb.h b/rsis_amd/csrc/conv3x3_limb.h
--- /dev/null
+++ b/rsis_amd/csrc/conv3x3_limb.h
@@ -0,0 +1,131 @@
+#pragma once
+#include "blk_cell.h"
+#include "limb_split.h"
+
+#define RSIS_CKL 16
+#define RSIS_LIMB_ROWS 54
+
+template <int BM, int TW, int TH>
+constexpr int limb_lds_floats() {
+  return 3 * (2 * (TW + 2) * (TH + 2) + 9 * 2 * BM) * 4;
+}
+
+template <int BM, int TW, int TH, int TN>
+__device__ __forceinline__ void rsis_limb_mainloop(const ConvArgs& p, const int b0, const int x0, const int y0, const int co_t, const int wm, const int wn,
+                                                   float* const lds, f32x16 (&acc)[TN]) {
+#if __HIP_DEVICE_COMPILE__
+  typedef const float __attribute__((address_space(1)))* gcf_t;
+  constexpr int NCB = RSIS_CKL / 8;
+  constexpr int PW = TW + 2, PH = TH + 2, IMS = PH * PW;
+  constexpr int XC1 = NCB * IMS, XC = 3 * XC1;
+  constexpr int WC1 = 9 * NCB * BM, WC = 3 * WC1;
+  constexpr int NXT = (XC1 + 255) / 256, NWT = (WC + 255) / 256;
+  static_assert(4 * (XC + WC) == limb_lds_floats<BM, TW, TH>(), "LDS size helper out of sync");
+  u32x4* const Xs = reinterpret_cast<u32x4*>(lds);
+  u32x4* const Ws = Xs + XC;
+
+  const gcf_t src0 = (gcf_t)p.src[0], src1 = (gcf_t)p.src[1], src2 = (gcf_t)p.src[2];
+  const int C0 = p.C[0], C1 = p.C[1], C2 = p.C[2];
+  const int q0 = (C0 + RSIS_CKL - 1) / RSIS_CKL, q1 = (C1 + RSIS_CKL - 1) / RSIS_CKL, q2 = (C2 + RSIS_CKL - 1) / RSIS_CKL;
+  const int nq = q0 + q1 + q2;
+  const int H = p.H, W = p.W, HW = H * W, ldw = p.ldw;
+  const int tid = threadIdx.x;
+  const int lane = tid & 63, l31 = lane & 31, hi = lane >> 5;
+
+  unsigned xvo[NXT];
+#pragma unroll
+  for (int i = 0; i < NXT; ++i) {
+    const int e = tid + i * 256;
+    const int cb = e / IMS, rem = e - cb * IMS;
+    const int py = rem / PW, pxx = rem - py * PW;
+    const int gy = y0 + py - 1, gx = x0 + pxx - 1;
+    const bool ok = (e < XC1) && ((unsigned)gy < (unsigned)H) && ((unsigned)gx < (unsigned)W);
+    xvo[i] = ok ? (unsigned)(cb * 8 * HW + gy * W + gx) * 4u : RSIS_OOB;
+  }
+  unsigned wvo[NWT];
+#pragma unroll
+  for (int i = 0; i < NWT; ++i) {
+    const int idx = tid + i * 256;
+    wvo[i] = idx < WC ? (unsigned)((idx / BM) * ldw + idx % BM) * 16u : RSIS_OOB;
+  }
+  const unsigned chs = (unsigned)HW * 4u;
+
+  int xoff[TN];
+#pragma unroll
+  for (int j = 0; j < TN; ++j) xoff[j] = blk_xoff<TN, TW, PW, IMS>(wn, j, l31, hi);
+  const int woff = hi * BM + wm * 32 + l31;
+  const char* const wbase = (const char*)p.wp + (size_t)co_t * BM * 16;
+
+  int cs = 0, cq = 0;
+  if (q0 == 0) { cs = 1; if (q1 == 0) cs = 2; }
+  float rx[NXT][8];
+  u32x4 rw[NWT];
+#define LIMB_ISSUE(QG)                                                                                             \
+  {                                                                                                                \
+    gcf_t src = src0; int Cs = C0;                                                                                 \
+    if (cs == 1) { src = src1; Cs = C1; }                                                                          \
+    if (cs == 2) { src = src2; Cs = C2; }                                                                          \
+    const int c0 = cq * RSIS_CKL;                                                                                  \
+    const int cn = min(RSIS_CKL, Cs - c0);                                                                         \
+    const float* xb = (const float*)src + ((size_t)b0 * Cs + c0) * HW;                                             \
+    const __amdgpu_buffer_rsrc_t rx_ = __builtin_amdgcn_make_buffer_rsrc((void*)xb, 0, cn * HW * 4, 0x00020000);   \
+    _Pragma("unroll") for (int i = 0; i < NXT; ++i)                                                                \
+      _Pragma("unroll") for (int c = 0; c < 8; ++c)                                                                \
+        rx[i][c] = __builtin_bit_cast(float, __builtin_amdgcn_raw_buffer_load_b32(rx_, xvo[i] + c * chs, 0, 0));   \
+    const char* wrow = wbase + (size_t)(QG) * RSIS_LIMB_ROWS * ldw * 16;                                           \
+    const __amdgpu_buffer_rsrc_t rw_ = __builtin_amdgcn_make_buffer_rsrc((void*)wrow, 0, RSIS_LIMB_ROWS * ldw * 16, 0x00020000); \
+    _Pragma("unroll") for (int i = 0; i < NWT; ++i) rw[i] = __builtin_amdgcn_raw_buffer_load_b128(rw_, wvo[i], 0, 0); \
+    if (++cq == (cs == 0 ? q0 : (cs == 1 ? q1 : q2))) { cq = 0; ++cs; if (cs == 1 && q1 == 0) ++cs; }             \
+  }
+#define LIMB_STORE()                                                                                               \
+  {                                                                                                                \
+    _Pragma("unroll") for (int i = 0; i < NXT; ++i) {                                                              \
+      const int e = tid + i * 256;                                                                                 \
+      if (XC1 % 256 == 0 || e < XC1) {                                                                             \
+        unsigned c0_[4], c1_[4], c2_[4];                                                                           \
+        rsis_limb_pack8_cells(rx[i], c0_, c1_, c2_);                                                               \
+        const u32x4 v0 = {c0_[0], c0_[1], c0_[2], c0_[3]}, v1 = {c1_[0], c1_[1], c1_[2], c1_[3]}, v2 = {c2_[0], c2_[1], c2_[2], c2_[3]}; \
+        Xs[e] = v0; Xs[XC1 + e] = v1; Xs[2 * XC1 + e] = v2;                                                        \
+      }                                                                                                            \
+    }                                                                                                              \
+    _Pragma("unroll") for (int i = 0; i < NWT; ++i) {                                                              \
+      const int idx = tid + i * 256;                                                                               \
+      if (WC % 256 == 0 || idx < WC) Ws[idx] = rw[i];                                                              \
+    }                                                                                                              \
+  }
+  if (nq > 0) {
+    LIMB_ISSUE(0)
+    LIMB_STORE()
+  }
+  __syncthreads();
+  for (int t = 0; t < nq; ++t) {
+    const bool more = t + 1 < nq;
+    if (more) LIMB_ISSUE(t + 1)
+#pragma unroll
+    for (int r = 0; r < 3; ++r)
+#pragma unroll
+      for (int s = 0; s < 3; ++s) {
+        const u32x4* Xt = Xs + r * PW + s;
+        const u32x4* Wt = Ws + woff + ((r * 3 + s) * NCB) * BM;
+        bf16x8 a[3], b[3][TN];
+#pragma unroll
+        for (int l = 0; l < 3; ++l) {
+          a[l] = __builtin_bit_cast(bf16x8, Wt[l * WC1]);
+#pragma unroll
+          for (int j = 0; j < TN; ++j) b[l][j] = __builtin_bit_cast(bf16x8, Xt[l * XC1 + xoff[j]]);
+        }
+#pragma unroll
+        for (int q = 0; q < RSIS_LIMB_PRODUCTS; ++q)
+#pragma unroll
+          for (int j = 0; j < TN; ++j) acc[j] = __builtin_amdgcn_mfma_f32_32x32x16_bf16(a[RSIS_LIMB_PA(q)], b[RSIS_LIMB_PB(q)][j], acc[j], 0, 0, 0);
+      }
+    __syncthreads();
+    if (more) {
+      LIMB_STORE()
+      __syncthreads();
+    }
+  }
+#undef LIMB_ISSUE
+#undef LIMB_STORE
+#endif
+}
diff --git a/rsis_amd/csrc/pack.hip b/rsis_amd/csrc/pack.hip
--- a/rsis_amd/csrc/pack.hip
+++ b/rsis_amd/csrc/pack.hip
@@ -1,4 +1,5 @@
 #include "blk_cell.h"
+#include "limb_split.h"
 #include "../../include/rsis_hip.h"
 #include "launchers.h"
 
@@ -72,6 +73,13 @@
 }
 
 __device__ __forceinline__ unsigned short to_bf16(float v) { return (unsigned short)(blk_pack2(v, 0.f) & 0xFFFFu); }
+__device__ __forceinline__ unsigned short pack_cvt(float v, int limb) {
+  if (limb < 0) return to_bf16(v);
+  float l0, l1, l2;
+  rsis_limb_split3(v, l0, l1, l2);
+  return (unsigned short)(__float_as_uint(limb == 0 ? l0 : (limb == 1 ? l1 : l2)) >> 16);
+}
+__device__ __forceinline__ int pack_limb_row(int kb, int limb) { return limb < 0 ? kb : ((kb / 18) * 3 + limb) * 18 + kb % 18; }
 
 __device__ __forceinline__ int pack_bf16_idx(int mode, int kb, int col, int e, int Cout, int Ctot, int KK, const SegMap& m, int hid) {
   const int CKB = bf16_ckb(KK), NCB = CKB / 8;
@@ -106,17 +114,17 @@
 }
 
 __global__ void pack_bf16_kernel(int mode, const float* __restrict__ W, unsigned short* __restrict__ out, int Cout, int Ctot, int KK,
-                                 SegMap m, int ldw, int nkb, int hid) {
+                                 SegMap m, int ldw, int nkb, int hid, int limb) {
   const long total = (long)nkb * ldw * 8;
   for (long i = blockIdx.x * (long)blockDim.x + threadIdx.x; i < total; i += (long)gridDim.x * blockDim.x) {
     const int e = (int)(i & 7);
     const long cell = i >> 3;
     const int kb = (int)(cell / ldw), col = (int)(cell - (long)kb * ldw);
-    out[i] = to_bf16(pack_bf16_src(mode, W, kb, col, e, Cout, Ctot, KK, m, hid));
-  }
-}
-
-__device__ __forceinline__ void pack_tile_bf16(const rsis_pack_job& j, int tb, unsigned short* lds16) {
+    out[((long)pack_limb_row(kb, limb) * ldw + col) * 8 + e] = pack_cvt(pack_bf16_src(mode, W, kb, col, e, Cout, Ctot, KK, m, hid), limb);
+  }
+}
+
+__device__ __forceinline__ void pack_tile_bf16(const rsis_pack_job& j, int tb, unsigned short* lds16, const int limb = -1) {
   SegMap m;
   m.n = j.nseg;
 #pragma unroll
@@ -125,7 +133,8 @@
   const int nct = j.ldw / 64;
   const int c0 = (tb % nct) * 64;
   unsigned short* out = (unsigned short*)j.out;
-  if (j.imode == PACK_BF16_FWD) {
+  const int nkb = limb < 0 ? j.krows : j.krows / 3;
+  if (j.imode == PACK_BF16_FWD || j.imode == PACK_LIMB_FWD) {
     const int R = KK * NCB;
     const int q = tb / nct;
     const int run = KK * CKB;
@@ -145,19 +154,19 @@
       for (int u = 0; u < 4; ++u) v[u] = j.W[src[u] < 0 ? 0 : src[u]];
 #pragma unroll
       for (int u = 0; u < 4; ++u)
-        if (dst[u] >= 0) lds16[dst[u]] = to_bf16(src[u] < 0 ? 0.f : v[u]);
+        if (dst[u] >= 0) lds16[dst[u]] = pack_cvt(src[u] < 0 ? 0.f : v[u], limb);
     }
     __syncthreads();
     const u32x4* src = (const u32x4*)lds16;
     for (int i = threadIdx.x; i < R * 64; i += 256) {
       const int rr = i >> 6, cl = i & 63;
-      *(u32x4*)(out + ((long)(q * R + rr) * j.ldw + c0 + cl) * 8) = src[i];
+      *(u32x4*)(out + ((long)pack_limb_row(q * R + rr, limb) * j.ldw + c0 + cl) * 8) = src[i];
     }
   } else {
     const int r0 = (tb / nct) * 16;
     for (int i = threadIdx.x; i < 16 * 64; i += 256) {
       const int rr = i >> 6, cl = i & 63;
-      if (r0 + rr >= j.krows) continue;
+      if (r0 + rr >= nkb) continue;
       int src[8];
       float f[8];
 #pragma unroll
@@ -167,11 +176,11 @@
       unsigned v[4];
 #pragma unroll
       for (int e2 = 0; e2 < 4; ++e2) {
-        const unsigned lo = to_bf16(src[2 * e2] < 0 ? 0.f : f[2 * e2]), hi = to_bf16(src[2 * e2 + 1] < 0 ? 0.f : f[2 * e2 + 1]);
+        const unsigned lo = pack_cvt(src[2 * e2] < 0 ? 0.f : f[2 * e2], limb), hi = pack_cvt(src[2 * e2 + 1] < 0 ? 0.f : f[2 * e2 + 1], limb);
         v[e2] = lo | (hi << 16);
       }
       const u32x4 cell = {v[0], v[1], v[2], v[3]};
-      *(u32x4*)(out + ((long)(r0 + rr) * j.ldw + c0 + cl) * 8) = cell;
+      *(u32x4*)(out + ((long)pack_limb_row(r0 + rr, limb) * j.ldw + c0 + cl) * 8) = cell;
     }
   }
 }
@@ -308,7 +317,13 @@
       next_begin = lo + 1 < njobs ? jobs[lo + 1].block_begin : total_tiles;
     }
     const int tb = b - j.block_begin;
-    if (j.imode >= PACK_WINO_FWD) {
+    if (j.imode >= PACK_LIMB_FWD) {
+      for (int l = 0; l < 3; ++l) {
+        pack_tile_bf16(j, tb, (unsigned short*)&tile[0][0], l);
+        if (l < 2) __syncthreads();
+      }
+    }
+    else if (j.imode >= PACK_WINO_FWD) {
       SegMap wm;
       wm.n = j.nseg;
 #pragma unroll
@@ -328,6 +343,8 @@
   return rsis_check_launch();
 }
 int rsis_l_pack_blocks(PackMode mode, int krows, int ldw, int ks) {
+  if (mode == PACK_LIMB_FWD) return rsis_l_pack_blocks(PACK_BF16_FWD, krows / 3, ldw, ks);
+  if (mode == PACK_LIMB_DGRAD) return rsis_l_pack_blocks(PACK_BF16_DGRAD, krows / 3, ldw, ks);
   if (mode >= PACK_WINO_FWD) return krows;
   if (mode == PACK_BF16_FWD) return krows / (ks * ks * (bf16_ckb(ks * ks) / 8)) * (ldw / 64);
   if (mode == PACK_BF16_DGRAD) return (krows + 15) / 16 * (ldw / 64);
@@ -348,13 +365,22 @@
   for (int s = 0; s < nseg; ++s) { m.C[s] = Cseg[s]; m.off[s] = Coff ? Coff[s] : base; base += Cseg[s]; }
   const long total = (long)krows * ldw;
   const dim3 g(pack_grid(total)), b(256);
+  if (mode >= PACK_LIMB_FWD) {
+    const int nkb = krows / 3;
+    for (int l = 0; l < 3; ++l) {
+      hipLaunchKernelGGL(pack_bf16_kernel, dim3(pack_grid((long)nkb * ldw * 8)), b, 0, st, mode == PACK_LIMB_FWD ? PACK_BF16_FWD : PACK_BF16_DGRAD, W,
+                         (unsigned short*)out, Cout, Ctot, ks * ks, m, ldw, nkb, hid, l);
+      if (rsis_check_launch() != RSIS_OK) return RSIS_ERR_LAUNCH;
+    }
+    return RSIS_OK;
+  }
   if (mode >= PACK_WINO_FWD) {
     hipLaunchKernelGGL(pack_wino_kernel, dim3(krows), b, 0, st, mode, W, (float*)out, Cout, Ctot, m, hid);
     return rsis_check_launch();
   }
   if (mode >= PACK_BF16_FWD) {
     hipLaunchKernelGGL(pack_bf16_kernel, dim3(pack_grid(total * 8)), b, 0, st, mode, W, (unsigned short*)out, Cout, Ctot, ks * ks, m, ldw,
-                       krows, hid);
+                       krows, hid, -1);
     return rsis_check_launch();
   }
   hipLaunchKernelGGL(pack_kernel, g, b, 0, st, mode, W, (float*)out, Cout, Ctot, ks * ks, m, ldw, krows, hid);
diff --git a/rsis_amd/decoder_fused.py b/rsis_amd/decoder_fused.py
--- a/rsis_amd/decoder_fused.py
+++ b/rsis_amd/decoder_fused.py
@@ -73,11 +73,31 @@
     return cell._packs[key]
 
 
-def dyn_dgrad_pack(cell, c_up, c_skip, H, W):
+def _limb_pack(cell, dyn, what):
+    key = ("fused-limb", what) + tuple(dyn.segs)
+    if key not in cell._packs:
+        cell._packs[key] = ops.PackedConv(3, list(dyn.segs), lstm_hid=cell.hidden_size, stride=1, pad=1, offs=list(dyn.offs), dtype=ops.DTYPE_F32_LIMB)
+    return cell._packs[key]
+
+
+def _limb_ok(cell, dyn):
+    return dyn.dtype == ops.DTYPE_F32 and cell.kernel_size == 3 and cell.padding == 1 and all(s % 8 == 0 for s in dyn.segs)
+
+
+def dyn_fwd_pack(cell, c_up, c_skip, level, training):
+    _hoist, dyn = _packs(cell, c_up, c_skip)
+    if not training or level is None or not ops.limb_class("f%d" % level) or not _limb_ok(cell, dyn):
+        return dyn
+    return _limb_pack(cell, dyn, "fwd")
+
+
+def dyn_dgrad_pack(cell, c_up, c_skip, H, W, level=None):
     _hoist, dyn = _packs(cell, c_up, c_skip)
     hid = cell.hidden_size
     if (dyn.dtype != ops.DTYPE_F32 or not ops.WINOGRAD_GATES[0] or cell.kernel_size != 3 or cell.padding != 1 or min(H, W) < 12
             or (c_up + hid) % 32 or c_up % 32 or c_up == 0 or (4 * hid) % 32):
+        if level is not None and ops.limb_class("d%d" % level) and _limb_ok(cell, dyn) and (4 * hid) % 8 == 0:
+            return _limb_pack(cell, dyn, "dgrad")
         return dyn
     key = ("fused-dgrad-wino", c_up, c_skip)
     if key not in cell._packs:
diff --git a/rsis_amd/decoder_seq.py b/rsis_amd/decoder_seq.py
--- a/rsis_amd/decoder_seq.py
+++ b/rsis_amd/decoder_seq.py
@@ -80,7 +80,7 @@
 
 
 class _Level(object):
-    __slots__ = ("cell", "hid", "c_up", "c_skip", "H", "W", "hoist", "dyn", "G", "Hs", "Cs", "ACT", "UP", "KEY", "SIDE", "ARG", "skip")
+    __slots__ = ("cell", "hid", "c_up", "c_skip", "H", "W", "hoist", "dyn", "fwd_pack", "G", "Hs", "Cs", "ACT", "UP", "KEY", "SIDE", "ARG", "skip")
 
 
 UPCONV = [os.environ.get("RSIS_UPCONV", "1") != "0"]
@@ -182,7 +182,7 @@
             (j.B, j.H, j.W, j.Wp, j.bias_packed, j.addend, j.c_prev, j.h_out, j.c_out, j.act_out, j.hid, j.ks, j.pad, j.tile, j.dtype,
              j.side_key) = (self.B, lv.H, lv.W, wps[i].data_ptr(), None, lv.G.data_ptr(), lv.Cs[t - 1].data_ptr() if t > 0 else None,
                             lv.Hs[t].data_ptr(), lv.Cs[t].data_ptr(), lv.ACT[t].data_ptr() if lv.ACT is not None else None, lv.hid, 3, 1,
-                            ops.FORCE_TILE[0], lv.dyn.dtype, lv.KEY[t].data_ptr())
+                            ops.FORCE_TILE[0], lv.fwd_pack.dtype, lv.KEY[t].data_ptr())
         check(self.L.rsis_convlstm_fwd_batch(jobs, len(cells), stream()), "rsis_convlstm_fwd_batch")
 
     def up(self, levels, cells, s2=None):
@@ -438,7 +438,9 @@
         UP5 = None if upc else lay.empty((T, B), last.hid, H5, W5)
         probs_tb = torch.empty((T, B, Wc.shape[0]), **f32)
         stop_tb = torch.empty((T, B, 1), **f32)
-        wps = [lv.dyn.fwd(w) for lv, w in zip(levels, gates_w)]
+        for i, lv in enumerate(levels):
+            lv.fwd_pack = decoder_fused.dyn_fwd_pack(lv.cell, lv.c_up, lv.c_skip, i, need_grad and not lay.blk)
+        wps = [lv.fwd_pack.fwd(w) for lv, w in zip(levels, gates_w)]
         for d in range(T + n - 1):
             cells = _diagonal(d, n, T)
             lay.gates(levels, cells, wps)
@@ -542,7 +544,7 @@
         DHP = [lay.empty((B,), lv.hid, lv.H, lv.W) for lv in levels]
         DC = [[torch.empty((B, lv.hid, lv.H, lv.W), **f32) for _ in range(2)] for lv in levels]
         DUP = [lay.empty((B,), lv.c_up, lv.H, lv.W) if lv.c_up > 0 else None for lv in levels]
-        dpk = [decoder_fused.dyn_dgrad_pack(lv.cell, lv.c_up, lv.c_skip, lv.H, lv.W) for lv in levels]
+        dpk = [decoder_fused.dyn_dgrad_pack(lv.cell, lv.c_up, lv.c_skip, lv.H, lv.W, level=i) for i, lv in enumerate(levels)]
         wds = [pk.dgrad(w) for pk, w in zip(dpk, gates_w)]
         d_hidden = d_hidden or (None,) * (2 * n)
         dhf = [lay.from_nchw(g.contiguous()) if g is not None else None for g in d_hidden[0::2]]
diff --git a/rsis_amd/ops.py b/rsis_amd/ops.py
--- a/rsis_amd/ops.py
+++ b/rsis_amd/ops.py
@@ -23,6 +23,7 @@
 
 DTYPE_F32, DTYPE_BF16 = 0, 1
 DTYPE_F32_WINO = 3
+DTYPE_F32_LIMB = 4
 
 
 def _wino_rule():
@@ -35,6 +36,25 @@
 
 
 WINOGRAD = [_wino_rule()]
+
+LIMB_DEFAULT = "f1,f2,f3,f4,d3,d4"
+
+
+def _limb_rule():
+    v = os.environ.get("RSIS_CONV_LIMBS", LIMB_DEFAULT).strip().lower()
+    if v in ("0", "", "off", "none"):
+        return frozenset()
+    if v == "all":
+        return "all"
+    return frozenset(t.strip() for t in v.split(",") if t.strip())
+
+
+LIMBS = [_limb_rule()]
+
+
+def limb_class(name):
+    rule = LIMBS[0]
+    return rule == "all" or name in rule
 TRAINING_FORWARD = [False]
 WINOGRAD_INFER = [os.environ.get("RSIS_WINOGRAD_INFER", "0") == "1"]
 WINOGRAD_GATES = [os.environ.get("RSIS_WINOGRAD_GATES", "1") != "0" and os.environ.get("RSIS_WINOGRAD", "x").strip().lower() not in ("0", "off", "none")]
@@ -85,7 +105,7 @@
             todo.append((p, w, b, p.wd, 1))
     if not todo:
         return
-    sig = tuple((id(p), w.data_ptr(), out.data_ptr(), d) for p, w, _b, out, d in todo)
+    sig = tuple(p._job_sig(w, out, d) for p, w, _b, out, d in todo)
     if _BATCH["sig"] != sig:
         jobs = (_lib.PackJob * len(todo))()
         blocks = 0
@@ -159,6 +179,10 @@
             j.Coff[i] = self.offs[i] if self.offs is not None else off
             off += c
         return j
+
+    def _job_sig(self, w, out, dgrad):
+        return (w.data_ptr(), out.data_ptr(), int(dgrad), self.dtype, tuple(w.shape), self.ks, self.stride, self.pad, tuple(self.segs),
+                tuple(self.offs) if self.offs is not None else None, self.lstm_hid)
 
     def _seg_args(self):
         return len(self.segs), int_array(self.segs), (int_array(self.offs) if self.offs is not None else None)
```
